# duckmayr/gpirt

Hardware: AMD Instinct MI355X
Metric: MCMC iterations/sec at N=8192 x m=1024 (higher is better)
Workload: dtype f64

## Files before the change

### gpirt_amd/_lib.py

```python
from __future__ import annotations

import ctypes as C
import os

import numpy as np

HERE = os.path.dirname(os.path.abspath(__file__))
LIB_PATH = os.environ.get("GPIRT_HIP_LIBRARY") or os.path.join(HERE, "libgpirt_hip.so")

NGRID = 1001
RNG_RSTREAM, RNG_ITEM = 0, 1
ST_INIT_F, ST_INIT_BETA, ST_F_Z, ST_F_ESS, ST_FSTAR, ST_THETA, ST_BETA = 1, 2, 3, 4, 5, 6, 7
ST_PPC = 8
ST_ELL = 9
ST_AMP = 10
ST_CARRY = 11

E_ARG, E_HIP, E_NODEVICE, E_ALLOC, E_RNG, E_INTERRUPT, E_NUMERIC = -1, -2, -3, -4, -5, -6, -7

SUM_THETA_BETA, SUM_F, SUM_PRED, SUM_WAIC = 1, 2, 4, 8
SUM_PARTS = {"theta_beta": SUM_THETA_BETA, "f": SUM_F, "pred": SUM_PRED, "waic": SUM_WAIC}
SUM_DIAG = 16
SUM_THETA_HIST, SUM_IRF_BAND = 32, 128
SUM_PARTS.update(diag=SUM_DIAG, theta_hist=SUM_THETA_HIST, irf_band=SUM_IRF_BAND)
# ... 650 lines not shown
    "gpirt_ppc_person_combine": (_i32, [_vp, _i32, C.POINTER(_vp), C.POINTER(PpcPerson)]),
    "gpirt_sampler_ppc_resid_enable": (_i32, [_vp, _i32]),
    "gpirt_sampler_ppc_resid_get": (_i32, [_vp, C.c_char_p, _vp, _i64]),
    "gpirt_sampler_ppc_resid_state": (_i32, [_vp, C.POINTER(_vp), C.POINTER(_i64)]),
    "gpirt_ppc_resid_combine": (_i32, [_vp, _i32, C.POINTER(_vp), C.POINTER(PpcResid)]),
    "gpirt_sampler_equate_enable": (_i32, [_vp, _vp, _vp, _i32]),
    "gpirt_sampler_equate_accumulate": (_i32, [_vp]),
    "gpirt_sampler_equate_get": (_i32, [_vp, C.c_char_p, _vp, _i64]),
    "gpirt_sampler_equate_state": (_i32, [_vp, C.POINTER(_vp), C.POINTER(_i64)]),
    "gpirt_equate_state_bytes": (_i32, [_i64, _i64, _i64, C.POINTER(_i64)]),
    "gpirt_equate_combine": (_i32, [_vp, _i32, C.POINTER(_vp), C.POINTER(Equate)]),
    "gpirt_sampler_loo_enable": (_i32, [_vp, _i64, _i32, _i32]),
    "gpirt_sampler_loo_accumulate": (_i32, [_vp]),
    "gpirt_sampler_loo_get": (_i32, [_vp, C.c_char_p, _vp, _i64]),
    "gpirt_sampler_loo_state": (_i32, [_vp, C.POINTER(_vp), C.POINTER(_i64)]),
    "gpirt_loo_tail_length": (_i32, [_i64, _i32, C.POINTER(_i64)]),
    "gpirt_loo_state_bytes": (_i32, [_i64, _i64, _i64, C.POINTER(_i64)]),
    "gpirt_loo_combine": (_i32, [_vp, _i32, C.POINTER(_vp), C.POINTER(Loo)]),
    "gpirt_sampler_shape_order_enable": (_i32, [_vp, _i32]),
    "gpirt_sampler_shape_order_get": (_i32, [_vp, C.c_char_p, _vp, _i64]),
    "gpirt_sampler_shape_order_state": (_i32, [_vp, C.POINTER(_vp), C.POINTER(_i64)]),
    "gpirt_shape_order_state_bytes": (_i32, [_i64, _i32, C.POINTER(_i64)]),
    "gpirt_shape_order_combine": (_i32, [_vp, _i32, C.POINTER(_vp), C.POINTER(ShapeOrder)]),
    "gpirt_sampler_summary_accumulate": (_i32, [_vp]),
    "gpirt_sampler_summary_get": (_i32, [_vp, C.c_char_p, _dp, _i64]),
    "gpirt_sampler_summary_totals": (_i32, [_vp, _dp]),
    "gpirt_sampler_create": (_i32, [C.POINTER(_vp), _vp, _dp, _i64, _i64, _dp, _dp, _dp, _dp,
                                     C.POINTER(Options), _vp]),
    "gpirt_sampler_destroy": (_i32, [_vp]),
    "gpirt_sampler_init": (_i32, [_vp]),
    "gpirt_sampler_step": (_i32, [_vp]),
    "gpirt_sampler_draw_f": (_i32, [_vp]),
    "gpirt_sampler_draw_fstar": (_i32, [_vp]),
    "gpirt_sampler_theta_partial": (_i32, [_vp]),
    "gpirt_sampler_theta_finish": (_i32, [_vp]),
    "gpirt_sampler_set_theta_block": (_i32, [_vp, _vp, _i64, _i64, _i64]),
    "gpirt_sampler_theta_block": (_i32, [_vp]),
    "gpirt_sampler_theta_commit": (_i32, [_vp]),
    "gpirt_sampler_draw_beta": (_i32, [_vp]),
    "gpirt_sampler_factor": (_i32, [_vp]),
    "gpirt_sampler_skip_factor": (_i32, [_vp]),
    "gpirt_sampler_adopt_factor": (_i32, [_vp, _i32]),
    "gpirt_sampler_build_cov": (_i32, [_vp]),
    "gpirt_sampler_panel_factor": (_i32, [_vp, _i64]),
    "gpirt_sampler_panel_update": (_i32, [_vp, _i64, _i64]),
    "gpirt_sampler_panel_copy": (_i32, [_vp, _i64, _vp, _i32]),
    "gpirt_sampler_panel_rows": (_i32, [_vp, C.POINTER(_i64)]),
    "gpirt_sampler_panel_factor_part": (_i32, [_vp, _i64, _i32]),
    "gpirt_sampler_panel_update_part": (_i32, [_vp, _i64, _i64, _i32]),
    "gpirt_sampler_panel_copy_part": (_i32, [_vp, _i64, _i32, _vp, _i64, _i32]),
    "gpirt_sampler_ldl": (_i32, [_vp, C.POINTER(_i64)]),
    "gpirt_sampler_nu_lr_draws": (_i32, [_vp, C.POINTER(_i64)]),
    "gpirt_sampler_ess_pack_draws": (_i32, [_vp, C.POINTER(_i64)]),
    "gpirt_sampler_nu_lr_rows": (_i32, [_vp, _vp, _i64]),
    "gpirt_sampler_fstar_free_draws": (_i32, [_vp, C.POINTER(_i64)]),
    "gpirt_sampler_factor_lr_count": (_i32, [_vp, C.POINTER(_i64)]),
    "gpirt_sampler_dense_factor_count": (_i32, [_vp, C.POINTER(_i64)]),
    "gpirt_sampler_dense_factor": (_i32, [_vp]),
    "gpirt_sampler_factor_lr_parts": (_i32, [_vp, _vp, _i64]),
    "gpirt_sampler_factor_lr_width": (_i32, [_vp, C.POINTER(_i32)]),
    "gpirt_sampler_factor_lr_blocks": (_i32, [_vp, _vp, _i64]),
    "gpirt_sampler_copy_state": (_i32, [_vp, _vp]),
    "gpirt_sampler_accumulate_irf": (_i32, [_vp]),
    "gpirt_sampler_iteration": (_i32, [_vp, C.POINTER(_i32)]),
    "gpirt_sampler_check": (_i32, [_vp]),
    "gpirt_sampler_devptr": (_i32, [_vp, C.c_char_p, C.POINTER(_vp), C.POINTER(_i64)]),
    "gpirt_sampler_get": (_i32, [_vp, C.c_char_p, _vp, _i64]),
    "gpirt_sampler_set": (_i32, [_vp, C.c_char_p, _dp, _i64]),
    "gpirt_sampler_finish_irfs": (_i32, [_vp, _i32, _dp]),
    "gpirt_sampler_enable_timing": (_i32, [_vp, _i32]),
    "gpirt_sampler_stage_times": (_i32, [_vp, _dp, _i32, C.POINTER(_i32), C.POINTER(C.c_char_p)]),
    "gpirt_prof_trailing": (_i32, [_vp, _i32, _dp, C.POINTER(_i64), _dp]),
    "gpirt_prof_enable": (_i32, [_vp, _i32]),
    "gpirt_prof_syrk": (_i32, [_vp, _i32, _i32, _dp, C.POINTER(_i64), _dp]),
    "gpirt_prof_syrk_bytes": (_i32, [_vp, _i32, _dp]),
    "gpirt_sampler_set_iteration": (_i32, [_vp, _i32]),
    "gpirt_ell_grid": (_i32, [_dbl, _dbl, _i32, _dp]),
    "gpirt_ell_check": (_i32, [_dbl, _dbl, _i32, _dp, _i32, _i32, C.POINTER(Kernel), C.POINTER(Options), _i64]),
    "gpirt_sampler_ell_enable": (_i32, [_vp, _dbl, _dbl, _i32, _dp, _i32, _i32, _i32]),
    "gpirt_sampler_draw_ell": (_i32, [_vp]),
    "gpirt_sampler_ell_width": (_i32, [_vp, _i32]),
    "gpirt_sampler_ell_get": (_i32, [_vp, C.c_char_p, _vp, _i64]),
    "gpirt_sampler_ell_stats": (_i32, [_vp, C.POINTER(Ell)]),
    "gpirt_sampler_draw_ell_centred": (_i32, [_vp]),
    "gpirt_sampler_ell_width_centred": (_i32, [_vp, _i32]),
    "gpirt_sampler_ell_centred_stats": (_i32, [_vp, C.POINTER(EllCentred)]),
    "gpirt_amp_check": (_i32, [_dbl, _dbl, _i32, _dp, _i32, C.POINTER(_i32), _i64, C.POINTER(Options)]),
    "gpirt_sampler_amp_set": (_i32, [_vp, _dp]),
    "gpirt_sampler_amp_enable": (_i32, [_vp, _dbl, _dbl, _i32, _dp, _i32, C.POINTER(_i32), _i64, _i32]),
    "gpirt_sampler_draw_amp": (_i32, [_vp]),
    "gpirt_sampler_amp_width": (_i32, [_vp, C.POINTER(_i32)]),
    "gpirt_sampler_amp_record": (_i32, [_vp]),
    "gpirt_sampler_amp_get": (_i32, [_vp, C.c_char_p, _vp, _i64]),
    "gpirt_sampler_amp_stats": (_i32, [_vp, C.POINTER(Amp)]),
    "gpirt_sampler_draw_amp_centred": (_i32, [_vp]),
    "gpirt_sampler_amp_centred_stats": (_i32, [_vp, C.POINTER(AmpCentred)]),
    "gpirt_sampler_draw_beta_centred": (_i32, [_vp]),
    "gpirt_sampler_beta_centred_get": (_i32, [_vp, C.c_char_p, _vp, _i64]),
    "gpirt_sampler_beta_centred_stats": (_i32, [_vp, C.POINTER(BetaCentred)]),
    "gpirt_sampler_scale_enable": (_i32, [_vp, _dbl, _dbl]),
    "gpirt_sampler_scale_width": (_i32, [_vp, _i32, _dbl]),
    "gpirt_sampler_draw_scale": (_i32, [_vp, _i32]),
    "gpirt_sampler_scale_get": (_i32, [_vp, C.c_char_p, _vp, _i64]),
    "gpirt_sampler_scale_stats": (_i32, [_vp, C.POINTER(Scale)]),
    "gpirt_sampler_step_consistent_scale": (_i32, [_vp, _i32, _i32]),
    "gpirt_pop_check": (_i32, [C.POINTER(C.c_int32), _i64, _i32, _dp, _i64, _i32, _dbl, _i32, _dbl, _dbl, _i32, _dp, _dp,
# ... 96 lines not shown
```

### gpirt_amd/csrc/api.hip

```cpp
#include "common.h"
#include "kernels.h"
#include "rstream.h"

#include <stdarg.h>
#include <stdlib.h>
#include <new>
#include <vector>
#include <algorithm>

namespace gpirt {

static thread_local char g_err[512] = "";

static int env_value(const char* name, int dflt)
{
    const char* v = getenv(name);
    if (!v || !*v) return dflt;
    return atoi(v);
}
const Config& env_config()
{
    static const Config c = [] {
        Config d;
        d.nbo = env_value("GPIRT_NBO", d.nbo);            d.nbp = env_value("GPIRT_NBP", d.nbp);
        d.lookahead = env_value("GPIRT_LOOKAHEAD", d.lookahead);
        d.panel = env_value("GPIRT_PANEL", d.panel);      d.defer = env_value("GPIRT_DEFER", d.defer);
        d.trsm_inv = env_value("GPIRT_TRSM_INV", d.trsm_inv);
        d.ll_exact = env_value("GPIRT_LL_EXACT", d.ll_exact);
        d.ess_screen = env_value("GPIRT_ESS_SCREEN", d.ess_screen);
        d.theta_fixed = env_value("GPIRT_THETA_FIXED", d.theta_fixed);
        d.bordered = env_value("GPIRT_BORDERED", d.bordered);
        d.early_inv = env_value("GPIRT_EARLY_INV", d.early_inv);
        d.prep_early = env_value("GPIRT_PREP_EARLY", d.prep_early);
        d.guard_verbose = env_value("GPIRT_GUARD_VERBOSE", d.guard_verbose);
        d.rs_predict = env_value("GPIRT_RS_PREDICT", d.rs_predict);
        d.rs_lr = env_value("GPIRT_RS_LR", d.rs_lr);
        d.nu_lr = env_value("GPIRT_NU_LR", d.nu_lr);
        d.nu_sub = env_value("GPIRT_NU_SUB", NU_LR_SUB);
        d.fstar_free = env_value("GPIRT_FSTAR_FREE", d.fstar_free);
        d.factor_lr = env_value("GPIRT_FACTOR_LR", d.factor_lr);
        d.flr_fuse = env_value("GPIRT_FLR_FUSE", d.flr_fuse);
        d.flr_narrow = env_value("GPIRT_FLR_NARROW", d.flr_narrow);
        d.beta_screen = env_value("GPIRT_BETA_SCREEN", d.beta_screen);
        d.zfill_compact = env_value("GPIRT_ZFILL_COMPACT", d.zfill_compact);
        d.ess_pack = env_value("GPIRT_ESS_PACK", d.ess_pack);
        if (d.nbo < 64) d.nbo = 1024;
        if (d.nbp != 0 && d.nbp < 64) d.nbp = 512;
        return d;
    }();
    return c;
}

void set_error(const char* fmt, ...)
{
    va_list ap;
    va_start(ap, fmt);
    vsnprintf(g_err, sizeof(g_err), fmt, ap);
    va_end(ap);
}

int ensure_work(gpirt_handle_t h, size_t bytes)
{
    if (bytes <= h->work_bytes) return 0;
    GP_HIP(hipStreamSynchronize(h->stream));
    if (h->d_work) GP_HIP(hipFree(h->d_work));
    h->d_work = nullptr;
    h->work_bytes = 0;
    hipError_t e = hipMalloc(&h->d_work, bytes);
    if (e != hipSuccess) { set_error("hipMalloc(%zu) failed: %s", bytes, hipGetErrorString(e)); return GPIRT_E_ALLOC; }
    h->work_bytes = bytes;
    GP_HIP(poison_fresh(h, h->d_work, bytes, h->stream));
    return 0;
}

static int check_device(int device)
{
    int count = 0;
    hipError_t e = hipGetDeviceCount(&count);
    if (e != hipSuccess || count <= 0) {
        set_error("no HIP device visible (%s): libgpirt_hip has no CPU fallback",
                  e == hipSuccess ? "device count 0" : hipGetErrorString(e));
        return GPIRT_E_NODEVICE;
    }
    if (device >= count) { set_error("device %d out of range (%d visible)", device, count); return GPIRT_E_ARG; }
    return 0;
}

__global__ __launch_bounds__(256) void mfma_f64_peak_kernel(double* out, int iters)
{
    d4 acc[8];
#pragma unroll
    for (int i = 0; i < 8; ++i) acc[i] = d4{0.0, 0.0, 0.0, 0.0};
    double a = 1.0 + threadIdx.x * 1e-3, b = 1.0 - threadIdx.x * 1e-3;
    for (int it = 0; it < iters; ++it) {
#pragma unroll
        for (int i = 0; i < 8; ++i) acc[i] = __builtin_amdgcn_mfma_f64_16x16x4f64(a, b, acc[i], 0, 0, 0);
    }
    double s = 0.0;
// ... 15 lines not shown

int potrf_panel_copy(hipStream_t stream, double* A, int64_t n, int64_t lda, int64_t p, double* buf, bool to_buf,
                     int64_t extra_rows, int half, int64_t capacity)
{
    const int64_t W = potrf_panel_width(), H = potrf_subpanel_width(n), P0 = p * W;
    if (p < 0 || P0 >= n || half < 0 || half > 2) { set_error("panel %lld / half %d out of range", (long long)p, half); return GPIRT_E_ARG; }
    const int64_t P1 = (P0 + W < n) ? P0 + W : n;
    const int64_t mid = (P0 + H < P1) ? P0 + H : P1;
    const int64_t K0 = (half == 1) ? mid : P0, K1 = (half == 0) ? mid : P1;
    const int64_t w = K1 - K0, rows = n + extra_rows - K0;
    if (w <= 0) return 0;
    if (capacity >= 0 && rows * w > capacity) {
        set_error("panel copy: part %d of panel %lld is %lld x %lld doubles, the buffer holds %lld", half, (long long)p,
                  (long long)rows, (long long)w, (long long)capacity);
        return GPIRT_E_ARG;
    }
    double* a = A + K0 + K0 * lda;
    if (to_buf) GP_HIP(hipMemcpy2DAsync(buf, (size_t)rows * 8, a, (size_t)lda * 8, (size_t)rows * 8, (size_t)w, hipMemcpyDeviceToDevice, stream));
    else        GP_HIP(hipMemcpy2DAsync(a, (size_t)lda * 8, buf, (size_t)rows * 8, (size_t)rows * 8, (size_t)w, hipMemcpyDeviceToDevice, stream));
    return 0;
}

}

using namespace gpirt;

static int create_own_stream(gpirt_handle_t* out, int device, bool high_priority);
namespace gpirt {
int create_side_handle(gpirt_handle_t* out, int device) { return create_own_stream(out, device, true); }
}

namespace gpirt {
int prof_pair_begin(gpirt_handle_t h, hipStream_t stream, ProfPair& pp)
{
    pp = ProfPair{nullptr, nullptr, 0.0, 0, 0.0};
    if (!h->prof.enabled) return 0;
    if (!h->prof.free_pairs.empty()) { pp = h->prof.free_pairs.back(); h->prof.free_pairs.pop_back(); }
    else { GP_HIP(hipEventCreate(&pp.e0)); GP_HIP(hipEventCreate(&pp.e1)); }
    GP_HIP(hipEventRecord(pp.e0, stream));
    return 0;
}
int prof_pair_end(gpirt_handle_t h, hipStream_t stream, ProfPair& pp, int cls, double flops, double bytes)
{
    if (!pp.e0) return 0;
    GP_HIP(hipEventRecord(pp.e1, stream));
    pp.flops = flops; pp.bytes = bytes; pp.cls = cls;
    h->prof.pending.push_back(pp);
    return 0;
}
}

extern "C" {

int gpirt_version(void) { return 144; }

const char* gpirt_last_error(void) { return g_err; }

int gpirt_device_count(int* count)
{
    GP_ARG(count != nullptr);
    int c = 0;
    hipError_t e = hipGetDeviceCount(&c);
    *count = (e == hipSuccess) ? c : 0;
    return 0;
}

int gpirt_create(gpirt_handle_t* out, int device, void* stream)
{
    GP_ARG(out != nullptr);
    *out = nullptr;
    GP_TRY(check_device(device < 0 ? 0 : device));
    if (device >= 0) GP_HIP(hipSetDevice(device));
    int cur = 0;
    GP_HIP(hipGetDevice(&cur));
    hipDeviceProp_t prop;
    GP_HIP(hipGetDeviceProperties(&prop, cur));
    if (strncmp(prop.gcnArchName, "gfx950", 6) != 0) {
        set_error("device %d is %s; libgpirt_hip is built for gfx950 (MI355X) only", cur, prop.gcnArchName);
        return GPIRT_E_NODEVICE;
    }
    gpirt_handle_s* h = new (std::nothrow) gpirt_handle_s();
    if (!h) { set_error("out of host memory"); return GPIRT_E_ALLOC; }
    h->device = cur;
    h->cfg = env_config();
    h->n_cu = prop.multiProcessorCount;
    h->stream = (hipStream_t)stream;
    h->own_stream = false;
    const size_t prog_cap = 2048;
    hipError_t e = hipMalloc(&h->d_info, 64);
    if (e == hipSuccess) e = hipMalloc(&h->d_prog, 2 * prog_cap * sizeof(unsigned long long));
    if (e == hipSuccess) e = hipHostMalloc(&h->h_info, 64, hipHostMallocDefault);
    if (e == hipSuccess) e = hipMemsetAsync(h->d_info, 0, 64, h->stream);
    if (e == hipSuccess) e = hipMemsetAsync(h->d_prog, 0, 2 * prog_cap * sizeof(unsigned long long), h->stream);
    if (e == hipSuccess) e = hipStreamSynchronize(h->stream);
    if (e != hipSuccess) {
        set_error("handle workspace setup failed: %s", hipGetErrorString(e));
        gpirt_destroy(h);
        return GPIRT_E_ALLOC;
    }
    h->prog_cap = prog_cap;
    *out = h;
    return 0;
}

int gpirt_destroy(gpirt_handle_t h)
{
    if (!h) return 0;
// ... 23 lines not shown
    if (h->own_stream) hipStreamDestroy(h->stream);
    delete h;
    return 0;
}

int gpirt_synchronize(gpirt_handle_t h)
{
    GP_ARG(h != nullptr);
    GP_HIP(hipStreamSynchronize(h->stream));
    return 0;
}

static int create_own_stream(gpirt_handle_t* out, int device, bool high_priority)
{
    GP_ARG(out != nullptr);
    *out = nullptr;
    GP_TRY(check_device(device < 0 ? 0 : device));
    if (device >= 0) GP_HIP(hipSetDevice(device));
    hipStream_t st = nullptr;
    int lo_pri = 0, hi_pri = 0;
    hipError_t e = hipSuccess;
    if (high_priority) e = hipDeviceGetStreamPriorityRange(&lo_pri, &hi_pri);
    if (e == hipSuccess)
        e = high_priority ? hipStreamCreateWithPriority(&st, hipStreamNonBlocking, hi_pri)
                          : hipStreamCreateWithFlags(&st, hipStreamNonBlocking);
    if (e != hipSuccess) { set_error("hipStreamCreate failed: %s", hipGetErrorString(e)); return GPIRT_E_HIP; }
    const int rc = gpirt_create(out, device, st);
    if (rc != 0) { hipStreamDestroy(st); return rc; }
    (*out)->own_stream = true;
    return 0;
}

int gpirt_create_own_stream(gpirt_handle_t* out, int device) { return create_own_stream(out, device, false); }

static int* config_slot(gpirt_handle_t h, const char* name, bool* read_only)
{
    struct E { const char* k; int* p; bool ro; } tab[] = {
        { "GPIRT_NBO", &h->cfg.nbo, true }, { "GPIRT_NBP", &h->cfg.nbp, true },
        { "GPIRT_LOOKAHEAD", &h->cfg.lookahead, false }, { "GPIRT_PANEL", &h->cfg.panel, false },
        { "GPIRT_DEFER", &h->cfg.defer, false }, { "GPIRT_TRSM_INV", &h->cfg.trsm_inv, false },
        { "GPIRT_LL_EXACT", &h->cfg.ll_exact, false }, { "GPIRT_ESS_SCREEN", &h->cfg.ess_screen, false }, { "GPIRT_THETA_FIXED", &h->cfg.theta_fixed, false }, { "GPIRT_BORDERED", &h->cfg.bordered, false },
        { "GPIRT_EARLY_INV", &h->cfg.early_inv, false }, { "GPIRT_PREP_EARLY", &h->cfg.prep_early, false },
        { "GPIRT_RS_PREDICT", &h->cfg.rs_predict, false },
        { "GPIRT_RS_LR", &h->cfg.rs_lr, false },
        { "GPIRT_NU_LR", &h->cfg.nu_lr, false },
        { "GPIRT_NU_SUB", &h->cfg.nu_sub, false },
        { "GPIRT_FSTAR_FREE", &h->cfg.fstar_free, false },
        { "GPIRT_FACTOR_LR", &h->cfg.factor_lr, false },
        { "GPIRT_FLR_FUSE", &h->cfg.flr_fuse, false },
        { "GPIRT_FLR_NARROW", &h->cfg.flr_narrow, false },
        { "GPIRT_BETA_SCREEN", &h->cfg.beta_screen, false },
        { "GPIRT_ZFILL_COMPACT", &h->cfg.zfill_compact, false },
        { "GPIRT_ESS_PACK", &h->cfg.ess_pack, false },
    };
    for (auto& e : tab)
        if (strcmp(e.k, name) == 0) { if (read_only) *read_only = e.ro; return e.p; }
    return nullptr;
}

int gpirt_config_get(gpirt_handle_t h, const char* name, int* value)
{
    GP_ARG(h && name && value);
    int* p = config_slot(h, name, nullptr);
    if (!p) { set_error("unknown switch '%s'", name); return GPIRT_E_ARG; }
    *value = *p;
    return 0;
}

int gpirt_config_set(gpirt_handle_t h, const char* name, int value)
{
    GP_ARG(h && name);
    bool ro = false;
    int* p = config_slot(h, name, &ro);
    if (!p) { set_error("unknown switch '%s'", name); return GPIRT_E_ARG; }
    if (ro) { set_error("%s is fixed per process (set it in the environment before the library is loaded)", name); return GPIRT_E_ARG; }
    if (p == &h->cfg.nu_sub && !nu_lr_sub_ok(value)) { set_error("GPIRT_NU_SUB must be 64, 128, 256 or 512 (got %d)", value); return GPIRT_E_ARG; }
    GP_HIP(hipStreamSynchronize(h->stream));
    *p = value;
    if (h->aux) *config_slot(h->aux, name, nullptr) = value;
    return 0;
}

void gpirt_kernel_default(gpirt_kernel* k)
{
    if (!k) return;
    memset(k, 0, sizeof(*k));
    k->family = GPIRT_KERNEL_SE;
    k->length_scale = 1.0;
}

int gpirt_kernel_check(const gpirt_kernel* k, int kstar_rank, double* cert_out, int* min_rank_out)
{
    if (cert_out) *cert_out = 0.0;
    if (min_rank_out) *min_rank_out = 0;
    KernelSpec spec;
    GP_TRY(kernel_spec_from(k, &spec));
    return kernel_rank_check(spec, kstar_rank, cert_out, min_rank_out);
}

int gpirt_kernel_set(gpirt_handle_t h, const gpirt_kernel* k)
{
    GP_ARG(h != nullptr);
    KernelSpec spec;
    GP_TRY(kernel_spec_from(k, &spec));
    if (h->live_samplers > 0) {
        set_error("gpirt_kernel_set: %d sampler(s) created on this handle are alive; a sampler keeps the kernel it was created "
// ... 625 lines not shown
```

### gpirt_amd/csrc/common.h

```cpp
#pragma once

#include <hip/hip_runtime.h>
#include <stdint.h>
#include <stdio.h>
#include <string.h>
#include <math.h>
#include <vector>

#include "../../include/gpirt_hip.h"

namespace gpirt {

void set_error(const char* fmt, ...);

#define GP_HIP(call)                                                                         \
    do {                                                                                     \
        hipError_t e_ = (call);                                                              \
        if (e_ != hipSuccess) {                                                              \
            gpirt::set_error("%s failed: %s (%s:%d)", #call, hipGetErrorString(e_), __FILE__, \
                             __LINE__);                                                      \
            return GPIRT_E_HIP;                                                              \
        }                                                                                    \
    } while (0)

#define GP_ARG(cond)                                                                         \
    do {                                                                                     \
        if (!(cond)) {                                                                       \
            gpirt::set_error("bad argument: %s (%s:%d)", #cond, __FILE__, __LINE__);         \
            return GPIRT_E_ARG;                                                              \
        }                                                                                    \
    } while (0)

#define GP_TRY(call)                                                                         \
    do {                                                                                     \
        int r_ = (call);                                                                     \
        if (r_ != 0) return r_;                                                              \
    } while (0)

constexpr int PROF_CLASSES = 6;
struct ProfPair { hipEvent_t e0, e1; double flops; int cls; double bytes; };
struct Prof {
    bool        enabled = false;
    double      ms[PROF_CLASSES] = {};
    int64_t     launches[PROF_CLASSES] = {};
    double      flops[PROF_CLASSES] = {};
    double      bytes[PROF_CLASSES] = {};
    std::vector<ProfPair> pending;
    std::vector<ProfPair> free_pairs;
};

struct Config {
    int  nbo = 1024, nbp = 0;
    int  lookahead = 1;
    int  panel = 1;
    int  defer = 0;
    int  trsm_inv = 1;
    int  ll_exact = 0;
    int  theta_fixed = 1;
    int  ess_screen = 1;
    int  bordered = 1;
    int  early_inv = 1;
    int  prep_early = 1;
    int  rs_lr = 1;
    int  nu_lr = 1;
    int  nu_sub = 0;
    int  fstar_free = 1;
    int  factor_lr = 1;
    int  flr_fuse = 1;
    int  flr_narrow = 1;
    int  beta_screen = 1;
    int  ess_pack = 1;
    int  zfill_compact = 1;
    int  rs_predict = 1;
    int  guard_verbose = 0;
};
const Config& env_config();

struct KernelSpec {
    int    family = GPIRT_KERNEL_SE;
    double length_scale = 1.0;
    double inv_ell = 1.0;
    bool is_default() const { return family == GPIRT_KERNEL_SE && length_scale == 1.0; }
};

}

struct gpirt_handle_s {
    int          device = 0;
    gpirt::Config cfg;
    gpirt::KernelSpec kern;
    hipStream_t  stream = nullptr;
    bool         own_stream = false;
    int*         d_info = nullptr;
    int*         h_info = nullptr;
    double*      d_work = nullptr;
    size_t       work_bytes = 0;
    gpirt::Prof  prof;
    hipStream_t  side = nullptr;
    hipEvent_t   ev_fork = nullptr, ev_join = nullptr, ev_mid = nullptr, ev_half = nullptr;
    gpirt_handle_t aux = nullptr;
    const double* inv_partial_L = nullptr;
    int64_t      inv_partial_pairs = 0;
    bool         slim_leaf = false;
    hipEvent_t   ev_prelast = nullptr;
    int64_t      prelast_cols = 0;
    unsigned long long* d_prog = nullptr;
    double*      d_winv = nullptr;
    int64_t      winv_blocks = 0;
    double*      d_defer_ws = nullptr;
    size_t       defer_ws_bytes = 0;
    size_t       prog_cap = 0;
    unsigned long long prog_seq = 0;
    long long*   panel_trace = nullptr;
    int64_t      panel_trace_k0 = -1;
    int64_t      panel_trace_cap = 0;
    int          n_cu = 0;
    int          live_samplers = 0;
    bool         zombie = false;
    int          guard_fallbacks = 0;
    int64_t      cur_nbp = 512;
    long long    factor_count = 0;
    int          rs_trace_pass = -1;
    int          rs_mispredict = 0;
    int          rs_cand_limit = 0;
// ... 141 lines not shown
```

### gpirt_amd/csrc/kernels.h

```cpp
#pragma once

#include "common.h"

namespace gpirt {

enum { TRI_NONE = 0, TRI_SYRK_LOWER = 1, TRI_A_LOWER = 2, TRI_A_UPPER = 3, TRI_SYRK_LOWER_TRAILING = 4,
       TRI_SYRK_LOWER_BACKGROUND = 5  };
bool gemm_trailing_uses_128(int64_t M, int64_t N, bool background = false);
int launch_gemm_update_potf2(hipStream_t stream, int64_t M, int64_t N, int64_t K, const double* P, int64_t ldp,
                             double* C, int64_t ldc, int nb_next, int k0_next, int* info);

int launch_gemm(gpirt_handle_t h, hipStream_t stream, bool ta, bool tb, int tri, int64_t M,
                int64_t N, int64_t K, double alpha, const double* A, int64_t lda, const double* B,
                int64_t ldb, double beta, double* C, int64_t ldc, int64_t Mread = 0, const int* run_if = nullptr);

int launch_gemm_batched(hipStream_t stream, bool ta, bool tb, int tri, int64_t M, int64_t N, int64_t K, double alpha,
                        const double* A, int64_t lda, int64_t strideA, const double* B, int64_t ldb, int64_t strideB,
                        double beta, double* C, int64_t ldc, int64_t strideC, int batch);
int launch_gemm_batched_dual(hipStream_t stream, int tri, int64_t M, int64_t N, int64_t K, const double* A, int64_t lda,
                             int64_t strideA, const double* B, int64_t ldb, int64_t strideB, int64_t K2, const double* A2,
                             int64_t lda2, int64_t strideA2, const double* B2, int64_t ldb2, int64_t strideB2, double* C,
                             int64_t ldc, int64_t strideC, int batch);

int launch_syrk_panels(hipStream_t stream, int64_t M, int64_t N, int64_t kpart, int nparts, double alpha, const double* A,
// ... 346 lines not shown
    int64_t n, m;
    int sub;
};
void nu_lr_nodes(std::vector<double>& nodes, std::vector<double>& wts);
int64_t nu_lr_slabs(int64_t n);
int launch_nu_lr_basis(hipStream_t stream, const double* theta, int64_t n, const double* nodes, const double* wts, double* V);
int launch_nu_lr(hipStream_t stream, const NuLrArgs& a, double* flops, double* bytes);
constexpr int FSTAR_FREE_RANK = NU_LR_RANK;
void fstar_free_factor(const KernelSpec& kern, std::vector<double>& F);
int launch_fstar_free(hipStream_t stream, const double* V, int64_t n, const double* F, double eps, double* work, double* parts,
                      int nsplit, double* Cu, int* err);
int launch_fstar_free_xhat(hipStream_t stream, const double* Gv, const double* F, double eps, double* Xh, int batch, int* err,
                           bool prefix = false, double* R = nullptr,
                           bool chain = false);
struct FactorLrArgs {
    const double* theta; int64_t n;
    const double *nodes, *wts;
    double* V;
    const double* F; double eps;
    double *G, *Xh;
    double* X;
    double* D;
    double* L; int64_t ldl;
    double* Bt;
    int* err;
    int part;
};
int64_t factor_lr_parts(int64_t n, int part = 0);
int launch_factor_lr(gpirt_handle_t h, hipStream_t stream, const FactorLrArgs& a);
int launch_rs3p_products(hipStream_t stream, const Rs3Args& a);
int launch_rs3p_decide(hipStream_t stream, const Rs3Args& a);
int launch_rs_pred_start(hipStream_t stream, const uint64_t* anchor, uint64_t* anchorP, const int* k_last, int64_t m);
int launch_rs_gather(hipStream_t stream, const double* Nrm, const uint64_t* posv, const uint64_t* anchorP, int64_t n, int64_t j0,
                     int64_t m, double* Z);
int launch_rs_verify(hipStream_t stream, const RsVerifyArgs& a);
int launch_rs_commit(hipStream_t stream, const RsVerifyArgs& a, uint64_t* anchor, uint64_t* pos, uint64_t* ctl, int* err, double* f,
                     int* k_out);
int launch_ll_term_probe(hipStream_t stream, const double* a, int64_t n, double* out, int fast);
int launch_ll_bar(hipStream_t stream, const double* f, const double* y, const double* mu, int64_t n,
                  int64_t m, double* out);

int launch_colnorm_s(hipStream_t stream, const double* tmp, int64_t n, int64_t N, int64_t ld, double* s);
int launch_lowrank_s(hipStream_t stream, const double* V, int64_t N, int r, const double* G, int64_t ldg, double* s);
struct FstarEpiArgs {
    const double* mean; const double* mu_star; const double* s; double* out;
    int64_t N, m;
    uint64_t seed; uint32_t iter; uint32_t item0;
    const double* U; uint64_t* pos; uint64_t cap; int* err;
    double* mean_out;
    int* off_scratch;
    const double* amp;
};
int launch_fstar_epilogue(hipStream_t stream, const FstarEpiArgs& a);

int launch_indicators(hipStream_t stream, const double* y, int64_t n, int64_t m, double* Ypm );
int launch_loglik_terms(hipStream_t stream, const double* fstar, int64_t N, int64_t m, double* Gpm , int64_t ldg,
                        const int* run_if = nullptr);
int launch_theta_nan_fix(hipStream_t stream, const double* Gpm, int64_t ldg, const double* Ypm , int64_t n, int64_t m,
                         double* lp, int64_t N, int64_t ldlp, const int* run_if = nullptr);
struct TfDims { int64_t mp, ksteps, iblocks, gblocks; };
TfDims tf_dims(int64_t n, int64_t m, int64_t N);
size_t tf_y8_bytes(const TfDims& d);
size_t tf_gq_bytes(const TfDims& d);
size_t tf_aux_bytes(const TfDims& d);
int* tf_overflow(void* aux, const TfDims& d);
int launch_tf_indicators(hipStream_t stream, const double* y, int64_t n, int64_t ldy, int64_t m, const TfDims& d, void* Y8);
int launch_theta_fixed(hipStream_t stream, const double* fstar, int64_t N, int64_t n, int64_t m, const TfDims& d,
                       const void* Y8, void* Gq, void* aux, double* logpost, int64_t ldlp, bool trace = false,
                       gpirt_handle_t prof = nullptr);
long long* tf_trace(void* aux, const TfDims& d);
int tf_trace_wgs();
struct ThetaArgs {
    const double* logpost;
    int64_t N, n;
    int64_t i0;
    int stabilise;
    uint64_t seed; uint32_t iter;
    const double* U; uint64_t* pos; uint64_t cap;
    double* theta_out; int* degenerate; int* err;
    const double* log_prior; const int32_t* codes;
};
int launch_theta_sample(hipStream_t stream, const ThetaArgs& a);

struct BetaArgs {
    double* beta; const double* theta; const double* y; const double* f;
    const double* pm; const double* ps; const double* step;
    int64_t n, m, N;
    double* mu; double* mu_star;
    uint64_t seed; uint32_t iter; uint32_t item0;
    const double* U; uint64_t* pos; const uint64_t* item_off; uint64_t cap; int* err;
    int screen;
    int* path;
};
int launch_draw_beta(hipStream_t stream, const BetaArgs& a);
int launch_linear_mean(hipStream_t stream, const double* x, int64_t n, const double* beta, int64_t m, double* mu);

int prof_pair_begin(gpirt_handle_t h, hipStream_t stream, ProfPair& pp);
int prof_pair_end(gpirt_handle_t h, hipStream_t stream, ProfPair& pp, int cls, double flops, double bytes);

int report_panel_guard(gpirt_handle_t h, const int* info_words, hipStream_t stream);

int create_side_handle(gpirt_handle_t* out, int device);

constexpr int SUM_LAYOUT_VERSION = 1;
constexpr int SUM_HEADER_WORDS = 8;
struct SumLayout {
    int64_t tb_mean = -1, tb_m2 = -1, lse = -1, ll_mean = -1, ll_m2 = -1, y = -1, p_sum = -1, f_mean = -1, f_m2 = -1, irf = -1;
    int64_t dtb[7] = { -1, -1, -1, -1, -1, -1, -1 };
    int64_t df[7] = { -1, -1, -1, -1, -1, -1, -1 };
    int64_t total = 0;
};
enum { DG_H1_MEAN, DG_H1_M2, DG_H2_MEAN, DG_H2_M2, DG_BSUM, DG_BM_MEAN, DG_BM_M2 };
SumLayout summary_layout(int64_t n, int64_t m, int parts);
struct QntLayout {
    int64_t th_hist[3] = { -1, -1, -1 };
    int64_t th_off = -1;
    int64_t psum = -1;
    int64_t band_nan = -1;
    int64_t band = -1;
    int64_t total = 0;
};
QntLayout quantile_layout(int64_t n, int64_t m, int parts);
// ... 526 lines not shown
```

### gpirt_amd/csrc/sampler.hip

```cpp
#include "common.h"
#include "kernels.h"
#include "rstream.h"

#include <stdlib.h>
#include <new>
#include <mutex>
#include <type_traits>
#include <string>
#include <vector>

using namespace gpirt;

namespace {

constexpr int KSPLIT = 16;

enum { ST_DRAW_F = 0, ST_FSTAR, ST_THETA_GEMM, ST_THETA_SAMPLE, ST_BETA, ST_FACTOR, ST_COUNT };
const char* const kStageNames[ST_COUNT] = { "draw_f", "draw_fstar", "theta_gemm", "theta_sample",
                                            "draw_beta", "factor" };

}

enum { ELL_WHITENED = 0, ELL_CENTRED = 1 };
struct EllUpdate {
// ... 92 lines not shown
    double last_ms = 0.0, item_ms = 0.0;
};

struct ScaleState {
    bool on = false;
    uint32_t t[2] = {};
    double width[2] = {};
    ScaleArgs a{};
    int last_kind = -1;
    int prior_ok = -1;
    hipEvent_t tev[7] = {};
    double last_ms[2] = {};
    double times[6] = {};
};

struct CarryState {
    int64_t calls = 0;
    unsigned long long* counters = nullptr;
    double* quad = nullptr;
    hipEvent_t tev[2] = {};
    double last_ms = 0.0;
};

struct gpirt_sampler_s {
    gpirt_handle_t h = nullptr;
    int64_t n = 0, m = 0, N = GPIRT_NGRID;
    gpirt_options opt{};
    KernelSpec kern;
    RStream* rs = nullptr;
    double *y = nullptr, *Ypm = nullptr, *theta = nullptr, *theta_new = nullptr, *f = nullptr,
           *Z = nullptr, *NU = nullptr, *beta = nullptr, *mu = nullptr, *mu_star = nullptr,
           *fstar = nullptr, *L = nullptr, *tstar = nullptr, *kstar = nullptr, *rhs = nullptr,
           *mean = nullptr, *s = nullptr, *Gpm = nullptr, *logpost = nullptr, *irf_sum = nullptr,
           *pm = nullptr, *ps = nullptr, *step = nullptr;
    int kr = 0;
    double *knodes = nullptr, *kV = nullptr, *kparts = nullptr, *kP = nullptr;
    int64_t ext = 0, ldl = 0, node_off = -1, rank_off = 0;
    bool ext_grid = false, rows_valid = false, fstar_rows = false;
    double *nu_nodes = nullptr, *nu_wts = nullptr, *nuV = nullptr, *nuT = nullptr;
    bool nu_kern_ok = false, theta_ok = false, theta_alone = false;
    int64_t nu_lr_draws = 0;
    gpirt_handle_t haux = nullptr;
    hipEvent_t ev_trmm = nullptr, ev_prep = nullptr;
    bool prep_valid = false, prep_pending = false;
    double *ffF = nullptr, *ffW = nullptr;
    bool ff_have = false, prep_free = false;
    double ff_ell = 0.0;
    int64_t fstar_free_draws = 0;
    double *theta_L = nullptr, *flrG = nullptr, *flrXh = nullptr, *flrX = nullptr, *flrD = nullptr;
    bool L_structured = false;
    int L_part_width = 0;
    hipEvent_t ev_flr = nullptr;
    int64_t factor_lr_count = 0, dense_factor_count = 0;
    uint32_t z_filled_iter = 0;
    hipEvent_t ev_zfill = nullptr;
    bool beta_deferred = false, beta_pending = false;
    hipEvent_t ev_beta = nullptr;
    int64_t blk_i0 = 0, blk_n = 0, blk_m = 0;
    double *Ypm_blk = nullptr, *Gpm_full = nullptr, *logpost_blk = nullptr, *fstar_full = nullptr, *theta_stage = nullptr;
    TfDims tfd{}, tfd_blk{};
    double *tf_y8 = nullptr, *tf_gq = nullptr, *tf_aux = nullptr, *tf_y8_blk = nullptr, *tf_gq_blk = nullptr, *tf_aux_blk = nullptr;
    int *ess_k = nullptr, *flags = nullptr;
    int *fstar_off = nullptr;
    int *h_flags = nullptr;
    double* U = nullptr; double* hU = nullptr; uint64_t U_cap = 0;
    uint64_t* pos = nullptr; uint64_t* h_pos = nullptr; uint64_t* beta_off = nullptr;
    uint64_t beta_total = 0;
    RStream saved{};
    bool stream_open = false;
    gpirt_rstream_s* rs_obj = nullptr;
    bool ahead_attached = false;
    uint64_t ahead_gen = 0, ahead_used = 0, a_len = 0;
    std::vector<std::pair<uint64_t, RStream>> snaps;
    uint32_t *hA = nullptr, *Sraw = nullptr;
    double *S = nullptr, *U2 = nullptr;
    hipStream_t cs = nullptr;
    hipEvent_t ev_up = nullptr, ev_asm = nullptr;
    bool spec_ok = false;
    uint64_t *posv = nullptr, *anchor = nullptr, *h_next = nullptr;
    unsigned long long* rs_flags = nullptr; double* rs_partial = nullptr; uint64_t rs_tag = 0;
    double* Lt = nullptr;
    double *Nrm = nullptr, *rs_part = nullptr;
    uint32_t* rs_units = nullptr; int rs_nunits = 0, rs_nfull = 0;
    uint32_t* rs_unitsP = nullptr; int rs_nunitsP = 0, rs_nfullP = 0;
    long long* rs_trace = nullptr;
    float *Lt32 = nullptr, *rs_part32 = nullptr;
    uint64_t *anchorP = nullptr, *rs_ctl = nullptr, *rs_posP = nullptr;
    double *rs_dec_part = nullptr, *rs_dec_rec = nullptr; unsigned* rs_dec_ticket = nullptr;
    double rs_pass_rate = 0.0; uint64_t rs_pass_seen = 0;
    int *rs_kpred = nullptr, *rs_kv = nullptr, *rs_used = nullptr, *rs_ierr = nullptr, *rs_errP = nullptr;
    double *lr_nodes = nullptr, *lr_wts = nullptr, *lr_M = nullptr, *lr_V64 = nullptr, *lr_Gb = nullptr;
    float *lr_V32t = nullptr, *lr_Ct32 = nullptr, *lr_Y = nullptr;
    int* lr_bad = nullptr; uint32_t* lr_units = nullptr; int lr_nunits = 0;
    bool lr_on = false; int lr_strikes = 0; uint64_t rs_mis_seen = 0;
    int iter = 0;
    bool initialised = false;
    bool sticky_info = false;
    bool factor_fresh = false;
    bool counted = false;
    bool in_init = false;
    bool timing = false;
    hipEvent_t ev[ST_COUNT + 1] = {};
    double stage_ms[ST_COUNT] = {};
    std::vector<void*> allocs;
    std::vector<double> host_tmp;
    SummaryState sum;
    PpcState ppc;
    RankState rank;
    ShapeState shape;
    ScoreState score;
    SumscoreState sumscore;
    EquateState equate;
    LooState loo;
    AcfState acf;
    GroupsState groups;
    EllState ell;
    AmpState amp;
    OrdState ord;
    PopState pop;
    CarryState carry;
    SmoothF sf;
    BetaCentredState bc;
    ScaleState sc;
    bool lp_current = false;
    bool mu_linear = false;
    uint32_t* ess_ypk = nullptr;
    bool ess_ypk_valid = false;
    int64_t ess_pack_draws = 0;
};

namespace {

template <typename T>
int dalloc(gpirt_sampler_s* s, T** p, size_t count, bool numbers = true)
{
    void* q = nullptr;
    const size_t bytes = (count ? count : 1) * sizeof(T);
    hipError_t e = hipMalloc(&q, bytes);
    if (e != hipSuccess) {
        set_error("hipMalloc(%zu bytes) failed: %s", bytes, hipGetErrorString(e));
        return GPIRT_E_ALLOC;
    }
    s->allocs.push_back(q);
    *p = reinterpret_cast<T*>(q);
    if (std::is_same<T, double>::value || std::is_same<T, float>::value) {
        if (numbers && poison_fresh(s->h, q, bytes, s->h->stream) != hipSuccess) {
            set_error("hipMemsetAsync(%zu bytes) failed", bytes);
            return GPIRT_E_HIP;
        }
    }
    return 0;
}

inline bool stream_mode(const gpirt_sampler_s* s) { return s->opt.rng_kind == GPIRT_RNG_RSTREAM; }

int report_degenerate_theta(gpirt_sampler_s* s, int count);

void ahead_generate(gpirt_sampler_s* s, uint32_t* dst, uint64_t count)
{
    constexpr uint64_t EVERY = 1ull << 16;
    while (count) {
        const uint64_t c = count < EVERY ? count : EVERY;
        s->snaps.emplace_back(s->ahead_gen, *s->rs);
        s->rs->fill_raw(dst, c);
        s->ahead_gen += c; dst += c; count -= c;
    }
}

void ahead_resolve(void* owner, bool gone)
{
    gpirt_sampler_s* s = static_cast<gpirt_sampler_s*>(owner);
    if (s->ahead_attached) {
        if (s->ev_up) hipEventSynchronize(s->ev_up);
        size_t best = 0;
        for (size_t q = 0; q < s->snaps.size(); ++q) if (s->snaps[q].first <= s->ahead_used) best = q;
        *s->rs = s->snaps[best].second;
        s->rs->skip(s->ahead_used - s->snaps[best].first);
    }
    s->ahead_attached = false;
    s->snaps.clear();
    s->ahead_gen = s->ahead_used = s->a_len = 0;
    if (s->rs_obj) { s->rs_obj->owner = nullptr; s->rs_obj->resolve = nullptr; }
    if (gone) { s->rs_obj = nullptr; s->rs = nullptr; }
// ... 156 lines not shown
        std::lock_guard<std::mutex> lock(mu);
        if (cached.empty() || cached_ell != s->kern.length_scale) {
            fstar_free_factor(s->kern, cached);
            cached_ell = s->kern.length_scale;
        }
        F = cached;
    }
    GP_HIP(hipMemcpyAsync(s->ffF, F.data(), sizeof(double) * F.size(), hipMemcpyHostToDevice, s->h->stream));
    GP_HIP(hipStreamSynchronize(s->h->stream));
    s->ff_have = true; s->ff_ell = s->kern.length_scale;
    return 0;
}

bool fstar_free_ok(const gpirt_sampler_s* s, bool state_only = false)
{
    const int mode = s->h->cfg.fstar_free;
    return mode != 2 && (mode == 3 || s->n >= 2048) && s->kr == NU_LR_RANK && s->fstar_rows && s->node_off >= 0 && s->nuV &&
           !stream_mode(s) && s->nu_kern_ok && !s->opt.kernel_fp32 && s->theta_ok && (state_only || !s->theta_alone) && !s->ell.on &&
           s->ffF && s->ff_have && s->kern.family == GPIRT_KERNEL_SE && s->ff_ell == s->kern.length_scale;
}

bool factor_lr_ok(const gpirt_sampler_s* s)
{
    const Config& c = s->h->cfg;
    return s->opt.factor_structured && s->theta_L && c.factor_lr != 2 && (c.factor_lr == 3 || s->n >= 2048) &&
           c.nu_lr != 2 && (c.nu_lr == 3 || s->n >= 2048) && fstar_free_ok(s, true);
}

int fstar_prep_free(gpirt_sampler_s* s, hipStream_t st, bool basis)
{
    const int64_t n = s->n;
    const int r = s->kr;
    const double* Bt = s->L + n + s->rank_off;
    if (basis) GP_TRY(launch_nu_lr_basis(st, s->theta, n, s->nu_nodes, s->nu_wts, s->nuV));
    GP_TRY(launch_fstar_free(st, s->nuV, n, s->ffF, GPIRT_JITTER, s->ffW, s->kparts, KSPLIT, s->rhs + (size_t)n * r, s->flags));
    return launch_gemm_splitk(st, false, true, r, r, n, 1.0, Bt, s->ldl, Bt, s->ldl, s->kparts, r, (int64_t)r * r, KSPLIT,
                              s->kP, r, 0.0);
}
int report_degenerate_theta(gpirt_sampler_s* s, int count);
int rebuild_rows(gpirt_sampler_s* s);
int beta_sync(gpirt_sampler_s* s);
int ensure_dense_factor(gpirt_sampler_s* s);
int ensure_factor_width(gpirt_sampler_s* s, int need);

int z_sync(gpirt_sampler_s* s)
{
    if (s->z_filled_iter != 0 && s->ev_zfill) GP_HIP(hipStreamWaitEvent(s->h->stream, s->ev_zfill, 0));
    s->z_filled_iter = 0;
    return 0;
}

int do_draw_f(gpirt_sampler_s* s)
{
    s->lp_current = false;
    gpirt_handle_t h = s->h;
    hipStream_t st = h->stream;
    const int64_t n = s->n, m = s->m;
    const uint32_t iter = (uint32_t)(s->iter + 1);
    GP_TRY(beta_sync(s));
    s->factor_fresh = false;
    if (!stream_mode(s)) {
        const bool nu_lr = s->node_off >= 0 && s->nuV && h->cfg.nu_lr != 2 && (h->cfg.nu_lr == 3 || n >= 2048) &&
                           s->nu_kern_ok && !s->opt.kernel_fp32 && s->theta_ok && !s->theta_alone;
        if (!nu_lr) GP_TRY(ensure_dense_factor(s));
        if (nu_lr) GP_TRY(rebuild_rows(s));
        if (nu_lr) GP_TRY(ensure_factor_width(s, h->cfg.nu_sub));
        const bool prep = s->haux && s->kr > 0 && s->fstar_rows && s->rows_valid && !s->prep_valid;
        const bool free = prep && fstar_free_ok(s);
        if (prep && !free) GP_TRY(ensure_dense_factor(s));
        const bool early = prep && !free && !(h->cfg.prep_early == 2 && m > 128);
        if (early || (free && !nu_lr)) GP_HIP(hipEventRecord(s->ev_trmm, st));
        if (nu_lr && s->prep_pending && s->prep_free) {
            GP_HIP(hipStreamWaitEvent(st, s->ev_prep, 0));
            s->prep_pending = false;
        }
        if (s->z_filled_iter == iter && s->ev_zfill) {
            GP_HIP(hipStreamWaitEvent(st, s->ev_zfill, 0));
            s->z_filled_iter = 0;
        } else {
            GP_TRY(z_sync(s));
            GP_TRY(launch_item_uniforms(st, s->opt.seed, iter, GPIRT_ST_F_Z, (uint32_t)s->opt.item0, m, n, s->Z, true, s->h->cfg.zfill_compact == 1));
        }
        {
            ProfPair pp;
            GP_TRY(prof_pair_begin(h, st, pp));
            if (nu_lr) {
                double flops = 0.0, bytes = 0.0;
                NuLrArgs q{};
                q.L = s->L; q.ldl = s->ldl; q.Bt = s->L + n + s->node_off; q.V = s->nuV; q.Z = s->Z; q.NU = s->NU; q.T = s->nuT;
                q.n = n; q.m = m; q.sub = h->cfg.nu_sub;
                GP_TRY(launch_nu_lr_basis(st, s->theta, n, s->nu_nodes, s->nu_wts, s->nuV));
                if (free) GP_HIP(hipEventRecord(s->ev_trmm, st));
                GP_TRY(launch_nu_lr(st, q, &flops, &bytes));
                GP_TRY(prof_pair_end(h, st, pp, 3, flops, bytes));
                s->nu_lr_draws += 1;
            } else {
                GP_TRY(launch_gemm(h, st, false, false, TRI_A_LOWER, n, m, n, 1.0, s->L, s->ldl, s->Z, n, 0.0, s->NU, n));
                GP_TRY(prof_pair_end(h, st, pp, 3, (double)n * (double)n * (double)m, 8.0 * (0.5 * (double)n * (double)n + 2.0 * (double)n * (double)m)));
            }
        }
        if (s->amp.mode) GP_TRY(launch_amp_scale(st, s->NU, s->amp.amp, n, m));
        if (prep && !early && !free) GP_HIP(hipEventRecord(s->ev_trmm, st));
        if (s->ord.on) {
            EssOrdArgs a{};
            a.f = s->f; a.nu = s->NU; a.mu = s->mu; a.cat = s->ord.cat; a.thr = s->ord.thr; a.counts = s->ord.counts;
            a.C = s->ord.C; a.n = n; a.m = m; a.k_out = s->ess_k; a.err = s->flags;
            a.seed = s->opt.seed; a.iter = iter; a.item0 = (uint32_t)s->opt.item0;
// ... 129 lines not shown
        if (predict) GP_HIP(hipMemcpyAsync(s->h_next + 2, s->rs_ctl + 3, sizeof(uint64_t), hipMemcpyDeviceToHost, st));
        if (predict) GP_HIP(hipMemcpyAsync(s->h_next + 3, s->rs_ctl + 1, sizeof(uint64_t), hipMemcpyDeviceToHost, st));
        if (lr) GP_HIP(hipMemcpyAsync(s->h_next + 4, s->lr_bad, sizeof(int), hipMemcpyDeviceToHost, st));
        if (s->stream_open && !topped) { GP_TRY(ahead_topup(s, stream_window(s))); topped = true; }
        GP_HIP(hipStreamSynchronize(st));
        if ((int)s->h_next[1] != 0) break;
        if (predict) {
            if (lr && (int)s->h_next[4] != 0) { s->lr_on = false; lr = false; }
            if (lr && s->h_next[3] != s->rs_mis_seen) { lr = false; lr_missed = true; }
            s->rs_mis_seen = s->h_next[3];
        }
        if ((int64_t)s->h_next[0] <= done) {
            if (predict) {
                predict = false;
                GP_TRY(launch_advance_pos(st, s->rs_ctl + 2, 1));
                continue;
            }
            set_error("R-stream replay: draw_f made no progress"); return GPIRT_E_NUMERIC;
        }
        if (predict && (int64_t)s->h_next[0] > done) {
            const uint64_t real = s->h_next[2] - s->rs_pass_seen;
            s->rs_pass_seen = s->h_next[2];
            s->rs_pass_rate = (double)real / (double)((int64_t)s->h_next[0] - done);
        }
        done = (int64_t)s->h_next[0];
    }
    if (s->lr_on) {
        s->lr_strikes = lr_missed ? s->lr_strikes + 1 : 0;
        if (s->lr_strikes >= 3) s->lr_on = false;
    }
    return 0;
}

int fstar_prep(gpirt_sampler_s* s, gpirt_handle_t hh)
{
    hipStream_t st = hh->stream;
    const int64_t n = s->n;
    const int r = s->kr;
    double* Cu = s->rhs + (size_t)n * r;
    const double* Bt = s->L + n + s->rank_off;
    GP_TRY(launch_transpose(st, Bt, r, n, s->ldl, Cu, n));
    if (hh == s->haux && hh->inv_partial_L == s->L && hh->inv_partial_pairs > 0 && hh->trsm_winv_L != s->L) {
        GP_TRY(trsm_inverses_build(hh, st, s->L, n, s->ldl, true, hh->inv_partial_pairs, (n / 256) / 2));
        trsm_inverses_mark(hh, s->L, n, s->ldl, true);
        hh->inv_partial_L = nullptr; hh->inv_partial_pairs = 0;
    }
    GP_TRY(launch_trsm_lower(hh, st, s->L, n, s->ldl, Cu, r, n, true, true));
    return launch_gemm_splitk(st, false, true, r, r, n, 1.0, Bt, s->ldl, Bt, s->ldl, s->kparts, r, (int64_t)r * r, KSPLIT,
                              s->kP, r, 0.0);
}

int do_draw_fstar(gpirt_sampler_s* s, uint32_t iter)
{
    s->lp_current = false;
    gpirt_handle_t h = s->h;
    hipStream_t st = h->stream;
    const int64_t n = s->n, m = s->m, N = s->N;
    double* tmp = s->rhs;
    double* W = s->rhs + (size_t)n * N;
    const bool fused = s->opt.fstar_fused != 0;
    GP_TRY(beta_sync(s));
    s->factor_fresh = false;
    GP_TRY(rebuild_rows(s));
    if (s->kr > 0) {
        const int r = s->kr;
        double* Bu = s->rhs;
        double* Cu = s->rhs + (size_t)n * r;
        const bool bordered = s->fstar_rows;
        if (bordered) {
            if (!s->prep_valid) {
                if (s->prep_pending) { GP_HIP(hipStreamWaitEvent(st, s->ev_prep, 0)); s->prep_pending = false; }
                s->prep_free = fstar_free_ok(s);
                if (s->prep_free) GP_TRY(fstar_prep_free(s, st, true));
                else { GP_TRY(ensure_dense_factor(s)); GP_TRY(fstar_prep(s, h)); }
                s->prep_valid = true;
            }
            else if (s->prep_pending) { GP_HIP(hipStreamWaitEvent(st, s->ev_prep, 0)); s->prep_pending = false; }
            if (s->prep_free) s->fstar_free_draws += 1;
        } else {
            GP_TRY(launch_se_kernel(st, s->kern, s->theta, n, s->knodes, r, Bu, n, 0.0));
            GP_TRY(launch_trsm_lower(h, st, s->L, n, s->ldl, Bu, r, n, false));
            GP_HIP(hipMemcpyAsync(Cu, Bu, sizeof(double) * (size_t)n * r, hipMemcpyDeviceToDevice, st));
            GP_TRY(launch_trsm_lower(h, st, s->L, n, s->ldl, Cu, r, n, true, true));
        }
        double* G = s->kP;
        double* Q = s->kP + (size_t)r * r;
        if (!bordered)
            GP_TRY(launch_gemm_splitk(st, true, false, r, r, n, 1.0, Bu, n, Bu, n, s->kparts, r, (int64_t)r * r, KSPLIT, G, r, 0.0));
        GP_TRY(launch_gemm_splitk(st, true, false, r, m, n, 1.0, Cu, n, s->f, n, s->kparts, r, (int64_t)r * m, KSPLIT, Q, r, 0.0));
        GP_TRY(launch_lowrank_s(st, s->kV, N, r, G, r, s->s));
        GP_TRY(launch_gemm(h, st, false, false, TRI_NONE, N, m, r, 1.0, s->kV, N, Q, r, 0.0, s->mean, N));
        FstarEpiArgs a{};
        a.mean = s->mean; a.mu_star = s->mu_star; a.s = s->s; a.out = s->fstar; a.N = N; a.m = m;
        a.seed = s->opt.seed; a.iter = iter; a.item0 = (uint32_t)s->opt.item0; a.err = s->flags;
        if (stream_mode(s)) { a.U = s->U; a.pos = s->pos; a.cap = s->U_cap; a.off_scratch = s->fstar_off; }
        if (s->shape.on) a.mean_out = s->shape.gbar;
        if (s->amp.mode) a.amp = s->amp.amp;
        return launch_fstar_epilogue(st, a);
    }
    GP_HIP(hipMemcpyAsync(W, s->f, sizeof(double) * (size_t)n * m, hipMemcpyDeviceToDevice, st));
    if (s->ext_grid) {
        if (!fused) GP_TRY(launch_se_kernel(st, s->kern, s->theta, n, s->tstar, N, s->kstar, n, 0.0));
        GP_TRY(launch_transpose(st, s->L + n, N, n, s->ldl, tmp, n));
        GP_TRY(launch_trsm_lower(h, st, s->L, n, s->ldl, W, m, n, false));
    } else {
        if (fused) {
            GP_TRY(launch_se_kernel(st, s->kern, s->theta, n, s->tstar, N, tmp, n, 0.0));
        } else {
            GP_TRY(launch_se_kernel(st, s->kern, s->theta, n, s->tstar, N, s->kstar, n, 0.0));
            GP_HIP(hipMemcpyAsync(tmp, s->kstar, sizeof(double) * (size_t)n * N, hipMemcpyDeviceToDevice, st));
        }
        GP_TRY(launch_trsm_lower(h, st, s->L, n, s->ldl, s->rhs, N + m, n, false));
    }
    GP_TRY(launch_colnorm_s(st, tmp, n, N, n, s->s));
    if (fused) {
        GP_TRY(launch_gemm(h, st, true, false, TRI_NONE, N, m, n, 1.0, tmp, n, W, n, 0.0, s->mean, N));
    } else {
        GP_TRY(launch_trsm_lower(h, st, s->L, n, s->ldl, W, m, n, true, true));
        GP_TRY(launch_gemm(h, st, true, false, TRI_NONE, N, m, n, 1.0, s->kstar, n, W, n, 0.0, s->mean, N));
    }
    FstarEpiArgs a{};
    a.mean = s->mean; a.mu_star = s->mu_star; a.s = s->s; a.out = s->fstar; a.N = N; a.m = m;
    a.seed = s->opt.seed; a.iter = iter; a.item0 = (uint32_t)s->opt.item0; a.err = s->flags;
    if (stream_mode(s)) { a.U = s->U; a.pos = s->pos; a.cap = s->U_cap; a.off_scratch = s->fstar_off; }
    if (s->shape.on) a.mean_out = s->shape.gbar;
    if (s->amp.mode) a.amp = s->amp.amp;
    return launch_fstar_epilogue(st, a);
}

int theta_product(gpirt_sampler_s* s, const double* fstar_in, double* logpost_out)
{
    hipStream_t st = s->h->stream;
    const int64_t n = s->n, m = s->m, N = s->N;
    const int64_t Np = (N + 127) / 128 * 128;
    const int* only_if = nullptr;
    if (s->h->cfg.theta_fixed == 1) {
        GP_TRY(launch_theta_fixed(st, fstar_in, N, n, m, s->tfd, s->tf_y8, s->tf_gq, s->tf_aux, logpost_out, N, false, s->h));
        only_if = tf_overflow(s->tf_aux, s->tfd);
    }
    GP_TRY(launch_loglik_terms(st, fstar_in, N, m, s->Gpm, Np, only_if));
    GP_TRY(launch_gemm(s->h, st, false, true, TRI_NONE, N, n, 2 * m, 1.0, s->Gpm, Np, s->Ypm, n, 0.0, logpost_out, N, Np, only_if));
    return launch_theta_nan_fix(st, s->Gpm, Np, s->Ypm, n, m, logpost_out, N, N, only_if);
}

int theta_product_ord(gpirt_sampler_s* s, const double* fstar_in, double* logpost_out)
{
    hipStream_t st = s->h->stream;
    const OrdState& A = s->ord;
    const int64_t n = s->n, m = s->m, N = s->N;
    const int64_t Np = (N + 127) / 128 * 128;
    GP_TRY(launch_ord_loglik_terms(st, fstar_in, N, m, A.C, A.thr, A.G, Np));
    GP_TRY(launch_gemm(s->h, st, false, true, TRI_NONE, N, n, (int64_t)A.C * m, 1.0, A.G, Np, A.Y, n, 0.0, logpost_out, N, Np));
    return launch_ord_nan_fix(st, A.G, Np, A.cat, n, m, logpost_out, N, N);
}

int do_theta_partial(gpirt_sampler_s* s)
{
    if (s->ord.on) {
        GP_TRY(theta_product_ord(s, s->fstar, s->logpost));
        s->lp_current = true;
        return 0;
    }
    GP_TRY(theta_product(s, s->fstar, s->logpost));
    s->lp_current = true;
    return 0;
}

int do_theta_finish(gpirt_sampler_s* s)
{
    hipStream_t st = s->h->stream;
    ThetaArgs a{};
    a.logpost = s->logpost; a.N = s->N; a.n = s->n; a.stabilise = s->opt.theta_stabilise;
    a.seed = s->opt.seed; a.iter = (uint32_t)(s->iter + 1);
    a.theta_out = s->theta; a.degenerate = s->flags + 1; a.err = s->flags;
    if (stream_mode(s)) { a.U = s->U; a.pos = s->pos; a.cap = s->U_cap; }
    if (s->pop.mode) { a.log_prior = s->pop.log_prior; a.codes = s->pop.codes; }
    GP_TRY(launch_theta_sample(st, a));
    if (stream_mode(s)) GP_TRY(launch_advance_pos(st, s->pos, (uint64_t)s->n));
    s->lp_current = false;
    s->mu_linear = false;
    s->theta_ok = true;
    return 0;
}

int do_theta_block(gpirt_sampler_s* s)
{
    hipStream_t st = s->h->stream;
    const int64_t N = s->N, nb = s->blk_n, mt = s->blk_m;
    const int64_t Np = (N + 127) / 128 * 128;
    GP_HIP(hipMemsetAsync(s->theta_stage, 0, sizeof(double) * (size_t)s->n, st));
    if (nb == 0) return 0;
    const int* only_if = nullptr;
    if (s->h->cfg.theta_fixed == 1) {
        GP_TRY(launch_theta_fixed(st, s->fstar_full, N, nb, mt, s->tfd_blk, s->tf_y8_blk, s->tf_gq_blk, s->tf_aux_blk, s->logpost_blk, N, false, s->h));
        only_if = tf_overflow(s->tf_aux_blk, s->tfd_blk);
    }
    GP_TRY(launch_loglik_terms(st, s->fstar_full, N, mt, s->Gpm_full, Np, only_if));
    GP_TRY(launch_gemm(s->h, st, false, true, TRI_NONE, N, nb, 2 * mt, 1.0, s->Gpm_full, Np, s->Ypm_blk, nb, 0.0,
                       s->logpost_blk, N, Np, only_if));
    GP_TRY(launch_theta_nan_fix(st, s->Gpm_full, Np, s->Ypm_blk, nb, mt, s->logpost_blk, N, N, only_if));
    ThetaArgs a{};
    a.logpost = s->logpost_blk; a.N = N; a.n = nb; a.i0 = s->blk_i0; a.stabilise = s->opt.theta_stabilise;
    a.seed = s->opt.seed; a.iter = (uint32_t)(s->iter + 1);
    a.theta_out = s->theta_stage; a.degenerate = s->flags + 1; a.err = s->flags;
    return launch_theta_sample(st, a);
}

int launch_beta_on(gpirt_sampler_s* s, hipStream_t st)
{
    s->lp_current = false;
    s->mu_linear = !s->ord.on;
    if (s->ord.on) {
        BetaOrdArgs a{};
        a.beta = s->beta; a.theta = s->theta; a.cat = s->ord.cat; a.f = s->f; a.thr = s->ord.thr; a.pm = s->pm; a.ps = s->ps;
        a.step = s->step; a.C = s->ord.C; a.n = s->n; a.m = s->m; a.N = s->N; a.mu = s->mu; a.mu_star = s->mu_star;
        a.seed = s->opt.seed; a.iter = (uint32_t)(s->iter + 1); a.item0 = (uint32_t)s->opt.item0;
        return launch_draw_beta_ord(st, a);
    }
    BetaArgs a{};
    a.beta = s->beta; a.theta = s->theta; a.y = s->y; a.f = s->f; a.pm = s->pm; a.ps = s->ps;
    a.step = s->step; a.n = s->n; a.m = s->m; a.N = s->N; a.mu = s->mu; a.mu_star = s->mu_star;
    a.seed = s->opt.seed; a.iter = (uint32_t)(s->iter + 1); a.item0 = (uint32_t)s->opt.item0;
    a.err = s->flags;
    a.screen = s->h->cfg.beta_screen == 1;
    if (stream_mode(s)) { a.U = s->U; a.pos = s->pos; a.item_off = s->beta_off; a.cap = s->U_cap; }
    GP_TRY(launch_draw_beta(st, a));
    if (stream_mode(s)) GP_TRY(launch_advance_pos(st, s->pos, s->beta_total));
    return 0;
}

int beta_sync(gpirt_sampler_s* s)
{
    if (s->beta_deferred) {
        s->beta_deferred = false;
        GP_TRY(launch_beta_on(s, s->h->stream));
    }
    if (s->beta_pending) {
        GP_HIP(hipStreamWaitEvent(s->h->stream, s->ev_beta, 0));
        s->beta_pending = false;
    }
    return 0;
}

int do_draw_beta(gpirt_sampler_s* s)
{
    const bool defer = s->h->cfg.early_inv != 2 && !stream_mode(s) && s->haux && s->ev_beta && s->initialised;
    GP_TRY(beta_sync(s));
    if (defer) { s->beta_deferred = true; return 0; }
    return launch_beta_on(s, s->h->stream);
}

int carry_refusals(gpirt_sampler_s* s, int nugget, const char* entry)
{
    if (!s->initialised) { set_error("%s needs an initialised sampler (gpirt_sampler_init)", entry); return GPIRT_E_ARG; }
    if (stream_mode(s)) {
        set_error("carry: rng = reference (GPIRT_RNG_RSTREAM) is refused, R's stream has no such draw");
        return GPIRT_E_ARG;
    }
    if (nugget != 0 && nugget != 1) { set_error("carry: nugget = %d, it must be 0 or 1", nugget); return GPIRT_E_ARG; }
    return 0;
}

int do_carry_f(gpirt_sampler_s* s, int nugget, bool timed)
{
    CarryState& c = s->carry;
    hipStream_t st = s->h->stream;
    GP_TRY(beta_sync(s));
    s->lp_current = false;
    s->mu_linear = false;
    if (!c.counters) {
        GP_TRY(dalloc(s, &c.counters, 6));
        GP_HIP(hipMemsetAsync(c.counters, 0, 6 * sizeof(unsigned long long), st));
    }
    CarryArgs a{};
    a.slot = (int)(c.calls & 1);
    a.f = s->f; a.theta = s->theta; a.fstar = s->fstar; a.mu_star = s->mu_star; a.n = s->n; a.m = s->m; a.N = s->N;
    a.amp = s->amp.mode ? s->amp.amp : nullptr;
    a.counters = c.counters;
    a.seed = s->opt.seed; a.iter = (uint32_t)(s->iter + 1); a.item0 = (uint32_t)s->opt.item0; a.nugget = nugget;
    if (timed) {
        for (hipEvent_t& t : c.tev) if (!t) GP_HIP(hipEventCreate(&t));
        GP_HIP(hipEventRecord(c.tev[0], st));
    }
    GP_TRY(launch_carry_f(st, a));
    if (timed) GP_HIP(hipEventRecord(c.tev[1], st));
    c.calls += 1;
    c.last_ms = 0.0;
    return 0;
}

void invalidate_factor_products(gpirt_sampler_s* s)
{
    s->prep_valid = false;
    if (s->haux && s->haux->inv_partial_L == s->L) { s->haux->inv_partial_L = nullptr; s->haux->inv_partial_pairs = 0; }
    if (s->h->trsm_winv_L == s->L) s->h->trsm_winv_L = nullptr;
    if (s->haux && s->haux->trsm_winv_L == s->L) s->haux->trsm_winv_L = nullptr;
}

int aux_join(gpirt_sampler_s* s, bool beta_too = true, bool z_too = true)
{
    hipStream_t st = s->h->stream;
    if (s->prep_pending) { GP_HIP(hipStreamWaitEvent(st, s->ev_prep, 0)); s->prep_pending = false; }
    if (beta_too) GP_TRY(beta_sync(s));
    if (z_too) GP_TRY(z_sync(s));
    return 0;
}

int build_cov(gpirt_sampler_s* s, const double* theta = nullptr)
{
    hipStream_t st = s->h->stream;
    if (!theta) theta = s->theta;
    s->L_structured = false;
    GP_TRY(launch_se_kernel_lower(st, s->kern, theta, s->n, s->L, s->ldl, GPIRT_JITTER, s->opt.kernel_fp32 != 0));
    if (s->fstar_rows && s->kr > 0) GP_TRY(launch_se_kernel(st, s->kern, s->knodes, s->kr, theta, s->n, s->L + s->n + s->rank_off, s->ldl, 0.0));
    if (s->ext_grid) GP_TRY(launch_se_kernel(st, s->kern, s->tstar, s->N, theta, s->n, s->L + s->n, s->ldl, 0.0));
    if (s->node_off >= 0 && !(s->fstar_rows && s->kr == NU_LR_RANK))
        GP_TRY(launch_se_kernel(st, s->kern, s->nu_nodes, NU_LR_RANK, theta, s->n, s->L + s->n + s->node_off, s->ldl, 0.0));
    return 0;
}

int rebuild_rows(gpirt_sampler_s* s)
// ... 204 lines not shown
                     (void*)p->hist_mu, (void*)p->hist_sd, (void*)p->draws })
        if (q) hipFree(q);
    for (hipEvent_t t : p->tev) if (t) hipEventDestroy(t);
    const uint32_t calls = p->t;
    *p = PopState();
    p->t = calls;
}

int ell_join(gpirt_sampler_s* s)
{
    GP_TRY(aux_join(s, true, false));
    if (s->haux) {
        GP_HIP(hipEventRecord(s->ell.ev, s->haux->stream));
        GP_HIP(hipStreamWaitEvent(s->h->stream, s->ell.ev, 0));
    }
    return 0;
}

void ell_set_kernel(gpirt_sampler_s* s, double ell)
{
    s->kern.length_scale = ell;
    s->kern.inv_ell = 1.0 / ell;
}

int ell_settle_factor(gpirt_sampler_s* s)
{
    if (!s->factor_fresh) return 0;
    gpirt_handle_t h = s->h;
    hipStream_t st = h->stream;
    GP_HIP(hipMemcpyAsync(h->h_info, h->d_info, 8 * sizeof(int), hipMemcpyDeviceToHost, st));
    GP_HIP(hipStreamSynchronize(st));
    if (h->h_info[1] != 0) {
        if (h->cfg.panel == 2) return report_panel_guard(h, h->h_info, st);
        GP_TRY(recover_factor(s));
        GP_HIP(hipMemcpyAsync(h->h_info, h->d_info, 8 * sizeof(int), hipMemcpyDeviceToHost, st));
        GP_HIP(hipStreamSynchronize(st));
        if (h->h_info[1] != 0) return report_panel_guard(h, h->h_info, st);
    }
    if (*h->h_info > 0) {
        set_error("chol(): decomposition failed (leading minor of order %d is not positive definite)", *h->h_info);
        return *h->h_info;
    }
    return 0;
}

int do_draw_ell(gpirt_sampler_s* s, int kind)
{
    EllState& e = s->ell;
    EllUpdate& c = e.up[kind];
    gpirt_handle_t h = s->h;
    hipStream_t st = h->stream;
    const int64_t n = s->n, m = s->m;
    GP_TRY(ell_settle_factor(s));
    s->lp_current = false;
    const uint32_t t = c.t + 1;
    const double u0 = item_uniform(s->opt.seed, t, GPIRT_ST_ELL, (uint32_t)kind, 0),
                 u1 = item_uniform(s->opt.seed, t, GPIRT_ST_ELL, (uint32_t)kind, 1);
    auto counted = [&]() { c.t = t; c.updates += 1; c.last_u0 = u0; c.last_u1 = u1; };
    const int w = c.w;
    int j = (int)floor(u0 * (double)(2 * w));
    if (j > 2 * w - 1) j = 2 * w - 1;
    const int kp = e.k + (j < w ? j - w : j - w + 1);
    if (kp < 0 || kp >= e.P) { counted(); c.last_proposed = kp; c.out_of_range += 1; c.last = 2; return 0; }
    GP_TRY(ell_join(s));
    GP_TRY(ensure_dense_factor(s));
    s->factor_fresh = false;
    const bool timed = s->timing;
    if (timed)
        for (hipEvent_t& t : e.tev) if (!t) GP_HIP(hipEventCreate(&t));
    auto tick = [&](int i) { if (timed) hipEventRecord(e.tev[i], st); };
    const KernelSpec kern_before = s->kern;
    const bool rows_before = s->rows_valid;
    const size_t fbytes = sizeof(double) * (size_t)(n * m), lbytes = sizeof(double) * (size_t)(s->ldl * n);
    auto restore = [&]() -> int {
        s->kern = kern_before;
        s->rows_valid = rows_before;
        invalidate_factor_products(s);
        GP_HIP(hipMemcpyAsync(s->L, e.Lsave, lbytes, hipMemcpyDeviceToDevice, st));
        return 0;
    };
    tick(0);
    GP_HIP(hipMemcpyAsync(s->NU, s->f, fbytes, hipMemcpyDeviceToDevice, st));
    if (kind == ELL_CENTRED) GP_HIP(hipMemcpyAsync(e.nuprop, s->f, fbytes, hipMemcpyDeviceToDevice, st));
    GP_HIP(hipMemcpyAsync(e.Lsave, s->L, lbytes, hipMemcpyDeviceToDevice, st));
    tick(1);
    GP_TRY(launch_trsm_lower(h, st, s->L, n, s->ldl, s->NU, m, n, false));
    tick(2);
    ell_set_kernel(s, e.grid[(size_t)kp]);
    int rc = factor_core(s);
    c.factorisations += 1;
    tick(3);
    const double lp_diff = e.log_prior[(size_t)kp] - e.log_prior[(size_t)e.k], log_u = log(u1);
    for (int attempt = 0; !rc; ++attempt) {
        if (kind == ELL_WHITENED) {
            rc = launch_gemm(h, st, false, false, TRI_A_LOWER, n, m, n, 1.0, s->L, s->ldl, s->NU, n, 0.0, e.fprop, n);
            tick(4);
            if (!rc) rc = launch_ell_delta(st, s->f, e.fprop, s->mu, s->y, n, m, e.delta, e.nonfin);
            tick(5);
            if (!rc) rc = launch_ell_decide(st, e.delta, e.nonfin, m, lp_diff, log_u, h->d_info, e.rec, e.flag);
            tick(6);
            if (!rc) rc = launch_ell_commit(st, e.flag, s->f, e.fprop, n * m);
            tick(7);
        } else {
            if (attempt > 0 && hipMemcpyAsync(e.nuprop, s->f, fbytes, hipMemcpyDeviceToDevice, st) != hipSuccess) {
                set_error("length-scale update: copying f failed: %s", hipGetErrorString(hipGetLastError()));
                rc = GPIRT_E_HIP;
            }
// ... 265 lines not shown
}

}

extern "C" {

int gpirt_sampler_create(gpirt_sampler_t* out, gpirt_handle_t h, const double* h_y, int64_t n,
                         int64_t m, const double* h_theta0, const double* h_pm, const double* h_ps,
                         const double* h_step, const gpirt_options* opts, gpirt_rstream_t rs)
{
    GP_ARG(out && h && h_y && h_theta0 && h_pm && h_ps && h_step && n > 0 && m > 0);
    *out = nullptr;
    for (int64_t i = 0; i < n * m; ++i) {
        const double v = h_y[i];
        if (!(v == 1.0 || v == -1.0 || v != v)) { set_error("y must be +1, -1 or NaN (a missing response)"); return GPIRT_E_ARG; }
    }
    gpirt_sampler_s* s = new (std::nothrow) gpirt_sampler_s();
    if (!s) { set_error("out of host memory"); return GPIRT_E_ALLOC; }
    s->h = h; s->n = n; s->m = m; s->N = GPIRT_NGRID;
    if (opts) s->opt = *opts; else gpirt_default_options(&s->opt);
    if (s->opt.m_total <= 0) s->opt.m_total = m;
    s->kern = h->kern;
    if (!s->kern.is_default()) {
        if (s->opt.kernel_fp32) {
            set_error("kernel_fp32 needs the default kernel (squared exponential, length_scale 1): the handle's kernel is family %d, "
                      "length_scale %g", s->kern.family, s->kern.length_scale);
            delete s;
            return GPIRT_E_ARG;
        }
        if (s->opt.kstar_rank != 0 && s->opt.fstar_fused && s->opt.kstar_rank >= 16 && s->opt.kstar_rank <= 128 &&
            (s->opt.kstar_rank % 16) == 0) {
            const int rc_k = kernel_rank_check(s->kern, s->opt.kstar_rank, nullptr, nullptr);
            if (rc_k) { delete s; return rc_k; }
        }
    }
    if (stream_mode(s)) {
        if (!rs) { set_error("GPIRT_RNG_RSTREAM needs an R stream state"); delete s; return GPIRT_E_ARG; }
        if (s->opt.item0 != 0 || s->opt.m_total != m) {
            set_error("R-stream replay is sequential over items and cannot be sharded"); delete s; return GPIRT_E_ARG;
        }
        rstream_sync(rs);
        s->rs = &rs->r; s->rs_obj = rs;
        rs->attached.push_back(s); rs->forget = rstream_forget;
    }
    const int64_t N = s->N;
    hipStream_t st = h->stream;
    int rc = 0;
#define GP_A(p, cnt) do { rc = dalloc(s, &(p), (size_t)(cnt)); if (rc) { gpirt_sampler_destroy(s); return rc; } } while (0)
    GP_A(s->y, n * m);       GP_A(s->Ypm, n * 2 * m);  GP_A(s->theta, n);       GP_A(s->theta_new, n);
    s->tfd = tf_dims(n, m, N);
#define GP_AI(p, cnt) do { rc = dalloc(s, &(p), (size_t)(cnt), false); if (rc) { gpirt_sampler_destroy(s); return rc; } } while (0)
    GP_AI(s->tf_y8, tf_y8_bytes(s->tfd) / 8 + 2); GP_AI(s->tf_gq, tf_gq_bytes(s->tfd) / 8 + 2); GP_AI(s->tf_aux, tf_aux_bytes(s->tfd) / 8 + 2);
#undef GP_AI
    GP_A(s->f, n * m);       GP_A(s->Z, n * m);        GP_A(s->NU, n * (m > 1 + TRMV_SPLIT ? m : 1 + TRMV_SPLIT));   GP_A(s->beta, 2 * m);
    s->kr = s->opt.kstar_rank;
    if (s->kr != 0 && (!s->opt.fstar_fused || s->kr < 16 || s->kr > 128 || (s->kr % 16) != 0)) {
        set_error("kstar_rank must be a multiple of 16 in 16..128 and needs fstar_fused");
        gpirt_sampler_destroy(s);
        return GPIRT_E_ARG;
    }
    if (s->opt.factor_structured != 0 && s->opt.factor_structured != 1) {
        set_error("factor_structured must be 0 or 1");
        gpirt_sampler_destroy(s);
        return GPIRT_E_ARG;
    }
    const bool bordered_ok = (n % 64) == 0 && h->cfg.bordered != 2;
    if (bordered_ok) {
        if (s->kr == NU_LR_RANK) { s->ext = s->kr; s->node_off = 0; s->rank_off = 0; s->fstar_rows = true; }
        else if (s->kr > 0) { s->ext = NU_LR_RANK + s->kr; s->node_off = 0; s->rank_off = NU_LR_RANK; s->fstar_rows = true; }
        else if (n >= 1024) {
            s->node_off = (N + 63) / 64 * 64;
            s->ext = s->node_off + NU_LR_RANK;
            s->ext_grid = true; s->fstar_rows = true;
        } else { s->ext = NU_LR_RANK; s->node_off = 0; }
    } else if ((n % 64) == 0) { s->ext = NU_LR_RANK; s->node_off = 0; }
    s->ldl = n + s->ext;
    s->theta_ok = true;
    for (int64_t i = 0; i < n; ++i) s->theta_ok = s->theta_ok && h_theta0[i] >= -5.0 && h_theta0[i] <= 5.0;
    s->nu_kern_ok = nu_kernel_ok(s->kern);
    GP_A(s->mu, n * m);      GP_A(s->mu_star, N * m + 1); GP_A(s->fstar, N * m + 1); GP_A(s->L, s->ldl * n);
    GP_A(s->tstar, N + 1);   GP_A(s->rhs, n * (N + m) + 2); GP_A(s->mean, N * m + 1); GP_A(s->s, N + 1);
    GP_A(s->Gpm, ((N + 127) / 128 * 128) * 2 * m + 2); GP_A(s->logpost, N * n + 2); GP_A(s->irf_sum, N * m + 1);
    if (hipMemsetAsync(s->Gpm, 0, sizeof(double) * (size_t)(((N + 127) / 128 * 128) * 2 * m + 2), st) != hipSuccess) {
        set_error("hipMemsetAsync(Gpm) failed"); gpirt_sampler_destroy(s); return GPIRT_E_HIP;
    }
    GP_A(s->pm, 2 * m);      GP_A(s->ps, 2 * m);       GP_A(s->step, 2 * m);
    GP_A(s->ess_k, m);       GP_A(s->flags, 4);
    if (!stream_mode(s) && ess_pack_eligible(n)) {
        rc = dalloc(s, &s->ess_ypk, (size_t)(512 * m), false);
        if (rc) { gpirt_sampler_destroy(s); return rc; }
    }
    if (!s->opt.fstar_fused) GP_A(s->kstar, n * N + 2);
    if (s->node_off >= 0) {
        GP_A(s->nu_nodes, NU_LR_RANK); GP_A(s->nu_wts, NU_LR_RANK);
        if (!stream_mode(s)) {
            GP_A(s->nuV, n * NU_LR_RANK); GP_A(s->nuT, nu_lr_slabs(n) * NU_LR_RANK * m);
            if (hipMemsetAsync(s->nuT, 0, sizeof(double) * (size_t)(NU_LR_RANK * m), st) != hipSuccess) {
                set_error("hipMemsetAsync(nuT) failed"); gpirt_sampler_destroy(s); return GPIRT_E_HIP;
            }
        }
        if (!stream_mode(s) && s->kr == NU_LR_RANK && s->fstar_rows) {
            GP_A(s->ffF, FSTAR_FREE_RANK * FSTAR_FREE_RANK); GP_A(s->ffW, 2 * FSTAR_FREE_RANK * FSTAR_FREE_RANK);
            if (s->opt.factor_structured) {
                const int64_t fp = factor_lr_parts(n, NU_LR_SUB_MIN) * NU_LR_RANK * NU_LR_RANK;
                GP_A(s->theta_L, n); GP_A(s->flrG, fp); GP_A(s->flrXh, fp); GP_A(s->flrX, NU_LR_RANK * n);
                GP_A(s->flrD, factor_lr_parts(n) * (NU_LR_PART / 64) * NU_LR_RANK * NU_LR_RANK);
// ... 305 lines not shown
}

int gpirt_sampler_draw_f(gpirt_sampler_t s) { GP_ARG(s && s->initialised); return do_draw_f(s); }
int gpirt_sampler_draw_fstar(gpirt_sampler_t s) { GP_ARG(s && s->initialised); return do_draw_fstar(s, (uint32_t)(s->iter + 1)); }
int gpirt_sampler_theta_partial(gpirt_sampler_t s) { GP_ARG(s && s->initialised); return do_theta_partial(s); }
int gpirt_sampler_theta_finish(gpirt_sampler_t s) { GP_ARG(s && s->initialised); return do_theta_finish(s); }

int gpirt_sampler_set_theta_block(gpirt_sampler_t s, const double* y_block, int64_t i0, int64_t n_block, int64_t m_total)
{
    GP_ARG(s && (y_block || n_block == 0) && i0 >= 0 && n_block >= 0 && i0 + n_block <= s->n && m_total >= s->m);
    if (stream_mode(s)) { set_error("the R-stream replay cannot be sharded"); return GPIRT_E_ARG; }
    if (s->fstar_full) { set_error("the theta block is already set"); return GPIRT_E_ARG; }
    GP_TRY(ord_refuse(s, "gpirt_sampler_set_theta_block", "the respondent-block theta path has no one-hot product"));
    if (s->pop.mode) {
        set_error("gpirt_sampler_set_theta_block is refused while a population prior is on: the block path would need the codes of its respondents");
        return GPIRT_E_ARG;
    }
    const int64_t N = s->N, Np = (N + 127) / 128 * 128;
    int rc = 0;
    double* yb = nullptr;
#define GP_B(p, cnt) do { rc = dalloc(s, &(p), (size_t)(cnt)); if (rc) return rc; } while (0)
    GP_B(s->Ypm_blk, n_block * 2 * m_total + 2); GP_B(s->Gpm_full, Np * 2 * m_total + 2);
    GP_B(s->logpost_blk, N * n_block + 2);       GP_B(s->fstar_full, N * m_total + 2);
    GP_B(s->theta_stage, s->n + 1);              GP_B(yb, n_block * m_total + 1);
    s->tfd_blk = tf_dims(n_block, m_total, N);
#undef GP_B
#define GP_B(p, cnt) do { rc = dalloc(s, &(p), (size_t)(cnt), false); if (rc) return rc; } while (0)
    GP_B(s->tf_y8_blk, tf_y8_bytes(s->tfd_blk) / 8 + 2); GP_B(s->tf_gq_blk, tf_gq_bytes(s->tfd_blk) / 8 + 2);
    GP_B(s->tf_aux_blk, tf_aux_bytes(s->tfd_blk) / 8 + 2);
#undef GP_B
    hipStream_t st = s->h->stream;
    GP_HIP(hipMemsetAsync(s->Gpm_full, 0, sizeof(double) * (size_t)(Np * 2 * m_total + 2), st));
    if (n_block > 0) {
        GP_HIP(hipMemcpyAsync(yb, y_block, sizeof(double) * (size_t)(n_block * m_total), hipMemcpyHostToDevice, st));
        GP_TRY(launch_indicators(st, yb, n_block, m_total, s->Ypm_blk));
        GP_TRY(launch_tf_indicators(st, yb, n_block, n_block, m_total, s->tfd_blk, s->tf_y8_blk));
    }
    GP_HIP(hipStreamSynchronize(st));
    s->blk_i0 = i0; s->blk_n = n_block; s->blk_m = m_total;
    return 0;
}

int gpirt_sampler_theta_block(gpirt_sampler_t s)
{
    GP_ARG(s && s->initialised);
    if (!s->fstar_full) { set_error("gpirt_sampler_set_theta_block has not been called"); return GPIRT_E_ARG; }
    return do_theta_block(s);
}

int gpirt_sampler_theta_commit(gpirt_sampler_t s)
{
    GP_ARG(s && s->initialised && s->theta_stage);
    GP_HIP(hipMemcpyAsync(s->theta, s->theta_stage, sizeof(double) * (size_t)s->n, hipMemcpyDeviceToDevice, s->h->stream));
    s->lp_current = false;
    s->mu_linear = false;
    s->theta_ok = true;
    return 0;
}
int gpirt_sampler_draw_beta(gpirt_sampler_t s) { GP_ARG(s && s->initialised); return do_draw_beta(s); }
int gpirt_sampler_factor(gpirt_sampler_t s)
{
    GP_ARG(s && s->initialised);
    GP_TRY(do_factor(s));
    s->iter += 1;
    return 0;
}

int gpirt_sampler_build_cov(gpirt_sampler_t s)
{
    GP_ARG(s && s->initialised);
    hipStream_t st = s->h->stream;
    if (!s->sticky_info) GP_HIP(hipMemsetAsync(s->h->d_info, 0, sizeof(int), st));
    GP_TRY(aux_join(s));
    invalidate_factor_products(s);
    return build_cov(s);
}

int gpirt_sampler_adopt_factor(gpirt_sampler_t s, int rows_with_L)
{
    GP_ARG(s && s->initialised);
    GP_TRY(beta_sync(s));
    invalidate_factor_products(s);
    s->L_structured = false;
    s->factor_fresh = false;
    s->rows_valid = rows_with_L != 0;
    s->theta_alone = false;
    s->iter += 1;
    return 0;
}

int gpirt_sampler_skip_factor(gpirt_sampler_t s) { return gpirt_sampler_adopt_factor(s, 0); }

int gpirt_sampler_step(gpirt_sampler_t s)
{
    GP_ARG(s && s->initialised);
    if (stream_mode(s)) GP_TRY(stream_begin(s, stream_window(s)));
    mark(s, 0);
    GP_TRY(do_draw_f(s));            mark(s, 1);
    GP_TRY(do_draw_fstar(s, (uint32_t)(s->iter + 1))); mark(s, 2);
    GP_TRY(do_theta_partial(s));     mark(s, 3);
    GP_TRY(do_theta_finish(s));      mark(s, 4);
    GP_TRY(do_draw_beta(s));         mark(s, 5);
    GP_TRY(do_factor(s));            mark(s, 6);
    s->iter += 1;
    if (stream_mode(s)) GP_TRY(stream_end(s, stream_window(s)));
    if (s->timing) {
        GP_HIP(hipEventSynchronize(s->ev[ST_COUNT]));
// ... 1188 lines not shown
    std::vector<double> F;
    fstar_free_factor(s->kern, F);
    uint64_t live = 0;
    int r = 0;
    for (int k = 0; k < R; ++k) {
        long double sq = 0.0L;
        for (int i = 0; i < R; ++i) sq += (long double)F[(size_t)(i + R * k)] * (long double)F[(size_t)(i + R * k)];
        if (sq <= 1e-13L) { for (int i = 0; i < R; ++i) F[(size_t)(i + R * k)] = 0.0; }
        else { live |= 1ull << k; r += 1; }
    }
    hipStream_t st = s->h->stream;
    S.have = false;
    GP_HIP(hipMemcpyAsync(S.F, F.data(), sizeof(double) * F.size(), hipMemcpyHostToDevice, st));
    GP_HIP(hipStreamSynchronize(st));
    S.live = live; S.r = r;
    S.have = true; S.ell = s->kern.length_scale;
    return 0;
}

int gpirt_sampler_draw_amp_centred(gpirt_sampler_t s)
{
    GP_ARG(s != nullptr);
    const char* me = "gpirt_sampler_draw_amp_centred";
    GP_TRY(ord_refuse(s, "gpirt_sampler_draw_amp_centred", ORD_BINARY));
    if (!s->initialised) { set_error("%s needs an initialised sampler (gpirt_sampler_init)", me); return GPIRT_E_ARG; }
    if (stream_mode(s)) { set_error("%s: rng = reference (GPIRT_RNG_RSTREAM) is refused, R's stream has no such draw", me); return GPIRT_E_ARG; }
    if (s->opt.kernel_fp32) { set_error("%s: kernel_fp32 is refused, the single-precision build is the default kernel's alone", me); return GPIRT_E_ARG; }
    if (s->opt.item0 != 0 || (s->opt.m_total > 0 && s->opt.m_total != s->m)) {
        set_error("%s: an item shard (item0 = %lld, m_total = %lld) is refused, the amplitudes are kept for all items of one sampler", me,
                  (long long)s->opt.item0, (long long)s->opt.m_total);
        return GPIRT_E_ARG;
    }
    AmpState& A = s->amp;
    if (A.mode != 2) {
        set_error("%s: the amplitudes are not in the sampled mode (gpirt_sampler_amp_enable): %s", me,
                  A.mode == 1 ? "they are fixed" : "they are off");
        return GPIRT_E_ARG;
    }
    if (!s->nu_kern_ok) {
        if (s->kern.family != GPIRT_KERNEL_SE) {
            set_error("%s: the handle's kernel is not a squared exponential, it has no rank-64 form (gpirt_kernel_check(kernel, 64))", me);
            return GPIRT_E_ARG;
        }
        const int rc = kernel_rank_check(s->kern, AMP_CENTRED_RANK, nullptr, nullptr);
        if (rc) return rc;
        set_error("%s: the length-scale grid's smallest value fails gpirt_kernel_check(kernel, 64)", me);
        return GPIRT_E_ARG;
    }
    if (!s->theta_ok) {
        set_error("%s: a theta is not finite or lies outside [-5, 5], the rank-64 basis does not hold there", me);
        return GPIRT_E_ARG;
    }
    GP_TRY(beta_sync(s));
    s->lp_current = false;
    s->mu_linear = false;
    GP_TRY(amp_centred_alloc(s));
    GP_TRY(smooth_factor(s));
    AmpCentredArgs a = A.ca;
    a.F = s->sf.F; a.live = s->sf.live; a.r = s->sf.r;
    a.f = s->f; a.mu = s->mu; a.y = s->y; a.n = s->n; a.m = s->m;
    a.theta = s->theta; a.eps = GPIRT_JITTER;
    a.H = s->NU;
    a.grid = A.d_grid; a.log_prior = A.d_log_prior; a.P = A.P;
    a.idx = A.idx; a.amp = A.amp;
    a.seed = s->opt.seed; a.t = A.ct + 1; a.item0 = (uint32_t)s->opt.item0;
    a.err = s->flags;
    hipStream_t st = s->h->stream;
    const bool timed = s->timing;
    if (timed) {
        for (hipEvent_t& t : A.ctev) if (!t) GP_HIP(hipEventCreate(&t));
        GP_HIP(hipEventRecord(A.ctev[0], st));
    }
    GP_TRY(launch_amp_centred(st, a));
    A.ct += 1;
    if (timed) {
        GP_HIP(hipEventRecord(A.ctev[1], st));
        GP_HIP(hipEventSynchronize(A.ctev[1]));
        float ms = 0.f;
        hipEventElapsedTime(&ms, A.ctev[0], A.ctev[1]);
        A.clast_ms = ms;
    }
    return 0;
}

int gpirt_sampler_amp_centred_stats(gpirt_sampler_t s, gpirt_amp_centred* out)
{
    GP_ARG(s && out);
    const AmpState& A = s->amp;
    memset(out, 0, sizeof(*out));
    out->calls = A.ct; out->accept_rate = (double)NAN; out->last_ms = A.clast_ms;
    if (A.mode != 2 || !A.cbuf) return 0;
    out->rank = s->sf.have ? s->sf.r : 0;
    const int64_t m = s->m;
    std::vector<long long> cnt(4 * (size_t)m);
    hipStream_t st = s->h->stream;
    GP_HIP(hipMemcpyAsync(cnt.data(), A.ca.counts, sizeof(long long) * 4 * (size_t)m, hipMemcpyDeviceToHost, st));
    GP_HIP(hipStreamSynchronize(st));
    for (int64_t j = 0; j < m; ++j) {
        out->updates += cnt[(size_t)j]; out->accepted += cnt[(size_t)(m + j)];
        out->same += cnt[(size_t)(2 * m + j)]; out->failed += cnt[(size_t)(3 * m + j)];
    }
    const int64_t decided = out->updates - out->same - out->failed;
    if (decided > 0) out->accept_rate = (double)out->accepted / (double)decided;
    return 0;
}

static int beta_centred_alloc(gpirt_sampler_t s)
// ... 21 lines not shown
    std::vector<double> hn, hw;
    nu_lr_nodes(hn, hw);
    hipStream_t st = s->h->stream;
    if (hipMemsetAsync(buf, 0, sizeof(double) * total, st) != hipSuccess ||
        hipMemcpyAsync(nodes, hn.data(), sizeof(double) * R, hipMemcpyHostToDevice, st) != hipSuccess ||
        hipMemcpyAsync(wts, hw.data(), sizeof(double) * R, hipMemcpyHostToDevice, st) != hipSuccess ||
        hipStreamSynchronize(st) != hipSuccess) {
        set_error("beta (centred): the upload failed");
        return GPIRT_E_HIP;
    }
    Bc.buf = buf;
    return 0;
}

int gpirt_sampler_draw_beta_centred(gpirt_sampler_t s)
{
    GP_ARG(s != nullptr);
    const char* me = "gpirt_sampler_draw_beta_centred";
    GP_TRY(ord_refuse(s, "gpirt_sampler_draw_beta_centred", "it moves the intercept, which ordinal responses pin at 0"));
    if (!s->initialised) { set_error("%s needs an initialised sampler (gpirt_sampler_init)", me); return GPIRT_E_ARG; }
    if (stream_mode(s)) { set_error("%s: rng = reference (GPIRT_RNG_RSTREAM) is refused, R's stream has no such draw", me); return GPIRT_E_ARG; }
    if (s->opt.kernel_fp32) { set_error("%s: kernel_fp32 is refused, the single-precision build is the default kernel's alone", me); return GPIRT_E_ARG; }
    if (s->opt.item0 != 0 || (s->opt.m_total > 0 && s->opt.m_total != s->m)) {
        set_error("%s: an item shard (item0 = %lld, m_total = %lld) is refused, the shared 2 x 2 matrix is built for all items of one sampler", me,
                  (long long)s->opt.item0, (long long)s->opt.m_total);
        return GPIRT_E_ARG;
    }
    if (!s->nu_kern_ok) {
        if (s->kern.family != GPIRT_KERNEL_SE) {
            set_error("%s: the handle's kernel is not a squared exponential, it has no rank-64 form (gpirt_kernel_check(kernel, 64))", me);
            return GPIRT_E_ARG;
        }
        const int rc = kernel_rank_check(s->kern, BETA_CENTRED_RANK, nullptr, nullptr);
        if (rc) return rc;
        set_error("%s: the length-scale grid's smallest value fails gpirt_kernel_check(kernel, 64)", me);
        return GPIRT_E_ARG;
    }
    if (!s->theta_ok) {
        set_error("%s: a theta is not finite or lies outside [-5, 5], the rank-64 basis does not hold there", me);
        return GPIRT_E_ARG;
    }
    BetaCentredState& Bc = s->bc;
    if (Bc.prior_ok < 0) {
        Bc.prior_ok = 1;
        const double* ps = s->host_tmp.data() + 2 * s->m;
        for (int64_t e = 0; e < 2 * s->m; ++e)
            if (!(ps[e] > 0.0) || !(ps[e] <= 1.79769313486231570815e308)) Bc.prior_ok = 0;
    }
    if (!Bc.prior_ok) {
        set_error("%s: a prior sd of beta is not finite and > 0, the conditional has no precision to add", me);
        return GPIRT_E_ARG;
    }
    GP_TRY(beta_sync(s));
    s->lp_current = false;
    s->mu_linear = false;
    GP_TRY(beta_centred_alloc(s));
    GP_TRY(smooth_factor(s));
    BetaCentredArgs a = Bc.a;
    a.f = s->f; a.beta = s->beta; a.mu = s->mu; a.mu_star = s->mu_star; a.n = s->n; a.m = s->m; a.N = s->N;
    a.theta = s->theta; a.tstar = s->tstar; a.pm = s->pm; a.ps = s->ps;
    a.amp = s->amp.mode ? s->amp.amp : nullptr;
    a.F = s->sf.F; a.eps = GPIRT_JITTER;
    a.seed = s->opt.seed; a.t = Bc.t + 1; a.item0 = (uint32_t)s->opt.item0;
    a.err = s->flags;
    hipStream_t st = s->h->stream;
    const bool timed = s->timing;
    if (timed) {
        for (hipEvent_t& t : Bc.tev) if (!t) GP_HIP(hipEventCreate(&t));
        GP_HIP(hipEventRecord(Bc.tev[0], st));
        a.kev[0] = Bc.tev[2]; a.kev[1] = Bc.tev[3];
    }
    GP_TRY(launch_beta_centred(st, a));
    Bc.t += 1;
    if (timed) {
        GP_HIP(hipEventRecord(Bc.tev[1], st));
        GP_HIP(hipEventSynchronize(Bc.tev[1]));
        float ms = 0.f;
        hipEventElapsedTime(&ms, Bc.tev[0], Bc.tev[1]);
        Bc.last_ms = ms;
        hipEventElapsedTime(&ms, Bc.tev[2], Bc.tev[3]);
        Bc.item_ms = ms;
    }
    return 0;
}

int gpirt_sampler_beta_centred_get(gpirt_sampler_t s, const char* name, void* h_out, int64_t bytes)
{
    GP_ARG(s && name && h_out);
    BetaCentredState& Bc = s->bc;
    if (strcmp(name, "time") == 0 || strcmp(name, "time_item") == 0) {
        if (bytes != 8) { set_error("beta (centred): '%s' holds 8 bytes, %lld were asked for", name, (long long)bytes); return GPIRT_E_ARG; }
        memcpy(h_out, name[4] ? &Bc.item_ms : &Bc.last_ms, 8);
        return 0;
    }
    GP_TRY(needs(Bc.buf != nullptr && Bc.t > 0, "the centred beta update's arrays are", "one gpirt_sampler_draw_beta_centred call"));
    const BetaCentredArgs& c = Bc.a;
    const int64_t n = s->n, m = s->m, R = BETA_CENTRED_RANK;
    const void* dev = nullptr;
    int64_t want = 0;
    if (strcmp(name, "W") == 0) { dev = c.W; want = 8 * 2 * n; }
    else if (strcmp(name, "B") == 0) { dev = c.B; want = 8 * 4; }
    else if (strcmp(name, "P") == 0) { dev = c.P; want = 8 * 2 * R; }
    else if (strcmp(name, "Gx") == 0) { dev = c.Gx; want = 8 * 2 * R; }
    else if (strcmp(name, "T") == 0) { dev = c.T; want = 8 * 2 * m; }
    else if (strcmp(name, "z") == 0) { dev = c.Z; want = 8 * 2 * m; }
    else if (strcmp(name, "mean") == 0) { dev = c.mean; want = 8 * 2 * m; }
    else if (strcmp(name, "beta_old") == 0) { dev = c.beta_old; want = 8 * 2 * m; }
// ... 223 lines not shown
        if (strcmp(name, "record") == 0) { dev = c.rec; want = 8 * SCALE_REC_COUNT; }
        else if (strcmp(name, "lz") == 0) { dev = c.lz; want = 8 * n; }
        else if (strcmp(name, "lz_prop") == 0) { dev = c.lz_prop; want = 8 * n; }
        else if (strcmp(name, "dlz") == 0) { dev = c.dlz; want = 8 * n; }
        else if (strcmp(name, "beta_prop") == 0) { dev = c.beta_prop; want = 8 * 2 * m; }
        else if (strcmp(name, "mu_prop") == 0) { dev = c.mu2; want = 8 * N * m; }
        else if (strcmp(name, "fstar_prop") == 0) { dev = c.fstar2; want = 8 * N * m; }
        else if (strcmp(name, "logpost_prop") == 0) { dev = c.logpost2; want = 8 * N * n; }
        else { set_error("unknown scale array '%s'", name); return GPIRT_E_ARG; }
    }
    if (bytes != want) { set_error("scale: '%s' holds %lld bytes, %lld were asked for", name, (long long)want, (long long)bytes); return GPIRT_E_ARG; }
    if (host) { memcpy(h_out, host, (size_t)want); return 0; }
    hipStream_t st = s->h->stream;
    GP_HIP(hipMemcpyAsync(h_out, dev, (size_t)want, hipMemcpyDeviceToHost, st));
    GP_HIP(hipStreamSynchronize(st));
    return 0;
}

int gpirt_sampler_scale_stats(gpirt_sampler_t s, gpirt_scale* out)
{
    GP_ARG(s && out);
    const ScaleState& Sc = s->sc;
    memset(out, 0, sizeof(*out));
    out->on = Sc.on ? 1 : 0;
    for (int k = 0; k < 2; ++k) { out->calls[k] = Sc.t[k]; out->width[k] = Sc.width[k]; out->last_ms[k] = Sc.last_ms[k]; }
    if (!Sc.on) return 0;
    long long cnt[6];
    hipStream_t st = s->h->stream;
    GP_HIP(hipMemcpyAsync(cnt, Sc.a.counts, sizeof(cnt), hipMemcpyDeviceToHost, st));
    GP_HIP(hipStreamSynchronize(st));
    for (int k = 0; k < 2; ++k) { out->accepted[k] = cnt[2 + k]; out->failed[k] = cnt[4 + k]; }
    return 0;
}

static int pop_refusals(gpirt_sampler_t s, const char* entry)
{
    if (!s->initialised) { set_error("%s needs an initialised sampler (gpirt_sampler_init)", entry); return GPIRT_E_ARG; }
    if (s->fstar_full) {
        set_error("%s is refused while gpirt_sampler_set_theta_block is in use: the block path would need the codes of its respondents", entry);
        return GPIRT_E_ARG;
    }
    if (s->opt.m_total > 0 && s->opt.m_total != s->m) {
        set_error("population prior: an item shard (item0 = %lld, m_total = %lld) is refused, the respondent-block theta path "
                  "would need the codes of its respondents", (long long)s->opt.item0, (long long)s->opt.m_total);
        return GPIRT_E_ARG;
    }
    return 0;
}

int gpirt_sampler_pop_set(gpirt_sampler_t s, const int32_t* codes, int G, const double* log_prior)
{
    GP_ARG(s != nullptr);
    PopState& A = s->pop;
    s->lp_current = false;
    s->mu_linear = false;
    if (!codes) {
        if (A.mode == 2) { set_error("gpirt_sampler_pop_set(NULL): the population prior is sampled, gpirt_sampler_pop_enable(on = 0) turns it off"); return GPIRT_E_ARG; }
        GP_HIP(hipStreamSynchronize(s->h->stream));
        pop_free(&A);
        return 0;
    }
    if (A.mode == 2) {
        set_error("gpirt_sampler_pop_set after gpirt_sampler_pop_enable: turn the sampled population prior off first (on = 0)");
        return GPIRT_E_ARG;
    }
    GP_ARG(log_prior != nullptr);
    GP_TRY(pop_refusals(s, "gpirt_sampler_pop_set"));
    const int64_t n = s->n, N = s->N;
    GP_TRY(gpirt_pop_check(codes, n, G, log_prior, G, 0, 0.0, 0, 0.0, 0.0, 0, nullptr, nullptr, nullptr, nullptr, &s->opt));
    hipStream_t st = s->h->stream;
    GP_HIP(hipStreamSynchronize(st));
    pop_free(&A);
    if (hipMalloc((void**)&A.codes, sizeof(int32_t) * (size_t)n) != hipSuccess ||
        hipMalloc((void**)&A.log_prior, sizeof(double) * (size_t)G * (size_t)N) != hipSuccess) {
        set_error("population prior: hipMalloc failed");
        pop_free(&A);
        return GPIRT_E_ALLOC;
    }
    if (hipMemcpyAsync(A.codes, codes, sizeof(int32_t) * (size_t)n, hipMemcpyHostToDevice, st) != hipSuccess ||
        hipMemcpyAsync(A.log_prior, log_prior, sizeof(double) * (size_t)G * (size_t)N, hipMemcpyHostToDevice, st) != hipSuccess ||
        hipStreamSynchronize(st) != hipSuccess) {
        set_error("population prior: the upload failed");
        pop_free(&A);
        return GPIRT_E_HIP;
    }
    A.G = G;
    A.mode = 1;
    return 0;
}

int gpirt_sampler_pop_enable(gpirt_sampler_t s, const int32_t* codes, int G, const double* anchor_row, double mu_hi, int P_mu,
                             double sd_lo, double sd_hi, int P_sd, const double* log_hyper_mu, const double* log_hyper_sd,
                             const int* a0, const int* b0, int64_t planned_draws, int on)
{
    GP_ARG(s != nullptr);
    PopState& A = s->pop;
    s->lp_current = false;
    s->mu_linear = false;
    if (!on) {
        if (A.mode == 1) { set_error("gpirt_sampler_pop_enable(on = 0): the population prior is fixed, gpirt_sampler_pop_set(NULL) turns it off"); return GPIRT_E_ARG; }
        GP_HIP(hipStreamSynchronize(s->h->stream));
        pop_free(&A);
        return 0;
    }
    if (A.mode == 1) {
        set_error("gpirt_sampler_pop_enable after gpirt_sampler_pop_set: turn the fixed population prior off first (gpirt_sampler_pop_set(NULL))");
        return GPIRT_E_ARG;
    }
    GP_ARG(codes != nullptr);
    GP_TRY(pop_refusals(s, "gpirt_sampler_pop_enable"));
    const int64_t n = s->n, N = s->N;
    GP_TRY(gpirt_pop_check(codes, n, G, anchor_row, anchor_row ? 1 : 0, 1, mu_hi, P_mu, sd_lo, sd_hi, P_sd, log_hyper_mu, log_hyper_sd,
                           a0, b0, &s->opt));
    if (planned_draws < 0 || planned_draws > (int64_t)1 << 31) {
        set_error("population prior: planned_draws = %lld, it must lie in 0 .. 2^31", (long long)planned_draws);
        return GPIRT_E_ARG;
    }
    hipStream_t st = s->h->stream;
    GP_HIP(hipStreamSynchronize(st));
    pop_free(&A);
    auto fail = [&](int rc, const char* what) { set_error("population prior: %s failed", what); pop_free(&A); return rc; };
    const size_t Gs = (size_t)G, Pm = (size_t)P_mu, Ps = (size_t)P_sd;
    const size_t draw_bytes = sizeof(int32_t) * (size_t)(planned_draws ? planned_draws : 1) * 2 * Gs;
    if (hipMalloc((void**)&A.codes, sizeof(int32_t) * (size_t)n) != hipSuccess ||
        hipMalloc((void**)&A.log_prior, sizeof(double) * Gs * (size_t)N) != hipSuccess ||
        hipMalloc((void**)&A.d_mu, sizeof(double) * Pm) != hipSuccess ||
        hipMalloc((void**)&A.d_sd, sizeof(double) * Ps) != hipSuccess ||
        hipMalloc((void**)&A.d_lse, sizeof(double) * Pm * Ps) != hipSuccess ||
        hipMalloc((void**)&A.d_hyper_mu, sizeof(double) * Pm) != hipSuccess ||
        hipMalloc((void**)&A.d_hyper_sd, sizeof(double) * Ps) != hipSuccess ||
        hipMalloc((void**)&A.lp_mu, sizeof(double) * Gs * Pm) != hipSuccess ||
        hipMalloc((void**)&A.lp_sd, sizeof(double) * Gs * Ps) != hipSuccess ||
        hipMalloc((void**)&A.idx, sizeof(int) * 2 * Gs) != hipSuccess ||
        hipMalloc((void**)&A.stats, sizeof(long long) * 4 * Gs) != hipSuccess ||
        hipMalloc((void**)&A.counts, sizeof(long long) * 4 * Gs) != hipSuccess ||
        hipMalloc((void**)&A.hist_mu, sizeof(uint32_t) * Pm * Gs) != hipSuccess ||
        hipMalloc((void**)&A.hist_sd, sizeof(uint32_t) * Ps * Gs) != hipSuccess ||
        hipMalloc((void**)&A.draws, draw_bytes) != hipSuccess) return fail(GPIRT_E_ALLOC, "hipMalloc");
    A.G = G; A.P_mu = P_mu; A.P_sd = P_sd; A.planned = planned_draws; A.recorded = 0;
    A.mu_hi = mu_hi; A.sd_lo = sd_lo; A.sd_hi = sd_hi;
    A.mu.resize(Pm); A.sd.resize(Ps); A.lse.resize(Pm * Ps);
    A.hyper_mu.assign(Pm, 0.0); A.hyper_sd.assign(Ps, 0.0);
    pop_grids_fill(mu_hi, P_mu, sd_lo, sd_hi, P_sd, A.mu.data(), A.sd.data());
    pop_lse_fill(A.mu.data(), P_mu, A.sd.data(), P_sd, A.lse.data());
    if (log_hyper_mu) A.hyper_mu.assign(log_hyper_mu, log_hyper_mu + Pm);
    if (log_hyper_sd) A.hyper_sd.assign(log_hyper_sd, log_hyper_sd + Ps);
    const int near1 = amp_nearest_one(A.sd.data(), P_sd);
    std::vector<int> idx(2 * Gs, -1);
    std::vector<double> table(Gs * (size_t)N);
    if (anchor_row) memcpy(table.data(), anchor_row, sizeof(double) * (size_t)N);
    else pop_default_row(table.data());
    for (int g = 1; g < G; ++g) {
        const int a = a0 ? a0[g] : (P_mu - 1) / 2, b = b0 ? b0[g] : near1;
        idx[2 * (size_t)g] = a; idx[2 * (size_t)g + 1] = b;
        pop_normal_row(A.mu[(size_t)a], A.sd[(size_t)b], table.data() + (size_t)g * (size_t)N);
    }
    if (hipMemcpyAsync(A.codes, codes, sizeof(int32_t) * (size_t)n, hipMemcpyHostToDevice, st) != hipSuccess ||
        hipMemcpyAsync(A.log_prior, table.data(), sizeof(double) * Gs * (size_t)N, hipMemcpyHostToDevice, st) != hipSuccess ||
        hipMemcpyAsync(A.d_mu, A.mu.data(), sizeof(double) * Pm, hipMemcpyHostToDevice, st) != hipSuccess ||
        hipMemcpyAsync(A.d_sd, A.sd.data(), sizeof(double) * Ps, hipMemcpyHostToDevice, st) != hipSuccess ||
        hipMemcpyAsync(A.d_lse, A.lse.data(), sizeof(double) * Pm * Ps, hipMemcpyHostToDevice, st) != hipSuccess ||
        hipMemcpyAsync(A.d_hyper_mu, A.hyper_mu.data(), sizeof(double) * Pm, hipMemcpyHostToDevice, st) != hipSuccess ||
        hipMemcpyAsync(A.d_hyper_sd, A.hyper_sd.data(), sizeof(double) * Ps, hipMemcpyHostToDevice, st) != hipSuccess ||
        hipMemcpyAsync(A.idx, idx.data(), sizeof(int) * 2 * Gs, hipMemcpyHostToDevice, st) != hipSuccess ||
        hipMemsetAsync(A.lp_mu, 0, sizeof(double) * Gs * Pm, st) != hipSuccess ||
        hipMemsetAsync(A.lp_sd, 0, sizeof(double) * Gs * Ps, st) != hipSuccess ||
        hipMemsetAsync(A.stats, 0, sizeof(long long) * 4 * Gs, st) != hipSuccess ||
        hipMemsetAsync(A.counts, 0, sizeof(long long) * 4 * Gs, st) != hipSuccess ||
        hipMemsetAsync(A.hist_mu, 0, sizeof(uint32_t) * Pm * Gs, st) != hipSuccess ||
        hipMemsetAsync(A.hist_sd, 0, sizeof(uint32_t) * Ps * Gs, st) != hipSuccess ||
        hipMemsetAsync(A.draws, 0, draw_bytes, st) != hipSuccess ||
        hipStreamSynchronize(st) != hipSuccess) return fail(GPIRT_E_HIP, "the upload");
    A.mode = 2;
    return 0;
}

int gpirt_sampler_draw_pop(gpirt_sampler_t s)
{
    GP_ARG(s && s->initialised);
    PopState& A = s->pop;
    GP_TRY(needs(A.mode == 2, "the population prior's update is", "gpirt_sampler_pop_enable"));
    s->lp_current = false;
    s->mu_linear = false;
    PopUpdateArgs a{};
    a.stats = A.stats; a.mu = A.d_mu; a.sd = A.d_sd; a.P_mu = A.P_mu; a.P_sd = A.P_sd;
    a.hyper_mu = A.d_hyper_mu; a.hyper_sd = A.d_hyper_sd; a.lse = A.d_lse;
    a.idx = A.idx; a.lp_mu = A.lp_mu; a.lp_sd = A.lp_sd; a.log_prior = A.log_prior; a.counts = A.counts;
    a.G = A.G; a.N = (int)s->N; a.seed = s->opt.seed; a.t = A.t + 1;
    hipStream_t st = s->h->stream;
    const bool timed = s->timing;
    if (timed) {
        for (hipEvent_t& t : A.tev) if (!t) GP_HIP(hipEventCreate(&t));
        GP_HIP(hipEventRecord(A.tev[0], st));
    }
    GP_TRY(launch_pop_stats(st, s->theta, A.codes, s->n, A.G, A.stats));
    GP_TRY(launch_pop_update(st, a));
    A.t += 1;
    if (timed) {
        GP_HIP(hipEventRecord(A.tev[1], st));
        GP_HIP(hipEventSynchronize(A.tev[1]));
        float ms = 0.f;
        hipEventElapsedTime(&ms, A.tev[0], A.tev[1]);
        A.last_ms = ms;
    }
    return 0;
}

int gpirt_sampler_pop_record(gpirt_sampler_t s)
{
    GP_ARG(s != nullptr);
    PopState& A = s->pop;
    GP_TRY(needs(A.mode == 2, "the population prior's update is", "gpirt_sampler_pop_enable"));
    if (A.recorded >= A.planned) {
        set_error("population prior: all %lld planned draws are recorded", (long long)A.planned);
        return GPIRT_E_ARG;
    }
    GP_TRY(launch_pop_record(s->h->stream, A.idx, A.G, A.P_mu, A.P_sd, A.recorded, A.hist_mu, A.hist_sd, A.draws));
    A.recorded += 1;
    return 0;
}

int gpirt_sampler_pop_get(gpirt_sampler_t s, const char* name, void* h_out, int64_t bytes)
{
    GP_ARG(s && name && h_out && bytes >= 0);
    PopState& A = s->pop;
    GP_TRY(needs(A.mode != 0, "a population prior is", "gpirt_sampler_pop_set, gpirt_sampler_pop_enable"));
    const int64_t n = s->n, N = s->N, G = A.G, Pm = A.P_mu, Ps = A.P_sd;
    const void* host = nullptr; const void* dev = nullptr; int64_t want = 0;
    const bool both = strcmp(name, "codes") == 0 || strcmp(name, "log_prior") == 0;
    if (!both) GP_TRY(needs(A.mode == 2, "the population prior's update is", "gpirt_sampler_pop_enable"));
    if (strcmp(name, "codes") == 0) { dev = A.codes; want = 4 * n; }
    else if (strcmp(name, "log_prior") == 0) { dev = A.log_prior; want = 8 * G * N; }
    else if (strcmp(name, "mu_grid") == 0) { host = A.mu.data(); want = 8 * Pm; }
    else if (strcmp(name, "sd_grid") == 0) { host = A.sd.data(); want = 8 * Ps; }
    else if (strcmp(name, "lse") == 0) { host = A.lse.data(); want = 8 * Pm * Ps; }
    else if (strcmp(name, "log_hyper_mu") == 0) { host = A.hyper_mu.data(); want = 8 * Pm; }
    else if (strcmp(name, "log_hyper_sd") == 0) { host = A.hyper_sd.data(); want = 8 * Ps; }
    else if (strcmp(name, "index") == 0) { dev = A.idx; want = 8 * G; }
    else if (strcmp(name, "stats") == 0) { dev = A.stats; want = 24 * G; }
    else if (strcmp(name, "off_grid") == 0) { dev = A.stats + 3 * G; want = 8 * G; }
    else if (strcmp(name, "lp_mu") == 0) { dev = A.lp_mu; want = 8 * G * Pm; }
    else if (strcmp(name, "lp_sd") == 0) { dev = A.lp_sd; want = 8 * G * Ps; }
    else if (strcmp(name, "counts") == 0) { dev = A.counts; want = 32 * G; }
    else if (strcmp(name, "hist_mu") == 0) { dev = A.hist_mu; want = 4 * Pm * G; }
    else if (strcmp(name, "hist_sd") == 0) { dev = A.hist_sd; want = 4 * Ps * G; }
    else if (strcmp(name, "draws") == 0) { dev = A.draws; want = 8 * A.recorded * G; }
    else if (strcmp(name, "time") == 0) { host = &A.last_ms; want = 8; }
    else { set_error("unknown population-prior array '%s'", name); return GPIRT_E_ARG; }
    if (bytes != want) { set_error("population prior: '%s' holds %lld bytes, %lld were asked for", name, (long long)want, (long long)bytes); return GPIRT_E_ARG; }
    if (want == 0) return 0;
    if (host) { memcpy(h_out, host, (size_t)want); return 0; }
    GP_HIP(hipMemcpyAsync(h_out, dev, (size_t)want, hipMemcpyDeviceToHost, s->h->stream));
    GP_HIP(hipStreamSynchronize(s->h->stream));
    return 0;
}

int gpirt_sampler_pop_stats(gpirt_sampler_t s, gpirt_pop* out)
{
    GP_ARG(s && out);
    const PopState& A = s->pop;
    memset(out, 0, sizeof(*out));
    out->on = A.mode; out->groups = A.G; out->n = s->n; out->calls = A.t;
    out->mu_hi = out->sd_lo = out->sd_hi = (double)NAN;
    if (A.mode != 2) return 0;
    const size_t G = (size_t)A.G;
    std::vector<long long> cnt(4 * G), stats(4 * G);
    hipStream_t st = s->h->stream;
    GP_HIP(hipMemcpyAsync(cnt.data(), A.counts, sizeof(long long) * 4 * G, hipMemcpyDeviceToHost, st));
    GP_HIP(hipMemcpyAsync(stats.data(), A.stats, sizeof(long long) * 4 * G, hipMemcpyDeviceToHost, st));
    GP_HIP(hipStreamSynchronize(st));
    out->points_mu = A.P_mu; out->points_sd = A.P_sd; out->planned_draws = A.planned; out->recorded = A.recorded;
    out->mu_hi = A.mu_hi; out->sd_lo = A.sd_lo; out->sd_hi = A.sd_hi; out->last_ms = A.last_ms;
    for (size_t g = 0; g < G; ++g) {
        out->updates += cnt[g]; out->updated += cnt[G + g]; out->skipped += cnt[2 * G + g]; out->failed += cnt[3 * G + g];
        out->off_grid += stats[3 * G + g];
    }
    return 0;
}

int gpirt_sampler_ordinal_enable(gpirt_sampler_t s, const int8_t* cat, int C, double hi, int P, const double* log_prior,
                                 const int32_t* K0, int W, int64_t planned_draws)
{
    GP_ARG(s != nullptr);
    OrdState& A = s->ord;
    const char* me = "gpirt_sampler_ordinal_enable";
    if (!cat) {
        GP_HIP(hipStreamSynchronize(s->h->stream));
        s->lp_current = false;
        ord_free(&A);
        return 0;
    }
    if (!s->initialised) { set_error("%s needs an initialised sampler (gpirt_sampler_init)", me); return GPIRT_E_ARG; }
    if (s->fstar_full) {
        set_error("%s is refused while gpirt_sampler_set_theta_block is in use: the respondent-block theta path has no one-hot product", me);
        return GPIRT_E_ARG;
    }
    if (s->opt.m_total > 0 && s->opt.m_total != s->m) {
        set_error("ordinal: an item shard (item0 = %lld, m_total = %lld) is refused, the respondent-block theta path has no one-hot product",
                  (long long)s->opt.item0, (long long)s->opt.m_total);
        return GPIRT_E_ARG;
    }
    if (s->h->cfg.ll_exact == 1) {
        set_error("%s is refused under GPIRT_LL_EXACT=1: the ordinal kernels have the fast term alone", me);
        return GPIRT_E_ARG;
    }
    const char* blk = nullptr;
    if (s->sum.parts & (GPIRT_SUM_PRED | GPIRT_SUM_WAIC)) blk = "the summaries' WAIC / pred parts (gpirt_sampler_summary_enable)";
    else if (s->ppc.on) blk = "the posterior predictive checks (gpirt_sampler_ppc_enable)";
    else if (s->loo.on) blk = "PSIS-LOO (gpirt_sampler_loo_enable)";
    else if (s->score.on) blk = "scoring (gpirt_sampler_score_enable)";
    else if (s->sumscore.on) blk = "the sum-score posteriors (gpirt_sampler_sumscore_enable)";
    else if (s->equate.on) blk = "the score equating (gpirt_sampler_equate_enable)";
    else if (s->groups.on) blk = "the group posteriors (gpirt_sampler_groups_enable)";
    else if (s->acf.on && (s->acf.parts & GPIRT_ACF_LL)) blk = "the ACF's log-likelihood series (gpirt_sampler_acf_enable)";
    if (blk) { set_error("%s is refused while %s are on: they evaluate the binary likelihood of y", me, blk); return GPIRT_E_ARG; }
    const int64_t n = s->n, m = s->m, N = s->N, Np = (N + 127) / 128 * 128;
    if (planned_draws < 0 || planned_draws > (int64_t)1 << 31) {
        set_error("ordinal: planned_draws = %lld, it must lie in 0 .. 2^31", (long long)planned_draws);
        return GPIRT_E_ARG;
    }
    hipStream_t st = s->h->stream;
    GP_TRY(beta_sync(s));
    std::vector<double> hy((size_t)(n * m));
    GP_HIP(hipMemcpyAsync(hy.data(), s->y, sizeof(double) * (size_t)(n * m), hipMemcpyDeviceToHost, st));
    GP_HIP(hipStreamSynchronize(st));
    GP_TRY(gpirt_ordinal_check(cat, hy.data(), n, m, C, hi, P, log_prior, K0, W, &s->opt));
    s->lp_current = false;
    ord_free(&A);
    auto fail = [&](int rc, const char* what) { set_error("ordinal: %s failed", what); ord_free(&A); return rc; };
    const size_t rows = (size_t)m * (size_t)(C - 1), Ps = (size_t)P;
    const size_t draw_bytes = sizeof(int32_t) * (size_t)(planned_draws ? planned_draws : 1) * rows;
    if (hipMalloc((void**)&A.cat, (size_t)(n * m)) != hipSuccess ||
        hipMalloc((void**)&A.d_grid, sizeof(double) * Ps) != hipSuccess ||
        hipMalloc((void**)&A.d_log_prior, sizeof(double) * Ps) != hipSuccess ||
        hipMalloc((void**)&A.thr, sizeof(double) * rows) != hipSuccess ||
        hipMalloc((void**)&A.lp, sizeof(double) * rows * GPIRT_ORD_MAX_WIDTH) != hipSuccess ||
        hipMalloc((void**)&A.cum, sizeof(double) * rows * (size_t)N) != hipSuccess ||
        hipMalloc((void**)&A.Y, sizeof(double) * (size_t)n * (size_t)C * (size_t)m) != hipSuccess ||
        hipMalloc((void**)&A.G, sizeof(double) * ((size_t)Np * (size_t)C * (size_t)m + 2)) != hipSuccess ||
        hipMalloc((void**)&A.idx, sizeof(int) * rows) != hipSuccess ||
        hipMalloc((void**)&A.window, sizeof(int) * rows) != hipSuccess ||
        hipMalloc((void**)&A.counts, sizeof(long long) * (size_t)m * (size_t)C) != hipSuccess ||
        hipMalloc((void**)&A.stat, sizeof(long long) * 4) != hipSuccess ||
        hipMalloc((void**)&A.hist, sizeof(uint32_t) * rows * Ps) != hipSuccess ||
        hipMalloc((void**)&A.draws, draw_bytes) != hipSuccess) return fail(GPIRT_E_ALLOC, "hipMalloc");
    A.C = C; A.P = P; A.W = W; A.lp_W = W; A.hi = hi; A.planned = planned_draws; A.recorded = 0; A.irf_draws = 0;
    A.grid.resize(Ps); A.log_prior.resize(Ps);
    ord_grid_fill(hi, P, A.grid.data());
    for (int k = 0; k < P; ++k) A.log_prior[(size_t)k] = log_prior ? log_prior[k] : -(A.grid[(size_t)k] * A.grid[(size_t)k]) / 18.0;
    std::vector<int> idx(rows);
    std::vector<double> thr(rows);
    for (int64_t j = 0; j < m; ++j)
        for (int c = 1; c < C; ++c) {
            const size_t r = (size_t)j * (size_t)(C - 1) + (size_t)(c - 1);
            idx[r] = K0 ? K0[r] : (2 * (P - 1) * c + C) / (2 * C);
            thr[r] = A.grid[(size_t)idx[r]];
        }
    if (hipMemcpyAsync(A.cat, cat, (size_t)(n * m), hipMemcpyHostToDevice, st) != hipSuccess ||
        hipMemcpyAsync(A.d_grid, A.grid.data(), sizeof(double) * Ps, hipMemcpyHostToDevice, st) != hipSuccess ||
        hipMemcpyAsync(A.d_log_prior, A.log_prior.data(), sizeof(double) * Ps, hipMemcpyHostToDevice, st) != hipSuccess ||
        hipMemcpyAsync(A.idx, idx.data(), sizeof(int) * rows, hipMemcpyHostToDevice, st) != hipSuccess ||
        hipMemcpyAsync(A.thr, thr.data(), sizeof(double) * rows, hipMemcpyHostToDevice, st) != hipSuccess ||
        hipMemsetAsync(A.lp, 0, sizeof(double) * rows * GPIRT_ORD_MAX_WIDTH, st) != hipSuccess ||
        hipMemsetAsync(A.cum, 0, sizeof(double) * rows * (size_t)N, st) != hipSuccess ||
        hipMemsetAsync(A.G, 0, sizeof(double) * ((size_t)Np * (size_t)C * (size_t)m + 2), st) != hipSuccess ||
        hipMemsetAsync(A.window, 0, sizeof(int) * rows, st) != hipSuccess ||
        hipMemsetAsync(A.stat, 0, sizeof(long long) * 4, st) != hipSuccess ||
        hipMemsetAsync(A.hist, 0, sizeof(uint32_t) * rows * Ps, st) != hipSuccess ||
        hipMemsetAsync(A.draws, 0, draw_bytes, st) != hipSuccess) return fail(GPIRT_E_HIP, "the upload");
    if (launch_ord_indicators(st, A.cat, n, m, C, A.Y) != 0 || launch_ord_counts(st, A.cat, n, m, C, A.counts) != 0)
        return fail(GPIRT_E_HIP, "the indicator launch");
    std::vector<double> hb((size_t)(2 * m));
    if (hipMemcpyAsync(hb.data(), s->beta, sizeof(double) * (size_t)(2 * m), hipMemcpyDeviceToHost, st) != hipSuccess ||
        hipStreamSynchronize(st) != hipSuccess) return fail(GPIRT_E_HIP, "reading beta");
    for (int64_t j = 0; j < m; ++j) hb[(size_t)(2 * j)] = 0.0;
    if (hipMemcpyAsync(s->beta, hb.data(), sizeof(double) * (size_t)(2 * m), hipMemcpyHostToDevice, st) != hipSuccess ||
        launch_linear_mean(st, s->theta, n, s->beta, m, s->mu) != 0 ||
        launch_linear_mean(st, s->tstar, N, s->beta, m, s->mu_star) != 0 ||
        hipStreamSynchronize(st) != hipSuccess) return fail(GPIRT_E_HIP, "pinning the intercept");
    A.on = true;
    return 0;
}

int gpirt_sampler_draw_thresholds(gpirt_sampler_t s)
{
    GP_ARG(s && s->initialised);
    OrdState& A = s->ord;
    GP_TRY(needs(A.on, "ordinal responses are", "gpirt_sampler_ordinal_enable"));
    GP_TRY(beta_sync(s));
    s->lp_current = false;
    OrdThrArgs a{};
    a.f = s->f; a.mu = s->mu; a.cat = A.cat; a.counts = A.counts; a.n = s->n; a.m = s->m;
    a.grid = A.d_grid; a.log_prior = A.d_log_prior; a.C = A.C; a.P = A.P; a.W = A.W;
    a.idx = A.idx; a.thr = A.thr; a.lp = A.lp; a.window = A.window; a.stat = A.stat;
    a.seed = s->opt.seed; a.t = A.t + 1; a.item0 = (uint32_t)s->opt.item0;
    hipStream_t st = s->h->stream;
    const bool timed = s->timing;
    if (timed) {
        for (hipEvent_t& t : A.tev) if (!t) GP_HIP(hipEventCreate(&t));
        GP_HIP(hipEventRecord(A.tev[0], st));
    }
    GP_TRY(launch_ord_thresholds(st, a));
    A.t += 1;
    A.lp_W = A.W;
    if (timed) {
        GP_HIP(hipEventRecord(A.tev[1], st));
        GP_HIP(hipEventSynchronize(A.tev[1]));
        float ms = 0.f;
        hipEventElapsedTime(&ms, A.tev[0], A.tev[1]);
        A.last_ms = ms;
    }
    return 0;
}

int gpirt_sampler_ordinal_width(gpirt_sampler_t s, int W)
{
    GP_ARG(s != nullptr);
    GP_TRY(needs(s->ord.on, "ordinal responses are", "gpirt_sampler_ordinal_enable"));
    if (W < 1 || W > GPIRT_ORD_MAX_WIDTH) { set_error("ordinal: window width W = %d, it must lie in 1 .. %d", W, GPIRT_ORD_MAX_WIDTH); return GPIRT_E_ARG; }
    s->ord.W = W;
    return 0;
}

int gpirt_sampler_ordinal_record(gpirt_sampler_t s)
{
    GP_ARG(s != nullptr);
    OrdState& A = s->ord;
    GP_TRY(needs(A.on, "ordinal responses are", "gpirt_sampler_ordinal_enable"));
    if (A.recorded >= A.planned) { set_error("ordinal: all %lld planned draws are recorded", (long long)A.planned); return GPIRT_E_ARG; }
    GP_TRY(launch_ord_record(s->h->stream, A.idx, s->m, A.C, A.P, A.recorded, A.hist, A.draws));
    A.recorded += 1;
    return 0;
}

int gpirt_sampler_ordinal_accumulate_irf(gpirt_sampler_t s)
{
    GP_ARG(s && s->initialised);
    OrdState& A = s->ord;
    GP_TRY(needs(A.on, "ordinal responses are", "gpirt_sampler_ordinal_enable"));
    GP_TRY(launch_ord_irf(s->h->stream, s->fstar, s->N, s->m, A.C, A.thr, A.cum));
    A.irf_draws += 1;
    return 0;
}
// ... 211 lines not shown

int gpirt_sampler_check(gpirt_sampler_t s)
{
    GP_ARG(s != nullptr);
    gpirt_handle_t h = s->h;
    hipStream_t st = h->stream;
    GP_TRY(aux_join(s));
    GP_HIP(hipMemcpyAsync(h->h_info, h->d_info, 8 * sizeof(int), hipMemcpyDeviceToHost, st));
    GP_HIP(hipMemcpyAsync(s->h_flags, s->flags, 2 * sizeof(int), hipMemcpyDeviceToHost, st));
    GP_HIP(hipStreamSynchronize(st));
    if (h->h_info[1] != 0) {
        if (!s->factor_fresh || h->cfg.panel == 2) return report_panel_guard(h, h->h_info, st);
        GP_TRY(recover_factor(s));
        GP_HIP(hipMemcpyAsync(h->h_info, h->d_info, 8 * sizeof(int), hipMemcpyDeviceToHost, st));
        GP_HIP(hipStreamSynchronize(st));
        if (h->h_info[1] != 0) return report_panel_guard(h, h->h_info, st);
    }
    if (*h->h_info > 0) {
        set_error("chol(): decomposition failed (leading minor of order %d is not positive definite)", *h->h_info);
        return *h->h_info;
    }
    if (s->h_flags[0] != 0) {
        set_error("sampler state is not finite (flag %d): elliptical slice sampler did not terminate or the R stream window overflowed", s->h_flags[0]);
        return s->h_flags[0];
    }
    if (s->h_flags[1] != 0) return report_degenerate_theta(s, s->h_flags[1]);
    return 0;
}

static int lookup(gpirt_sampler_t s, const char* name, void** p, int64_t* count)
{
    const int64_t n = s->n, m = s->m, N = s->N;
    struct E { const char* k; void* p; int64_t c; } tab[] = {
        { "theta", s->theta, n }, { "f", s->f, n * m }, { "beta", s->beta, 2 * m }, { "mu", s->mu, n * m },
        { "mu_star", s->mu_star, N * m }, { "fstar", s->fstar, N * m }, { "L", s->L, n * n },
        { "logpost", s->logpost, N * n }, { "irf_sum", s->irf_sum, N * m }, { "ess_k", s->ess_k, m },
        { "s", s->s, N }, { "mean", s->mean, N * m }, { "nu", s->NU, n * m }, { "z", s->Z, n * m },
        { "y", s->y, n * m }, { "rs_trace", s->rs_trace, s->rs_trace ? 128 : 0 },
        { "rs_stats", s->rs_ctl, s->rs_ctl ? 8 : 0 },
        { "fstar_full", s->fstar_full, s->fstar_full ? N * s->blk_m : 0 }, { "theta_stage", s->theta_stage, s->theta_stage ? n : 0 },
        { "gbar", s->shape.gbar, s->shape.on ? N * m : 0 },
    };
    for (auto& e : tab)
        if (strcmp(e.k, name) == 0) { *p = e.p; *count = e.c; return 0; }
    set_error("unknown sampler array '%s'", name);
    return GPIRT_E_ARG;
}

int gpirt_sampler_devptr(gpirt_sampler_t s, const char* name, void** d_ptr, int64_t* count)
{
    GP_ARG(s && name && d_ptr && count);
    GP_TRY(lookup(s, name, d_ptr, count));
    if (strcmp(name, "theta") == 0 || strcmp(name, "beta") == 0 || strcmp(name, "mu") == 0) s->mu_linear = false;
    if (strcmp(name, "y") == 0) s->ess_ypk_valid = false;
    if (strcmp(name, "L") == 0) {
        *count = s->ldl * s->n;
        GP_TRY(ensure_dense_factor(s));
    }
    return 0;
}

int gpirt_sampler_ldl(gpirt_sampler_t s, int64_t* ldl)
{
    GP_ARG(s && ldl);
    *ldl = s->ldl;
    return 0;
}

int gpirt_sampler_panel_factor(gpirt_sampler_t s, int64_t p)
{
    GP_ARG(s && s->initialised);
    GP_TRY(ensure_dense_factor(s));
    return potrf_panel_factor(s->h, s->h->stream, s->L, s->n, s->ldl, p, s->ext);
}

int gpirt_sampler_panel_update(gpirt_sampler_t s, int64_t p, int64_t c)
{
    GP_ARG(s && s->initialised);
    GP_TRY(ensure_dense_factor(s));
    return potrf_panel_update(s->h, s->h->stream, s->L, s->n, s->ldl, p, c, s->ext);
}

int gpirt_sampler_panel_copy(gpirt_sampler_t s, int64_t p, double* d_buf, int to_buf)
{
    GP_ARG(s && s->initialised && d_buf);
    GP_TRY(ensure_dense_factor(s));
    return potrf_panel_copy(s->h->stream, s->L, s->n, s->ldl, p, d_buf, to_buf != 0, s->ext);
}

int gpirt_sampler_panel_rows(gpirt_sampler_t s, int64_t* rows)
{
    GP_ARG(s && rows);
    *rows = s->n + s->ext;
    return 0;
}

int gpirt_sampler_ess_pack_draws(gpirt_sampler_t s, int64_t* draws)
{
    GP_ARG(s && draws);
    *draws = s->ess_pack_draws;
    return 0;
}

int gpirt_sampler_nu_lr_draws(gpirt_sampler_t s, int64_t* draws)
{
    GP_ARG(s && draws);
    *draws = s->nu_lr_draws;
    return 0;
}

int gpirt_sampler_fstar_free_draws(gpirt_sampler_t s, int64_t* draws)
{
    GP_ARG(s && draws);
    *draws = s->fstar_free_draws;
    return 0;
}

int gpirt_sampler_factor_lr_count(gpirt_sampler_t s, int64_t* count)
{
    GP_ARG(s && count);
    *count = s->factor_lr_count;
    return 0;
}

int gpirt_sampler_dense_factor_count(gpirt_sampler_t s, int64_t* count)
{
    GP_ARG(s && count);
    *count = s->dense_factor_count;
    return 0;
}

int gpirt_sampler_dense_factor(gpirt_sampler_t s)
{
    GP_ARG(s && s->initialised);
    return ensure_dense_factor(s);
}

int gpirt_sampler_factor_lr_parts(gpirt_sampler_t s, double* h_out, int64_t count)
{
    GP_ARG(s && h_out && count == (int64_t)NU_LR_PART * s->n);
    GP_TRY(aux_join(s));
    GP_TRY(ensure_factor_width(s, NU_LR_PART));
    memset(h_out, 0, sizeof(double) * (size_t)count);
    for (int64_t p = 0; p < s->n; p += NU_LR_PART) {
        const int64_t w = s->n - p < NU_LR_PART ? s->n - p : NU_LR_PART;
        GP_HIP(hipMemcpy2DAsync(h_out + p * NU_LR_PART, (size_t)NU_LR_PART * 8, s->L + p * (s->ldl + 1), (size_t)s->ldl * 8, (size_t)w * 8, (size_t)w,
                                hipMemcpyDeviceToHost, s->h->stream));
    }
    GP_HIP(hipStreamSynchronize(s->h->stream));
    return 0;
}

int gpirt_sampler_factor_lr_width(gpirt_sampler_t s, int* width)
// ... 29 lines not shown
    GP_HIP(hipStreamSynchronize(s->h->stream));
    return 0;
}

int gpirt_sampler_panel_factor_part(gpirt_sampler_t s, int64_t p, int half)
{
    GP_ARG(s && s->initialised);
    GP_TRY(ensure_dense_factor(s));
    return potrf_panel_factor(s->h, s->h->stream, s->L, s->n, s->ldl, p, s->ext, half);
}

int gpirt_sampler_panel_update_part(gpirt_sampler_t s, int64_t p, int64_t c, int part)
{
    GP_ARG(s && s->initialised);
    GP_TRY(ensure_dense_factor(s));
    return potrf_panel_update(s->h, s->h->stream, s->L, s->n, s->ldl, p, c, s->ext, part);
}

int gpirt_sampler_panel_copy_part(gpirt_sampler_t s, int64_t p, int half, double* d_buf, int64_t buf_doubles, int to_buf)
{
    GP_ARG(s && s->initialised && d_buf && buf_doubles >= 0);
    GP_TRY(ensure_dense_factor(s));
    return potrf_panel_copy(s->h->stream, s->L, s->n, s->ldl, p, d_buf, to_buf != 0, s->ext, half, buf_doubles);
}

int gpirt_sampler_copy_state(gpirt_sampler_t dst, gpirt_sampler_t src)
{
    GP_ARG(dst && src && dst->initialised && src->initialised && dst->n == src->n && dst->m == src->m && dst->h == src->h);
    if (dst->ord.on || src->ord.on) {
        set_error("gpirt_sampler_copy_state is refused while ordinal responses are on: the categories, thresholds and records are not copied");
        return GPIRT_E_ARG;
    }
    if (dst->ell.on || src->ell.on) {
        set_error("gpirt_sampler_copy_state is not defined while the length-scale update is on (the index and its tables are not copied)");
        return GPIRT_E_ARG;
    }
    if (dst->amp.mode || src->amp.mode) {
        set_error("gpirt_sampler_copy_state is not defined while per-item amplitudes are on (they are not copied)");
        return GPIRT_E_ARG;
    }
    if (dst->pop.mode || src->pop.mode) {
        set_error("gpirt_sampler_copy_state is not defined while a population prior is on (it is not copied)");
        return GPIRT_E_ARG;
    }
    if (dst->kern.family != src->kern.family || dst->kern.length_scale != src->kern.length_scale) {
        set_error("gpirt_sampler_copy_state: the samplers' kernels differ (length_scale %g and %g)", dst->kern.length_scale, src->kern.length_scale);
        return GPIRT_E_ARG;
    }
    hipStream_t st = dst->h->stream;
    const int64_t n = dst->n, m = dst->m, N = dst->N;
    GP_TRY(aux_join(dst)); GP_TRY(aux_join(src));
    GP_TRY(ensure_dense_factor(src));
    dst->L_structured = false;
    dst->lp_current = false;
    dst->mu_linear = false;
    src->factor_fresh = false;
    invalidate_factor_products(dst);
    GP_HIP(hipMemcpyAsync(dst->theta, src->theta, sizeof(double) * (size_t)n, hipMemcpyDeviceToDevice, st));
    GP_HIP(hipMemcpyAsync(dst->f, src->f, sizeof(double) * (size_t)(n * m), hipMemcpyDeviceToDevice, st));
    GP_HIP(hipMemcpyAsync(dst->beta, src->beta, sizeof(double) * (size_t)(2 * m), hipMemcpyDeviceToDevice, st));
    GP_HIP(hipMemcpyAsync(dst->mu, src->mu, sizeof(double) * (size_t)(n * m), hipMemcpyDeviceToDevice, st));
    GP_HIP(hipMemcpyAsync(dst->mu_star, src->mu_star, sizeof(double) * (size_t)(N * m), hipMemcpyDeviceToDevice, st));
    GP_HIP(hipMemcpyAsync(dst->fstar, src->fstar, sizeof(double) * (size_t)(N * m), hipMemcpyDeviceToDevice, st));
    GP_HIP(hipMemcpy2DAsync(dst->L, (size_t)dst->ldl * 8, src->L, (size_t)src->ldl * 8, (size_t)n * 8, (size_t)n,
                            hipMemcpyDeviceToDevice, st));
    dst->rows_valid = false;
    dst->theta_ok = src->theta_ok; dst->theta_alone = src->theta_alone;
    GP_TRY(rebuild_rows(dst));
    dst->iter = src->iter;
    return 0;
}

int gpirt_sampler_get(gpirt_sampler_t s, const char* name, double* h_out, int64_t count)
{
    GP_ARG(s && name && h_out);
    void* p; int64_t c;
    GP_TRY(lookup(s, name, &p, &c));
    GP_ARG(count <= c);
    const size_t esz = strcmp(name, "ess_k") == 0 ? sizeof(int) : sizeof(double);
    GP_TRY(aux_join(s));
    if (strcmp(name, "L") == 0) GP_TRY(ensure_dense_factor(s));
    if (strcmp(name, "L") == 0 && s->ldl != s->n) {
        GP_ARG(count == s->n * s->n);
        GP_HIP(hipMemcpy2DAsync(h_out, (size_t)s->n * 8, p, (size_t)s->ldl * 8, (size_t)s->n * 8, (size_t)s->n,
                                hipMemcpyDeviceToHost, s->h->stream));
    } else {
        GP_HIP(hipMemcpyAsync(h_out, p, esz * (size_t)count, hipMemcpyDeviceToHost, s->h->stream));
    }
    GP_HIP(hipStreamSynchronize(s->h->stream));
    return 0;
}

int gpirt_sampler_set(gpirt_sampler_t s, const char* name, const double* h_in, int64_t count)
{
    GP_ARG(s && name && h_in);
    void* p; int64_t c;
    GP_TRY(lookup(s, name, &p, &c));
    GP_ARG(count <= c && strcmp(name, "ess_k") != 0);
    if (s->ord.on && strcmp(name, "y") == 0)
        GP_TRY(ord_refuse(s, "gpirt_sampler_set(\"y\")", "the categories were checked against y's missing cells at enable"));
    if (s->ord.on && strcmp(name, "beta") == 0)
        for (int64_t q = 0; q < count; q += 2)
            if (h_in[q] != 0.0) GP_TRY(ord_refuse(s, "gpirt_sampler_set(\"beta\") with a non-zero intercept", "the intercept is pinned at 0"));
    GP_TRY(aux_join(s));
    invalidate_factor_products(s);
    s->lp_current = false;
    if (strcmp(name, "theta") == 0 || strcmp(name, "beta") == 0 || strcmp(name, "mu") == 0) s->mu_linear = false;
    if (strcmp(name, "y") == 0) s->ess_ypk_valid = false;
    if (strcmp(name, "L") == 0 || strcmp(name, "theta") == 0) s->rows_valid = false;
    if (strcmp(name, "L") == 0) s->theta_alone = false;
    if (strcmp(name, "L") == 0) {
        if (count < c) GP_TRY(ensure_dense_factor(s));
        s->L_structured = false;
    }
    if (strcmp(name, "theta") == 0) {
        s->theta_alone = true;
        s->theta_ok = count == s->n;
        for (int64_t i = 0; i < count; ++i) s->theta_ok = s->theta_ok && h_in[i] >= -5.0 && h_in[i] <= 5.0;
    }
    if (strcmp(name, "L") == 0 && s->ldl != s->n) {
        GP_ARG(count == s->n * s->n);
        GP_HIP(hipMemcpy2DAsync(p, (size_t)s->ldl * 8, h_in, (size_t)s->n * 8, (size_t)s->n * 8, (size_t)s->n,
                                hipMemcpyHostToDevice, s->h->stream));
    } else {
        GP_HIP(hipMemcpyAsync(p, h_in, sizeof(double) * (size_t)count, hipMemcpyHostToDevice, s->h->stream));
    }
    GP_HIP(hipStreamSynchronize(s->h->stream));
    return 0;
}

int gpirt_sampler_finish_irfs(gpirt_sampler_t s, int sample_iterations, double* h_irfs)
{
    GP_ARG(s && h_irfs);
    const int64_t cnt = s->N * s->m;
    GP_HIP(hipMemcpyAsync(h_irfs, s->irf_sum, sizeof(double) * (size_t)cnt, hipMemcpyDeviceToHost, s->h->stream));
    GP_HIP(hipStreamSynchronize(s->h->stream));
    const double inv = 1.0 / (double)sample_iterations;
    for (int64_t i = 0; i < cnt; ++i) h_irfs[i] = 1.0 / (1.0 + exp(-(h_irfs[i] * inv)));
    return 0;
}

int gpirt_sampler_enable_timing(gpirt_sampler_t s, int on)
{
    GP_ARG(s != nullptr);
    s->timing = on != 0;
    return 0;
}

int gpirt_sampler_stage_times(gpirt_sampler_t s, double* ms_out, int max_stages, int* n_stages,
                              const char** names_out)
{
    GP_ARG(s && ms_out && n_stages);
    static const char names[] = "draw_f\0draw_fstar\0theta_gemm\0theta_sample\0draw_beta\0factor\0";
    const int k = max_stages < ST_COUNT ? max_stages : ST_COUNT;
    for (int i = 0; i < k; ++i) ms_out[i] = s->stage_ms[i];
    *n_stages = k;
    if (names_out) *names_out = names;
    (void)kStageNames;
    return 0;
// ... 174 lines not shown
        return v;
    };
    auto save_ckpt = [&](int k) -> int {
        const int q = k % NS;
        hipStream_t st = h->stream;
        if (beta_sync(s) != 0) return fail_hip("draw_beta join");
        if (copy_pending[q] && hipStreamWaitEvent(st, ev_copied[q], 0) != hipSuccess) return fail_hip("hipStreamWaitEvent");
        double* d = ck[q];
        for (const Part& pt : parts()) {
            if (hipMemcpyAsync(d, pt.p, pt.cnt * sizeof(double), hipMemcpyDeviceToDevice, st) != hipSuccess) return fail_hip("checkpoint");
            d += even(pt.cnt);
        }
        if (hipMemcpyAsync(h_poll + 16 * q, h->d_info, 8 * sizeof(int), hipMemcpyDeviceToHost, st) != hipSuccess ||
            hipMemcpyAsync(h_poll + 16 * q + 8, s->flags, 2 * sizeof(int), hipMemcpyDeviceToHost, st) != hipSuccess ||
            hipEventRecord(ev_flags[q], st) != hipSuccess)
            return fail_hip("flag read-back");
        return 0;
    };
    auto finish_store = [&](int q) -> int {
        if (!copy_pending[q]) return 0;
        if (hipEventSynchronize(ev_copied[q]) != hipSuccess) return fail_hip("draw copy");
        const int slot = copy_slot[q];
        if (h_theta_draws)
            for (int64_t i = 0; i < n; ++i) h_theta_draws[slot + i * (int64_t)(S_it + 1)] = th_stage[q][(size_t)i];
        copy_pending[q] = false;
        return 0;
    };
    auto start_store = [&](int k) -> int {
        const int q = k % NS, slot = k - B_it;
        GP_TRY(finish_store(q));
        const double* d = ck[q];
        GP_TRY(accumulate_run(s, DrawView{ d, d + off_beta, d + off_f, d + off_mu, d + off_fstar, d + off_gbar, (uint32_t)k }));
        if (!h_theta_draws && !h_beta_draws && !h_f_draws) return 0;
        if ((h_theta_draws && hipMemcpyAsync(th_stage[q].data(), d, sizeof(double) * (size_t)n, hipMemcpyDeviceToHost, copy_stream) != hipSuccess) ||
            (h_beta_draws && hipMemcpyAsync(h_beta_draws + (int64_t)slot * 2 * m, d + off_beta, sizeof(double) * (size_t)(2 * m), hipMemcpyDeviceToHost, copy_stream) != hipSuccess) ||
            (h_f_draws && hipMemcpyAsync(h_f_draws + (int64_t)slot * n * m, d + off_f, sizeof(double) * (size_t)(n * m), hipMemcpyDeviceToHost, copy_stream) != hipSuccess) ||
            hipEventRecord(ev_copied[q], copy_stream) != hipSuccess)
            return fail_hip("draw copy");
        copy_pending[q] = true; copy_slot[q] = slot;
        return 0;
    };
    auto rollback = [&](int k) -> int {
        hipStream_t st = h->stream;
        if (hipStreamSynchronize(st) != hipSuccess) return fail_hip("hipStreamSynchronize");
        if (h->side) hipStreamSynchronize(h->side);
        if (s->haux) hipStreamSynchronize(s->haux->stream);
        s->beta_deferred = false; s->beta_pending = false; s->prep_pending = false; s->z_filled_iter = 0;
        const double* d = ck[k % NS];
        for (const Part& pt : parts()) {
            if (hipMemcpyAsync(pt.p, d, pt.cnt * sizeof(double), hipMemcpyDeviceToDevice, st) != hipSuccess) return fail_hip("rollback");
            d += even(pt.cnt);
        }
        if (hipMemsetAsync(s->flags, 0, 4 * sizeof(int), st) != hipSuccess) return fail_hip("rollback");
        s->mu_linear = false;
        s->iter = k;
        return recover_factor(s);
    };
    s->sticky_info = true;
    const int panel_mode = h->cfg.panel;
    int it = 0, verified = 0, fallback_until = 0, last_fallback = -1;
    if (!rc) rc = save_ckpt(0);
    if (!rc && hipEventSynchronize(ev_flags[0]) != hipSuccess) rc = fail_hip("hipEventSynchronize");
    while (!rc && verified < total) {
        if (it < total && verified >= it - 1) {
            if (ticked(it, total)) { set_error("interrupted"); rc = GPIRT_E_INTERRUPT; break; }
            h->cfg.panel = (it < fallback_until) ? 2 : panel_mode;
            if (h->aux) h->aux->cfg.panel = h->cfg.panel;
            rc = gpirt_sampler_step(s);
            h->cfg.panel = panel_mode;
            if (h->aux) h->aux->cfg.panel = panel_mode;
            if (!rc && it >= B_it) rc = gpirt_sampler_accumulate_irf(s);
            if (!rc) rc = save_ckpt(it + 1);
            ++it;
            continue;
        }
        const int k = verified + 1, q = k % NS;
        if (hipEventSynchronize(ev_flags[q]) != hipSuccess) { rc = fail_hip("hipEventSynchronize"); break; }
        const int* w = h_poll + 16 * q;
        if (w[1] != 0) {
            if (panel_mode == 2 || last_fallback == verified) { rc = report_panel_guard(h, w, h->stream); break; }
            rc = rollback(verified);
            last_fallback = verified; fallback_until = it; it = verified;
            continue;
        }
        if (w[0] > 0) {
            set_error("chol(): decomposition failed (leading minor of order %d is not positive definite)", w[0]);
            rc = w[0];
        } else if (w[8] != 0) {
            set_error("sampler state is not finite (flag %d)", w[8]); rc = w[8];
        } else if (w[9] != 0) {
            rc = report_degenerate_theta(s, w[9]);
        } else {
            verified = k;
            if (k > B_it) rc = start_store(k);
        }
    }
    for (int q = 0; q < NS; ++q) { const int r2 = finish_store(q); if (!rc) rc = r2; }
    if (rc != GPIRT_E_INTERRUPT) {
        const int rc2 = gpirt_sampler_check(s);
        if (!rc) rc = rc2;
    }
    if (copy_stream) { hipStreamSynchronize(copy_stream); hipStreamDestroy(copy_stream); }
    for (int q = 0; q < NS; ++q) {
        if (ck[q]) hipFree(ck[q]);
        if (ev_flags[q]) hipEventDestroy(ev_flags[q]);
        if (ev_copied[q]) hipEventDestroy(ev_copied[q]);
    }
// ... 291 lines not shown
```

### gpirt_amd/csrc/stages.hip

```cpp
#include "common.h"
#include "kernels.h"
#include "ll_fast.h"

namespace gpirt {

namespace {

#define GP_LN_SQRT_2PI 0.918938533204672741780329736406

__device__ __forceinline__ double r_rnorm(double mu, double sd, double z, bool& consumes)
{
    consumes = false;
    if (mu != mu || !isfinite(sd) || sd < 0.0) return __builtin_nan("");
    if (sd == 0.0 || !isfinite(mu)) return mu;
    consumes = true;
    return mu + sd * z;
}

__device__ __forceinline__ double r_dnorm_log(double x, double mu, double sd)
{
    const double z = fabs((x - mu) / sd);
    return -(GP_LN_SQRT_2PI + 0.5 * z * z + log(sd));
}

// ... 22 lines not shown
        t *= sv[k];
    }
    red[k] = t;
    __syncthreads();
    for (int w = 64; w > 0; w >>= 1) {
        if (k < w) red[k] += red[k + w];
        __syncthreads();
    }
    if (k == 0) s[j] = 1.0 - sqrt(fmax(red[0], 0.0));
}

__global__ __launch_bounds__(256) void fstar_offsets_kernel(const double* __restrict__ s, int N, int* __restrict__ off)
{
    __shared__ int cnt[256];
    const int tid = threadIdx.x;
    const int per = (N + 255) / 256;
    const int i0 = tid * per, i1 = (i0 + per < N) ? i0 + per : N;
    int c = 0;
    for (int i = i0; i < i1; ++i) { const double v = s[i]; c += (isfinite(v) && v > 0.0) ? 1 : 0; }
    cnt[tid] = c;
    __syncthreads();
    if (tid == 0) {
        int run = 0;
        for (int q = 0; q < 256; ++q) { const int t = cnt[q]; cnt[q] = run; run += t; }
        off[N] = run;
    }
    __syncthreads();
    c = cnt[tid];
    for (int i = i0; i < i1; ++i) {
        off[i] = c;
        const double v = s[i];
        if (isfinite(v) && v > 0.0) ++c;
    }
}

__global__ __launch_bounds__(256) void fstar_epilogue_kernel(FstarEpiArgs a, const int* __restrict__ off)
{
    const int64_t j = blockIdx.y;
    const int64_t i = (int64_t)blockIdx.x * 256 + threadIdx.x;
    if (i >= a.N) return;
    const double mean = a.mean[i + j * a.N] + a.mu_star[i + j * a.N];
    const double sd = a.amp ? a.amp[j] * a.s[i] : a.s[i];
    double z;
    if (a.U) {
        const uint64_t q = *a.pos + 2ull * ((uint64_t)j * (uint64_t)off[a.N] + (uint64_t)off[i]);
        if (q + 1 >= a.cap) { if (a.err) atomicCAS(a.err, 0, (int)GPIRT_E_RNG); z = 0.0; }
        else z = rnorm_from_two(a.U[q], a.U[q + 1]);
    } else {
        z = qnorm_as241(item_uniform(a.seed, a.iter, GPIRT_ST_FSTAR, a.item0 + (uint32_t)j, (uint32_t)i));
    }
    bool consumes;
    a.out[i + j * a.N] = r_rnorm(mean, sd, z, consumes);
    if (a.mean_out) a.mean_out[i + j * a.N] = mean;
}

__global__ void fstar_advance_kernel(uint64_t* pos, const int* off, int N, int64_t m)
{
    *pos += 2ull * (uint64_t)off[N] * (uint64_t)m;
}

__global__ void indicators_kernel(const double* __restrict__ y, int64_t total, double* __restrict__ Ypm)
{
    for (int64_t g = (int64_t)blockIdx.x * blockDim.x + threadIdx.x; g < total;
         g += (int64_t)gridDim.x * blockDim.x) {
        const double v = y[g];
        Ypm[g] = (v == 1.0) ? 1.0 : 0.0;
        Ypm[g + total] = (v == -1.0) ? 1.0 : 0.0;
    }
}

__global__ void loglik_terms_kernel(const double* __restrict__ fstar, int64_t N, int64_t m, double* __restrict__ Gpm,
                                    int64_t ldg, const int* __restrict__ run_if)
{
    if (run_if != nullptr && *run_if == 0) return;
    const int64_t total = N * m;
    for (int64_t g = (int64_t)blockIdx.x * blockDim.x + threadIdx.x; g < total;
         g += (int64_t)gridDim.x * blockDim.x) {
        const double v = fstar[g];
        const int64_t o = (g % N) + (g / N) * ldg;
        double gp = -ll_term(1.0 * v), gm = -ll_term(-1.0 * v);
        if (gp == -INFINITY) gp = -1e300;
        if (gm == -INFINITY) gm = -1e300;
        Gpm[o] = gp;
        Gpm[o + ldg * m] = gm;
    }
}

__global__ void theta_nan_fix_kernel(const double* __restrict__ Gpm, int64_t ldg, const double* __restrict__ Ypm, int64_t n,
                                     int64_t m, double* __restrict__ lp, int64_t N, int64_t ldlp, const int* __restrict__ run_if)
{
    if (run_if != nullptr && *run_if == 0) return;
    const int64_t total = N * n;
    for (int64_t g = (int64_t)blockIdx.x * blockDim.x + threadIdx.x; g < total;
         g += (int64_t)gridDim.x * blockDim.x) {
        const int64_t k = g % N, i = g / N;
        double* out = lp + k + i * ldlp;
        if (*out == *out) continue;
        double acc = 0.0;
        for (int64_t j = 0; j < m; ++j) {
            if (Ypm[i + j * n] != 0.0) acc += Gpm[k + j * ldg];
            if (Ypm[i + (m + j) * n] != 0.0) acc += Gpm[k + (m + j) * ldg];
        }
        *out = acc;
    }
}

// ... 294 lines not shown
        mu[g] = beta[0 + 2 * j] + x[i] * beta[1 + 2 * j];
    }
}

__global__ void axpy_kernel(double* __restrict__ acc, const double* __restrict__ x, int64_t count)
{
    for (int64_t g = (int64_t)blockIdx.x * blockDim.x + threadIdx.x; g < count;
         g += (int64_t)gridDim.x * blockDim.x)
        acc[g] += x[g];
}

inline unsigned grid_for(int64_t total)
{
    int64_t b = (total + 255) / 256;
    if (b > 8192) b = 8192;
    if (b < 1) b = 1;
    return (unsigned)b;
}

}

int launch_colnorm_s(hipStream_t stream, const double* tmp, int64_t n, int64_t N, int64_t ld, double* s)
{
    if (N <= 0) return 0;
    hipLaunchKernelGGL(colnorm_s_kernel, dim3((unsigned)N), dim3(256), 0, stream, tmp, n, ld, s);
    GP_HIP(hipGetLastError());
    return 0;
}

int launch_lowrank_s(hipStream_t stream, const double* V, int64_t N, int r, const double* G, int64_t ldg, double* s)
{
    if (N <= 0) return 0;
    hipLaunchKernelGGL(lowrank_s_kernel, dim3((unsigned)N), dim3(128), 0, stream, V, N, r, G, ldg, s);
    GP_HIP(hipGetLastError());
    return 0;
}

int launch_fstar_epilogue(hipStream_t stream, const FstarEpiArgs& a)
{
    if (a.N <= 0 || a.m <= 0) return 0;
    const int* off = nullptr;
    if (a.U) {
        if (!a.off_scratch) { set_error("R-stream fstar replay needs the offset scratch (N + 1 ints)"); return GPIRT_E_ARG; }
        hipLaunchKernelGGL(fstar_offsets_kernel, dim3(1), dim3(256), 0, stream, a.s, (int)a.N, a.off_scratch);
        off = a.off_scratch;
    }
    dim3 grid((unsigned)((a.N + 255) / 256), (unsigned)a.m);
    hipLaunchKernelGGL(fstar_epilogue_kernel, grid, dim3(256), 0, stream, a, off);
    if (a.U) hipLaunchKernelGGL(fstar_advance_kernel, dim3(1), dim3(1), 0, stream, a.pos, off, (int)a.N, a.m);
    GP_HIP(hipGetLastError());
    return 0;
}

int launch_indicators(hipStream_t stream, const double* y, int64_t n, int64_t m, double* Ypm)
{
    hipLaunchKernelGGL(indicators_kernel, dim3(grid_for(n * m)), dim3(256), 0, stream, y, n * m, Ypm);
    GP_HIP(hipGetLastError());
    return 0;
}

int launch_loglik_terms(hipStream_t stream, const double* fstar, int64_t N, int64_t m, double* Gpm, int64_t ldg, const int* run_if)
{
    const unsigned blocks = run_if ? (grid_for(N * m) < 256u ? grid_for(N * m) : 256u) : grid_for(N * m);
    hipLaunchKernelGGL(loglik_terms_kernel, dim3(blocks), dim3(256), 0, stream, fstar, N, m, Gpm, ldg, run_if);
    GP_HIP(hipGetLastError());
    return 0;
}

int launch_theta_nan_fix(hipStream_t stream, const double* Gpm, int64_t ldg, const double* Ypm, int64_t n, int64_t m,
                         double* lp, int64_t N, int64_t ldlp, const int* run_if)
{
    if (N * n <= 0) return 0;
    const unsigned blocks = run_if ? (grid_for(N * n) < 256u ? grid_for(N * n) : 256u) : grid_for(N * n);
    hipLaunchKernelGGL(theta_nan_fix_kernel, dim3(blocks), dim3(256), 0, stream, Gpm, ldg, Ypm, n, m, lp, N, ldlp, run_if);
    GP_HIP(hipGetLastError());
    return 0;
}

int launch_theta_sample(hipStream_t stream, const ThetaArgs& a)
{
    if (a.n <= 0) return 0;
    if (a.N > 1024) { set_error("theta grid larger than 1024 points is not supported"); return GPIRT_E_ARG; }
    if (a.log_prior && a.codes) hipLaunchKernelGGL(theta_sample_kernel<true>, dim3((unsigned)a.n), dim3(256), 0, stream, a);
    else hipLaunchKernelGGL(theta_sample_kernel<false>, dim3((unsigned)a.n), dim3(256), 0, stream, a);
    GP_HIP(hipGetLastError());
    return 0;
}

int launch_draw_beta(hipStream_t stream, const BetaArgs& a)
{
    if (a.m <= 0) return 0;
    const bool reg = a.screen == 1 && a.U == nullptr && a.n >= 1 && a.n <= 256 * 32;
    if (reg && a.n <= 256 * 8) hipLaunchKernelGGL(draw_beta_reg_kernel<8>, dim3((unsigned)a.m), dim3(256), 0, stream, a);
    else if (reg && a.n <= 256 * 16) hipLaunchKernelGGL(draw_beta_reg_kernel<16>, dim3((unsigned)a.m), dim3(256), 0, stream, a);
    else if (reg) hipLaunchKernelGGL(draw_beta_reg_kernel<32>, dim3((unsigned)a.m), dim3(256), 0, stream, a);
    else hipLaunchKernelGGL(draw_beta_kernel, dim3((unsigned)a.m), dim3(256), 0, stream, a);
    GP_HIP(hipGetLastError());
    return 0;
}

int launch_linear_mean(hipStream_t stream, const double* x, int64_t n, const double* beta, int64_t m, double* mu)
{
    if (n * m <= 0) return 0;
    hipLaunchKernelGGL(linear_mean_kernel, dim3(grid_for(n * m)), dim3(256), 0, stream, x, n, beta, m, mu);
    GP_HIP(hipGetLastError());
    return 0;
// ... 40 lines not shown
```

### gpirt_amd/csrc/theta_fixed.hip

```cpp
#include "kernels.h"

namespace gpirt {
namespace {

typedef int v4i __attribute__((ext_vector_type(4)));
typedef int v16i __attribute__((ext_vector_type(16)));

constexpr int TF_BITS = 54;
constexpr int TF_DIGITS = 7;
constexpr int TF_KS = 4;
constexpr int TF_STAGE = TF_DIGITS * TF_KS * 1024;
constexpr int TF_TRACE_WGS = 1024;
static_assert((TF_DIGITS * TF_KS) % 4 == 0 && TF_KS % 2 == 0, "the pieces of a stage are dealt to four waves in whole rounds");
static_assert(2 * TF_STAGE <= 64 * 1024, "two stages in the static LDS allowance");

__device__ __forceinline__ uint32_t pack4(int b0, int b1, int b2, int b3)
{
    return (uint32_t)(b0 & 255) | ((uint32_t)(b1 & 255) << 8) | ((uint32_t)(b2 & 255) << 16) | ((uint32_t)(b3 & 255) << 24);
}

__device__ __forceinline__ bool tf_column(int64_t k, int64_t m, int64_t mp, int64_t* j, double* sign)
{
    if (k < mp) { *j = k; *sign = 1.0; return k < m; }
    if (k < 2 * mp) { *j = k - mp; *sign = -1.0; return k - mp < m; }
    return false;
}

__global__ __launch_bounds__(256) void tf_y8_kernel(const double* __restrict__ y, int64_t n, int64_t ldy, int64_t m, TfDims d,
                                                    uint4* __restrict__ Y8)
{
    const int64_t total = d.iblocks * d.ksteps * 64;
    for (int64_t t = (int64_t)blockIdx.x * 256 + threadIdx.x; t < total; t += (int64_t)gridDim.x * 256) {
        const int lane = (int)(t & 63);
        const int64_t ks = (t >> 6) % d.ksteps, ib = (t >> 6) / d.ksteps;
        const int64_t i = ib * 32 + (lane & 31);
        int b[16];
#pragma unroll
        for (int q = 0; q < 16; ++q) {
            int64_t j; double sign;
            const bool real = tf_column(ks * 32 + 16 * (lane >> 5) + q, m, d.mp, &j, &sign);
            b[q] = (real && i < n && y[i + j * ldy] == sign) ? 1 : 0;
        }
        Y8[t] = make_uint4(pack4(b[0], b[1], b[2], b[3]), pack4(b[4], b[5], b[6], b[7]), pack4(b[8], b[9], b[10], b[11]),
                           pack4(b[12], b[13], b[14], b[15]));
    }
}

__global__ __launch_bounds__(256) void tf_rowmax_kernel(const double* __restrict__ fstar, int64_t N, int64_t m,
                                                        unsigned long long* __restrict__ amax)
{
    const int64_t g = (int64_t)blockIdx.x * 256 + threadIdx.x;
    if (g >= N) return;
    const int64_t j0 = (int64_t)blockIdx.y * 16, j1 = (j0 + 16 < m) ? j0 + 16 : m;
    unsigned long long best = 0;
    for (int64_t j = j0; j < j1; ++j) {
        const unsigned long long bits = (unsigned long long)__double_as_longlong(fabs(fstar[g + j * N]));
        best = bits > best ? bits : best;
    }
    atomicMax(amax + g, best);
}

__global__ __launch_bounds__(256) void tf_quant_kernel(const double* __restrict__ fstar, int64_t N, int64_t m, TfDims d,
                                                       const unsigned long long* __restrict__ amax, uint4* __restrict__ Gq,
                                                       double* __restrict__ scale, int* __restrict__ ovf)
{
    const int64_t g = (int64_t)blockIdx.x * 256 + threadIdx.x;
    const int64_t kg = blockIdx.y;
    if (g >= d.gblocks * 32) return;
    const int64_t ks = kg >> 1;
    const int lane = (int)(g & 31) + 32 * (int)(kg & 1);
    const int64_t piece = ((g >> 5) * d.ksteps + ks) * 64 + lane;
    const int64_t plane = d.gblocks * d.ksteps * 64;
    int64_t q[16];
#pragma unroll
    for (int t = 0; t < 16; ++t) q[t] = 0;
    if (g < N) {
        const double fmax = __longlong_as_double((long long)amax[g]);
        const bool ok = fmax <= 709.0;
        if (!ok) { if (kg == 0) atomicOr(ovf, 1); }
        const int e = ok ? ilogb(fmax + 0.6931471805599453) + 1 : 0;
        if (kg == 0) scale[g] = ok ? ldexp(1.0, e - TF_BITS) : 0.0;
        if (ok) {
#pragma unroll
            for (int t = 0; t < 16; ++t) {
                int64_t j; double sign;
                if (tf_column(kg * 16 + t, m, d.mp, &j, &sign)) {
                    const double term = ll_term(sign * fstar[g + j * N]);
                    q[t] = (int64_t)rint(ldexp(term, TF_BITS - e));
                }
            }
        }
    }
#pragma unroll
    for (int s = 0; s < TF_DIGITS; ++s) {
        int b[16];
#pragma unroll
        for (int t = 0; t < 16; ++t) {
            const int dg = (s + 1 < TF_DIGITS) ? (int)(int8_t)(q[t] & 255) : (int)q[t];
            b[t] = dg;
            q[t] = (q[t] - dg) >> 8;
        }
        Gq[(int64_t)s * plane + piece] = make_uint4(pack4(b[0], b[1], b[2], b[3]), pack4(b[4], b[5], b[6], b[7]),
                                                    pack4(b[8], b[9], b[10], b[11]), pack4(b[12], b[13], b[14], b[15]));
    }
}

struct TfMfmaArgs {
    const unsigned char* Y8; const unsigned char* Gq; const double* scale; const int* ovf;
    double* logpost; int64_t ldlp; int64_t n, N; int64_t ksteps, gblocks; int itiles;
    long long* trace;
};

template <int P>
__device__ __forceinline__ void tf_chunk(const TfMfmaArgs& a, unsigned char* lds, int c, int nchunks, int lane, int wave,
                                         const unsigned char* srcA0, const unsigned char* srcA1, const unsigned char* srcB,
                                         v4i (&ya)[2][TF_KS][2], v4i (&fb)[2][TF_DIGITS], v16i (&acc)[2][TF_DIGITS])
{
    constexpr int KS = TF_KS;
    static_assert(KS == 4, "the schedule below is written out for four k-steps");
    constexpr int NP = (TF_DIGITS * KS) / 4;
    const int64_t ksteps = a.ksteps;
// ... 112 lines not shown
        tf_chunk<1>(a, tf_lds, c + 1, nchunks, lane, wave, srcA0, srcA1, srcB, ya, fb, acc);
    }
    if (tr) { tr[2] = (long long)__builtin_amdgcn_s_memtime(); tr[3] = (long long)__builtin_amdgcn_s_memrealtime(); }

    const int64_t g = (int64_t)gb * 32 + (lane & 31);
    const double sc = g < a.N ? a.scale[g] : 0.0;
#pragma unroll
    for (int r = 0; r < 2; ++r) {
        if (g >= a.N) break;
        const int64_t i0 = (int64_t)it * 256 + (2 * wave + r) * 32 + 4 * (lane >> 5);
#pragma unroll
        for (int v = 0; v < 16; ++v) {
            const int64_t i = i0 + (v & 3) + 8 * (v >> 2);
            if (i >= a.n) continue;
            const int64_t hi = (((int64_t)acc[r][6][v] * 256 + acc[r][5][v]) * 256 + acc[r][4][v]) * 256 + acc[r][3][v];
            const int64_t lo = ((int64_t)acc[r][2][v] * 256 + acc[r][1][v]) * 256 + acc[r][0][v];
            a.logpost[g + i * a.ldlp] = -(((double)hi * 16777216.0 + (double)lo) * sc);
        }
    }
    if (tr) { tr[4] = (long long)__builtin_amdgcn_s_memtime(); tr[5] = (long long)__builtin_amdgcn_s_memrealtime(); }
}

}

TfDims tf_dims(int64_t n, int64_t m, int64_t N)
{
    TfDims d;
    d.mp = (m + 15) / 16 * 16;
    const int64_t steps = (2 * d.mp + 31) / 32;
    d.ksteps = (steps + 2 * TF_KS - 1) / (2 * TF_KS) * (2 * TF_KS);
    if (d.ksteps == 0) d.ksteps = 2 * TF_KS;
    d.iblocks = (n + 255) / 256 * 8;
    d.gblocks = (N + 31) / 32;
    return d;
}
size_t tf_y8_bytes(const TfDims& d) { return (size_t)d.iblocks * d.ksteps * 1024; }
size_t tf_gq_bytes(const TfDims& d) { return (size_t)TF_DIGITS * d.gblocks * d.ksteps * 1024; }
size_t tf_aux_bytes(const TfDims& d) { return (size_t)d.gblocks * 32 * 16 + 16 + (size_t)TF_TRACE_WGS * 6 * 8; }
long long* tf_trace(void* aux, const TfDims& d) { return reinterpret_cast<long long*>(reinterpret_cast<unsigned char*>(aux) + (size_t)d.gblocks * 32 * 16 + 16); }
int tf_trace_wgs() { return TF_TRACE_WGS; }

int launch_tf_indicators(hipStream_t stream, const double* y, int64_t n, int64_t ldy, int64_t m, const TfDims& d, void* Y8)
{
    const int64_t total = d.iblocks * d.ksteps * 64;
    if (total <= 0) return 0;
    int64_t blocks = (total + 255) / 256;
    if (blocks > 16384) blocks = 16384;
    hipLaunchKernelGGL(tf_y8_kernel, dim3((unsigned)blocks), dim3(256), 0, stream, y, n, ldy, m, d, reinterpret_cast<uint4*>(Y8));
    GP_HIP(hipGetLastError());
    return 0;
}

int launch_theta_fixed(hipStream_t stream, const double* fstar, int64_t N, int64_t n, int64_t m, const TfDims& d,
                       const void* Y8, void* Gq, void* aux, double* logpost, int64_t ldlp, bool trace, gpirt_handle_t prof)
{
    if (n <= 0 || N <= 0) return 0;
    if (m > (1 << 20) || 2 * d.ksteps > 65535) { set_error("theta_fixed: m = %lld is beyond the fixed-point product's range (GPIRT_THETA_FIXED=2 selects the fp64 product)", (long long)m); return GPIRT_E_ARG; }
    if (d.gblocks != 32) { set_error("theta_fixed: the work-group map is laid out for the reference's 1001-point grid"); return GPIRT_E_ARG; }
    unsigned long long* amax = reinterpret_cast<unsigned long long*>(aux);
    double* scale = reinterpret_cast<double*>(amax + d.gblocks * 32);
    int* ovf = tf_overflow(aux, d);
    GP_HIP(hipMemsetAsync(aux, 0, trace ? tf_aux_bytes(d) : (size_t)d.gblocks * 32 * 16 + 16, stream));
    if (m > 0) {
        hipLaunchKernelGGL(tf_rowmax_kernel, dim3((unsigned)((N + 255) / 256), (unsigned)((m + 15) / 16)), dim3(256), 0, stream, fstar, N, m, amax);
        GP_HIP(hipGetLastError());
    }
    hipLaunchKernelGGL(tf_quant_kernel, dim3((unsigned)((d.gblocks * 32 + 255) / 256), (unsigned)(d.ksteps * 2)), dim3(256), 0, stream,
                       fstar, N, m, d, amax, reinterpret_cast<uint4*>(Gq), scale, ovf);
    GP_HIP(hipGetLastError());
    TfMfmaArgs a;
    a.Y8 = reinterpret_cast<const unsigned char*>(Y8); a.Gq = reinterpret_cast<const unsigned char*>(Gq); a.scale = scale; a.ovf = ovf;
    a.logpost = logpost; a.ldlp = ldlp; a.n = n; a.N = N; a.ksteps = d.ksteps; a.gblocks = d.gblocks; a.itiles = (int)(d.iblocks / 8);
    a.trace = trace ? tf_trace(aux, d) : nullptr;
    ProfPair pp;
    if (prof) GP_TRY(prof_pair_begin(prof, stream, pp));
    hipLaunchKernelGGL(tf_mfma_kernel, dim3((unsigned)(32 * a.itiles)), dim3(256), 2 * TF_STAGE, stream, a);
    GP_HIP(hipGetLastError());
    if (prof) GP_TRY(prof_pair_end(prof, stream, pp, 5, (double)TF_DIGITS * 2.0 * (double)N * (double)n * 2.0 * (double)m,
                                   (double)tf_y8_bytes(d) + (double)tf_gq_bytes(d) + 8.0 * (double)N * (double)n));
    return 0;
}

int* tf_overflow(void* aux, const TfDims& d) { return reinterpret_cast<int*>(reinterpret_cast<unsigned char*>(aux) + (size_t)d.gblocks * 32 * 16); }

}
```

### gpirt_amd/sampler.py

```python
from __future__ import annotations

import ctypes as C

import numpy as np

from . import _lib
from ._lib import NGRID, RNG_ITEM, RNG_RSTREAM, Options, check
from .response_matrix import as_response_matrix

_dp = C.POINTER(C.c_double)


def _f64(a):
    return np.asfortranarray(np.array(a, dtype=np.float64))


def _ptr(a):
    return a.ctypes.data_as(_dp)


def _options(rng, seed, theta_stabilise, fstar_fused, device, item0=0, m_total=0, kernel_fp32=False,
             kstar_rank=0, factor_structured=False) -> Options:
    o = _lib.default_options()
    o.rng_kind = RNG_RSTREAM if rng == "reference" else RNG_ITEM
# ... 507 lines not shown

    @property
    def torch_device(self):
        import torch
        return torch.device("cuda", self.handle.device)

    @property
    def panel_rows(self) -> int:
        r = C.c_int64()
        check(self.lib.gpirt_sampler_panel_rows(self._s, C.byref(r)))
        return r.value

    def panel_factor(self, p: int):
        check(self.lib.gpirt_sampler_panel_factor(self._s, int(p)))

    def panel_update(self, p: int, c: int):
        check(self.lib.gpirt_sampler_panel_update(self._s, int(p), int(c)))

    def panel_copy(self, p: int, buf, to_buf: bool):
        check(self.lib.gpirt_sampler_panel_copy(self._s, int(p), C.c_void_p(buf.data_ptr()), int(bool(to_buf))))

    @property
    def subpanel_width(self) -> int:
        return int(self.lib.gpirt_potrf_subpanel_width(int(self.n)))

    def panel_factor_part(self, p: int, half: int):
        check(self.lib.gpirt_sampler_panel_factor_part(self._s, int(p), int(half)))

    def panel_update_part(self, p: int, c: int, part: int):
        check(self.lib.gpirt_sampler_panel_update_part(self._s, int(p), int(c), int(part)))

    def panel_copy_part(self, p: int, half: int, buf, to_buf: bool):
        check(self.lib.gpirt_sampler_panel_copy_part(self._s, int(p), int(half), C.c_void_p(buf.data_ptr()), buf.numel(),
                                                     int(bool(to_buf))))

    def streams_busy(self) -> int:
        b = C.c_int()
        check(self.lib.gpirt_debug_streams_busy(self.handle.ptr, C.byref(b)))
        return b.value

    @property
    def nu_lr_draws(self) -> int:
        r = C.c_int64()
        check(self.lib.gpirt_sampler_nu_lr_draws(self._s, C.byref(r)))
        return r.value

    @property
    def ess_pack_draws(self) -> int:
        r = C.c_int64()
        check(self.lib.gpirt_sampler_ess_pack_draws(self._s, C.byref(r)))
        return r.value

    @property
    def fstar_free_draws(self) -> int:
        r = C.c_int64()
        check(self.lib.gpirt_sampler_fstar_free_draws(self._s, C.byref(r)))
        return r.value

    @property
    def factor_lr_count(self) -> int:
        r = C.c_int64()
        check(self.lib.gpirt_sampler_factor_lr_count(self._s, C.byref(r)))
        return int(r.value)

    @property
    def dense_factor_count(self) -> int:
        r = C.c_int64()
        check(self.lib.gpirt_sampler_dense_factor_count(self._s, C.byref(r)))
        return int(r.value)

    def dense_factor(self):
        self._call("gpirt_sampler_dense_factor")

    def factor_lr_parts(self) -> list:
        out = np.empty((self.n, 512), dtype=np.float64)
        check(self.lib.gpirt_sampler_factor_lr_parts(self._s, C.c_void_p(out.ctypes.data), out.size))
        return [out[p:p + 512, :min(512, self.n - p)].T.copy() for p in range(0, self.n, 512)]

    @property
    def factor_lr_width(self) -> int:
        r = C.c_int()
        check(self.lib.gpirt_sampler_factor_lr_width(self._s, C.byref(r)))
        return int(r.value)

    def factor_lr_blocks(self) -> list:
        W = self.factor_lr_width
        out = np.empty((self.n, max(W, 1)), dtype=np.float64)
        check(self.lib.gpirt_sampler_factor_lr_blocks(self._s, C.c_void_p(out.ctypes.data), self.n * W))
        return [out[p:p + W, :min(W, self.n - p)].T.copy() for p in range(0, self.n, W)]

    def nu_lr_rows(self) -> np.ndarray:
        out = np.empty((64, self.n), order="F")
        check(self.lib.gpirt_sampler_nu_lr_rows(self._s, C.c_void_p(out.ctypes.data), out.size))
        return out

    def copy_state_from(self, other: "Sampler"):
        check(self.lib.gpirt_sampler_copy_state(self._s, other._s))

    def accumulate_irf(self): self._call("gpirt_sampler_accumulate_irf")
    def check(self): self._call("gpirt_sampler_check")

    @property
    def iteration(self) -> int:
        it = C.c_int()
        check(self.lib.gpirt_sampler_iteration(self._s, C.byref(it)))
        return it.value
# ... 1117 lines not shown
```

### include/gpirt_hip.h

```cpp
#ifndef GPIRT_HIP_H
#define GPIRT_HIP_H

#include <stddef.h>
#include <stdint.h>

#ifdef __cplusplus
extern "C" {
#endif

#define GPIRT_NGRID 1001
#define GPIRT_JITTER 0.001

enum {
    GPIRT_OK          = 0,
    GPIRT_E_ARG       = -1,
    GPIRT_E_HIP       = -2,
    GPIRT_E_NODEVICE  = -3,
    GPIRT_E_ALLOC     = -4,
    GPIRT_E_RNG       = -5,
    GPIRT_E_INTERRUPT = -6,
    GPIRT_E_NUMERIC   = -7
};

enum { GPIRT_RNG_RSTREAM = 0, GPIRT_RNG_ITEM = 1 };
// ... 48 lines not shown
} gpirt_kernel;
void gpirt_kernel_default(gpirt_kernel* k);
int  gpirt_kernel_check(const gpirt_kernel* k, int kstar_rank, double* cert_out, int* min_rank_out);
int  gpirt_kernel_set(gpirt_handle_t h, const gpirt_kernel* k);
int  gpirt_kernel_get(gpirt_handle_t h, gpirt_kernel* k);

int gpirt_se_kernel(gpirt_handle_t h, const double* d_x1, int64_t n1, const double* d_x2,
                    int64_t n2, double* d_out, int64_t ld, double jitter);

int gpirt_potrf_lower(gpirt_handle_t h, double* d_A, int64_t n, int64_t lda);

int gpirt_factor(gpirt_handle_t h, const double* d_theta, int64_t n, double* d_L, int64_t ldl);

int64_t gpirt_potrf_panel_width(void);
int gpirt_potrf_begin(gpirt_handle_t h);
int gpirt_potrf_panel_factor(gpirt_handle_t h, double* d_A, int64_t n, int64_t lda, int64_t p);
int gpirt_potrf_panel_update(gpirt_handle_t h, double* d_A, int64_t n, int64_t lda, int64_t p, int64_t c);
int gpirt_potrf_panel_copy(gpirt_handle_t h, double* d_A, int64_t n, int64_t lda, int64_t p, double* d_buf, int to_buf);
int gpirt_potrf_finish(gpirt_handle_t h);
int64_t gpirt_potrf_subpanel_width(int64_t n);
int gpirt_potrf_panel_factor_part(gpirt_handle_t h, double* d_A, int64_t n, int64_t lda, int64_t p, int half);
int gpirt_potrf_panel_update_part(gpirt_handle_t h, double* d_A, int64_t n, int64_t lda, int64_t p, int64_t c, int part);
int gpirt_potrf_panel_copy_part(gpirt_handle_t h, double* d_A, int64_t n, int64_t lda, int64_t p, int half, double* d_buf,
                                int64_t buf_doubles, int to_buf);
int gpirt_debug_streams_busy(gpirt_handle_t h, int* busy);
int gpirt_debug_panel_trace(gpirt_handle_t h, int64_t k0, long long* host_out, int64_t count);
int gpirt_debug_ll_term(gpirt_handle_t h, const double* d_a, int64_t n, double* d_out, int fast);
int gpirt_debug_theta_logpost(gpirt_handle_t h, const double* d_y, const double* d_fstar, int64_t n, int64_t m,
                              double* d_logpost_out, int* fell_back);
int gpirt_debug_theta_clock(gpirt_handle_t h, const double* d_y, const double* d_fstar, int64_t n, int64_t m,
                            long long* host_stamps, int64_t count);

int gpirt_trmm_lz(gpirt_handle_t h, const double* d_L, int64_t n, int64_t ldl, const double* d_Z,
                  int64_t m, int64_t ldz, double* d_out, int64_t ldo);

int gpirt_trsm_lower(gpirt_handle_t h, const double* d_L, int64_t n, int64_t ldl, double* d_B,
                     int64_t nrhs, int64_t ldb, int trans);

int gpirt_gemm(gpirt_handle_t h, int ta, int tb, int64_t M, int64_t N, int64_t K, double alpha,
               const double* d_A, int64_t lda, const double* d_B, int64_t ldb, double beta,
               double* d_C, int64_t ldc);

int gpirt_ll_bar(gpirt_handle_t h, const double* d_f, const double* d_y, const double* d_mu,
                 int64_t n, int64_t m, double* d_out);

int gpirt_draw_f(gpirt_handle_t h, double* d_f, const double* d_y, const double* d_L, int64_t ldl,
                 const double* d_mu, int64_t n, int64_t m, uint64_t seed, uint32_t iter,
                 int* d_k_out);

int gpirt_draw_f_linear(gpirt_handle_t h, double* d_f, const double* d_y, const double* d_L, int64_t ldl,
                        const double* d_theta, const double* d_beta, int64_t n, int64_t m, uint64_t seed,
                        uint32_t iter, int* d_k_out);
int gpirt_sampler_ess_pack_draws(gpirt_sampler_t s, int64_t* draws);

int gpirt_draw_fstar(gpirt_handle_t h, const double* d_f, const double* d_theta, const double* d_L,
                     int64_t ldl, const double* d_mu_star, int64_t n, int64_t m, uint64_t seed,
                     uint32_t iter, int fused, double* d_out, double* d_s_out, double* d_mean_out);

int gpirt_draw_theta(gpirt_handle_t h, const double* d_y, const double* d_fstar, int64_t n,
                     int64_t m, uint64_t seed, uint32_t iter, int stabilise, double* d_theta_out,
                     int* d_degenerate);

int gpirt_draw_beta(gpirt_handle_t h, double* d_beta, const double* d_theta, const double* d_y,
                    const double* d_f, const double* d_prior_means, const double* d_prior_sds,
                    const double* d_step_sizes, int64_t n, int64_t m, uint64_t seed, uint32_t iter);
int gpirt_draw_beta_paths(gpirt_handle_t h, double* d_beta, const double* d_theta, const double* d_y,
                          const double* d_f, const double* d_prior_means, const double* d_prior_sds,
                          const double* d_step_sizes, int64_t n, int64_t m, uint64_t seed, uint32_t iter, int* d_path);

int gpirt_item_uniforms(gpirt_handle_t h, uint64_t seed, uint32_t iter, uint32_t stage,
                        uint32_t item0, int64_t n_items, int64_t n_index, double* d_out);
int gpirt_item_normals(gpirt_handle_t h, uint64_t seed, uint32_t iter, uint32_t stage,
                       uint32_t item0, int64_t n_items, int64_t n_index, double* d_out);

typedef struct gpirt_rstream_s* gpirt_rstream_t;
int gpirt_rstream_create(gpirt_rstream_t* r, uint32_t seed);
int gpirt_rstream_from_state(gpirt_rstream_t* r, const uint32_t mt[624], int mti);
int gpirt_rstream_get_state(gpirt_rstream_t r, uint32_t mt[624], int* mti);
int gpirt_rstream_destroy(gpirt_rstream_t r);
int gpirt_rstream_unif(gpirt_rstream_t r, double* h_out, int64_t n);
int gpirt_rstream_norm(gpirt_rstream_t r, double* h_out, int64_t n);

typedef int (*gpirt_tick_fn)(void* ctx, int iter, int total);

typedef struct gpirt_options {
    int      rng_kind;
    uint64_t seed;
    int      theta_stabilise;
    int      fstar_fused;
    int      device;
    int      reserved0;
    int64_t  item0;
    int64_t  m_total;
    int      reserved1;
    int      kernel_fp32;
    int      kstar_rank;
    int      reserved[4];
    int      factor_structured;
} gpirt_options;

void gpirt_default_options(gpirt_options* o);
void gpirt_fast_options(gpirt_options* o);

int gpirt_mcmc(const double* h_y, int64_t n, int64_t m, const double* h_theta0,
               int sample_iterations, int burn_iterations, const double* h_prior_means,
               const double* h_prior_sds, const double* h_step_sizes, const gpirt_options* opts,
// ... 1033 lines not shown
```

Baseline: 1237.

## Fuse rank-64 fstar mean GEMM with epilogue and per-row absmax for theta

For rank-64 non-stream f* draws, a single MFMA kernel now computes the V·Q mean product, applies the sampling epilogue and atomically records each row's absolute maximum. The next theta_fixed call can then skip its memset and row-max pass over f*, and the quantisation kernel clears the alternate double-buffered maxima for the following iteration. This removes one GEMM launch, one full read of f*, and a memset per iteration. In exchange it adds state tracking for which maxima buffer matches the current f*, which must be invalidated whenever f* changes.

```diff
diff --git a/gpirt_amd/_lib.py b/gpirt_amd/_lib.py
--- a/gpirt_amd/_lib.py
+++ b/gpirt_amd/_lib.py
@@ -726,6 +726,7 @@
     "gpirt_sampler_ldl": (_i32, [_vp, C.POINTER(_i64)]),
     "gpirt_sampler_nu_lr_draws": (_i32, [_vp, C.POINTER(_i64)]),
     "gpirt_sampler_ess_pack_draws": (_i32, [_vp, C.POINTER(_i64)]),
+    "gpirt_sampler_tail_fuse_draws": (_i32, [_vp, C.POINTER(_i64)]),
     "gpirt_sampler_nu_lr_rows": (_i32, [_vp, _vp, _i64]),
     "gpirt_sampler_fstar_free_draws": (_i32, [_vp, C.POINTER(_i64)]),
     "gpirt_sampler_factor_lr_count": (_i32, [_vp, C.POINTER(_i64)]),
diff --git a/gpirt_amd/csrc/api.hip b/gpirt_amd/csrc/api.hip
--- a/gpirt_amd/csrc/api.hip
+++ b/gpirt_amd/csrc/api.hip
@@ -44,6 +44,7 @@
         d.beta_screen = env_value("GPIRT_BETA_SCREEN", d.beta_screen);
         d.zfill_compact = env_value("GPIRT_ZFILL_COMPACT", d.zfill_compact);
         d.ess_pack = env_value("GPIRT_ESS_PACK", d.ess_pack);
+        d.tail_fuse = env_value("GPIRT_TAIL_FUSE", d.tail_fuse);
         if (d.nbo < 64) d.nbo = 1024;
         if (d.nbp != 0 && d.nbp < 64) d.nbp = 512;
         return d;
@@ -165,7 +166,7 @@
 
 extern "C" {
 
-int gpirt_version(void) { return 144; }
+int gpirt_version(void) { return 145; }
 
 const char* gpirt_last_error(void) { return g_err; }
 
@@ -295,6 +296,7 @@
         { "GPIRT_BETA_SCREEN", &h->cfg.beta_screen, false },
         { "GPIRT_ZFILL_COMPACT", &h->cfg.zfill_compact, false },
         { "GPIRT_ESS_PACK", &h->cfg.ess_pack, false },
+        { "GPIRT_TAIL_FUSE", &h->cfg.tail_fuse, false },
     };
     for (auto& e : tab)
         if (strcmp(e.k, name) == 0) { if (read_only) *read_only = e.ro; return e.p; }
diff --git a/gpirt_amd/csrc/common.h b/gpirt_amd/csrc/common.h
--- a/gpirt_amd/csrc/common.h
+++ b/gpirt_amd/csrc/common.h
@@ -48,6 +48,9 @@
     std::vector<ProfPair> pending;
     std::vector<ProfPair> free_pairs;
 };
+
+constexpr int TAIL_FUSE_TAIL = 1;
+constexpr int TAIL_FUSE_DEFAULT = TAIL_FUSE_TAIL;
 
 struct Config {
     int  nbo = 1024, nbp = 0;
@@ -70,6 +73,7 @@
     int  flr_narrow = 1;
     int  beta_screen = 1;
     int  ess_pack = 1;
+    int  tail_fuse = TAIL_FUSE_DEFAULT;
     int  zfill_compact = 1;
     int  rs_predict = 1;
     int  guard_verbose = 0;
diff --git a/gpirt_amd/csrc/kernels.h b/gpirt_amd/csrc/kernels.h
--- a/gpirt_amd/csrc/kernels.h
+++ b/gpirt_amd/csrc/kernels.h
@@ -422,6 +422,13 @@
     const double* amp;
 };
 int launch_fstar_epilogue(hipStream_t stream, const FstarEpiArgs& a);
+struct FstarTailArgs {
+    FstarEpiArgs e;
+    const double* V; const double* Q; double* mean;
+    double alpha;
+    unsigned long long* amax; int* ovf_clear;
+};
+int launch_fstar_tail(hipStream_t stream, const FstarTailArgs& a);
 
 int launch_indicators(hipStream_t stream, const double* y, int64_t n, int64_t m, double* Ypm );
 int launch_loglik_terms(hipStream_t stream, const double* fstar, int64_t N, int64_t m, double* Gpm , int64_t ldg,
@@ -437,7 +444,8 @@
 int launch_tf_indicators(hipStream_t stream, const double* y, int64_t n, int64_t ldy, int64_t m, const TfDims& d, void* Y8);
 int launch_theta_fixed(hipStream_t stream, const double* fstar, int64_t N, int64_t n, int64_t m, const TfDims& d,
                        const void* Y8, void* Gq, void* aux, double* logpost, int64_t ldlp, bool trace = false,
-                       gpirt_handle_t prof = nullptr);
+                       gpirt_handle_t prof = nullptr,
+                       const unsigned long long* amax_ready = nullptr, unsigned long long* amax_clear = nullptr);
 long long* tf_trace(void* aux, const TfDims& d);
 int tf_trace_wgs();
 struct ThetaArgs {
diff --git a/gpirt_amd/csrc/sampler.hip b/gpirt_amd/csrc/sampler.hip
--- a/gpirt_amd/csrc/sampler.hip
+++ b/gpirt_amd/csrc/sampler.hip
@@ -168,6 +168,9 @@
     int L_part_width = 0;
     hipEvent_t ev_flr = nullptr;
     int64_t factor_lr_count = 0, dense_factor_count = 0;
+    unsigned long long* amax_alt = nullptr;
+    int amax_clean = -1, amax_of_fstar = -1;
+    int64_t tail_draws = 0;
     uint32_t z_filled_iter = 0;
     hipEvent_t ev_zfill = nullptr;
     bool beta_deferred = false, beta_pending = false;
@@ -245,6 +248,8 @@
     int64_t ess_pack_draws = 0;
 };
 
+inline void logpost_inputs_written(gpirt_sampler_s* s) { s->lp_current = false; s->amax_of_fstar = -1; }
+
 namespace {
 
 template <typename T>
@@ -507,7 +512,7 @@
 
 int do_draw_f(gpirt_sampler_s* s)
 {
-    s->lp_current = false;
+    logpost_inputs_written(s);
     gpirt_handle_t h = s->h;
     hipStream_t st = h->stream;
     const int64_t n = s->n, m = s->m;
@@ -743,7 +748,7 @@
 
 int do_draw_fstar(gpirt_sampler_s* s, uint32_t iter)
 {
-    s->lp_current = false;
+    logpost_inputs_written(s);
     gpirt_handle_t h = s->h;
     hipStream_t st = h->stream;
     const int64_t n = s->n, m = s->m, N = s->N;
@@ -780,13 +785,27 @@
             GP_TRY(launch_gemm_splitk(st, true, false, r, r, n, 1.0, Bu, n, Bu, n, s->kparts, r, (int64_t)r * r, KSPLIT, G, r, 0.0));
         GP_TRY(launch_gemm_splitk(st, true, false, r, m, n, 1.0, Cu, n, s->f, n, s->kparts, r, (int64_t)r * m, KSPLIT, Q, r, 0.0));
         GP_TRY(launch_lowrank_s(st, s->kV, N, r, G, r, s->s));
-        GP_TRY(launch_gemm(h, st, false, false, TRI_NONE, N, m, r, 1.0, s->kV, N, Q, r, 0.0, s->mean, N));
         FstarEpiArgs a{};
         a.mean = s->mean; a.mu_star = s->mu_star; a.s = s->s; a.out = s->fstar; a.N = N; a.m = m;
         a.seed = s->opt.seed; a.iter = iter; a.item0 = (uint32_t)s->opt.item0; a.err = s->flags;
         if (stream_mode(s)) { a.U = s->U; a.pos = s->pos; a.cap = s->U_cap; a.off_scratch = s->fstar_off; }
         if (s->shape.on) a.mean_out = s->shape.gbar;
         if (s->amp.mode) a.amp = s->amp.amp;
+        if (r == 64 && !stream_mode(s) && (h->cfg.tail_fuse & TAIL_FUSE_TAIL)) {
+            FstarTailArgs t{};
+            t.e = a; t.V = s->kV; t.Q = Q; t.mean = s->mean; t.alpha = 1.0;
+            const int buf = (h->cfg.theta_fixed == 1 && !s->ord.on && s->tf_aux && s->amax_alt) ? s->amax_clean : -1;
+            if (buf >= 0) {
+                t.amax = buf == 0 ? reinterpret_cast<unsigned long long*>(s->tf_aux) : s->amax_alt;
+                t.ovf_clear = tf_overflow(s->tf_aux, s->tfd);
+            }
+            GP_TRY(launch_fstar_tail(st, t));
+            s->amax_of_fstar = buf;
+            if (buf >= 0) s->amax_clean = -1;
+            s->tail_draws += 1;
+            return 0;
+        }
+        GP_TRY(launch_gemm(h, st, false, false, TRI_NONE, N, m, r, 1.0, s->kV, N, Q, r, 0.0, s->mean, N));
         return launch_fstar_epilogue(st, a);
     }
     GP_HIP(hipMemcpyAsync(W, s->f, sizeof(double) * (size_t)n * m, hipMemcpyDeviceToDevice, st));
@@ -826,7 +845,13 @@
     const int64_t Np = (N + 127) / 128 * 128;
     const int* only_if = nullptr;
     if (s->h->cfg.theta_fixed == 1) {
-        GP_TRY(launch_theta_fixed(st, fstar_in, N, n, m, s->tfd, s->tf_y8, s->tf_gq, s->tf_aux, logpost_out, N, false, s->h));
+        unsigned long long* bufs[2] = { reinterpret_cast<unsigned long long*>(s->tf_aux), s->amax_alt };
+        const int have = (fstar_in == s->fstar && (s->h->cfg.tail_fuse & TAIL_FUSE_TAIL) && m > 0) ? s->amax_of_fstar : -1;
+        const int clear = have >= 0 ? 1 - have : 1;
+        GP_TRY(launch_theta_fixed(st, fstar_in, N, n, m, s->tfd, s->tf_y8, s->tf_gq, s->tf_aux, logpost_out, N, false, s->h,
+                                  have >= 0 ? bufs[have] : nullptr, bufs[clear]));
+        if (have < 0) s->amax_of_fstar = -1;
+        s->amax_clean = clear;
         only_if = tf_overflow(s->tf_aux, s->tfd);
     }
     GP_TRY(launch_loglik_terms(st, fstar_in, N, m, s->Gpm, Np, only_if));
@@ -868,7 +893,7 @@
     if (s->pop.mode) { a.log_prior = s->pop.log_prior; a.codes = s->pop.codes; }
     GP_TRY(launch_theta_sample(st, a));
     if (stream_mode(s)) GP_TRY(launch_advance_pos(st, s->pos, (uint64_t)s->n));
-    s->lp_current = false;
+    logpost_inputs_written(s);
     s->mu_linear = false;
     s->theta_ok = true;
     return 0;
@@ -899,7 +924,7 @@
 
 int launch_beta_on(gpirt_sampler_s* s, hipStream_t st)
 {
-    s->lp_current = false;
+    logpost_inputs_written(s);
     s->mu_linear = !s->ord.on;
     if (s->ord.on) {
         BetaOrdArgs a{};
@@ -957,7 +982,7 @@
     CarryState& c = s->carry;
     hipStream_t st = s->h->stream;
     GP_TRY(beta_sync(s));
-    s->lp_current = false;
+    logpost_inputs_written(s);
     s->mu_linear = false;
     if (!c.counters) {
         GP_TRY(dalloc(s, &c.counters, 6));
@@ -1268,7 +1293,7 @@
     hipStream_t st = h->stream;
     const int64_t n = s->n, m = s->m;
     GP_TRY(ell_settle_factor(s));
-    s->lp_current = false;
+    logpost_inputs_written(s);
     const uint32_t t = c.t + 1;
     const double u0 = item_uniform(s->opt.seed, t, GPIRT_ST_ELL, (uint32_t)kind, 0),
                  u1 = item_uniform(s->opt.seed, t, GPIRT_ST_ELL, (uint32_t)kind, 1);
@@ -1640,6 +1665,13 @@
 #define GP_AI(p, cnt) do { rc = dalloc(s, &(p), (size_t)(cnt), false); if (rc) { gpirt_sampler_destroy(s); return rc; } } while (0)
     GP_AI(s->tf_y8, tf_y8_bytes(s->tfd) / 8 + 2); GP_AI(s->tf_gq, tf_gq_bytes(s->tfd) / 8 + 2); GP_AI(s->tf_aux, tf_aux_bytes(s->tfd) / 8 + 2);
 #undef GP_AI
+    {
+        double* alt = nullptr;
+        rc = dalloc(s, &alt, (size_t)s->tfd.gblocks * 32, false);
+        if (rc || hipMemsetAsync(alt, 0, sizeof(double) * (size_t)s->tfd.gblocks * 32, st) != hipSuccess) { gpirt_sampler_destroy(s); return rc ? rc : GPIRT_E_HIP; }
+        s->amax_alt = reinterpret_cast<unsigned long long*>(alt);
+        s->amax_clean = 1;
+    }
     GP_A(s->f, n * m);       GP_A(s->Z, n * m);        GP_A(s->NU, n * (m > 1 + TRMV_SPLIT ? m : 1 + TRMV_SPLIT));   GP_A(s->beta, 2 * m);
     s->kr = s->opt.kstar_rank;
     if (s->kr != 0 && (!s->opt.fstar_fused || s->kr < 16 || s->kr > 128 || (s->kr % 16) != 0)) {
@@ -2051,7 +2083,7 @@
 {
     GP_ARG(s && s->initialised && s->theta_stage);
     GP_HIP(hipMemcpyAsync(s->theta, s->theta_stage, sizeof(double) * (size_t)s->n, hipMemcpyDeviceToDevice, s->h->stream));
-    s->lp_current = false;
+    logpost_inputs_written(s);
     s->mu_linear = false;
     s->theta_ok = true;
     return 0;
@@ -3346,7 +3378,7 @@
         return GPIRT_E_ARG;
     }
     GP_TRY(beta_sync(s));
-    s->lp_current = false;
+    logpost_inputs_written(s);
     s->mu_linear = false;
     GP_TRY(amp_centred_alloc(s));
     GP_TRY(smooth_factor(s));
@@ -3474,7 +3506,7 @@
         return GPIRT_E_ARG;
     }
     GP_TRY(beta_sync(s));
-    s->lp_current = false;
+    logpost_inputs_written(s);
     s->mu_linear = false;
     GP_TRY(beta_centred_alloc(s));
     GP_TRY(smooth_factor(s));
@@ -3804,7 +3836,7 @@
 {
     GP_ARG(s != nullptr);
     PopState& A = s->pop;
-    s->lp_current = false;
+    logpost_inputs_written(s);
     s->mu_linear = false;
     if (!codes) {
         if (A.mode == 2) { set_error("gpirt_sampler_pop_set(NULL): the population prior is sampled, gpirt_sampler_pop_enable(on = 0) turns it off"); return GPIRT_E_ARG; }
@@ -3847,7 +3879,7 @@
 {
     GP_ARG(s != nullptr);
     PopState& A = s->pop;
-    s->lp_current = false;
+    logpost_inputs_written(s);
     s->mu_linear = false;
     if (!on) {
         if (A.mode == 1) { set_error("gpirt_sampler_pop_enable(on = 0): the population prior is fixed, gpirt_sampler_pop_set(NULL) turns it off"); return GPIRT_E_ARG; }
@@ -3932,7 +3964,7 @@
     GP_ARG(s && s->initialised);
     PopState& A = s->pop;
     GP_TRY(needs(A.mode == 2, "the population prior's update is", "gpirt_sampler_pop_enable"));
-    s->lp_current = false;
+    logpost_inputs_written(s);
     s->mu_linear = false;
     PopUpdateArgs a{};
     a.stats = A.stats; a.mu = A.d_mu; a.sd = A.d_sd; a.P_mu = A.P_mu; a.P_sd = A.P_sd;
@@ -4038,7 +4070,7 @@
     const char* me = "gpirt_sampler_ordinal_enable";
     if (!cat) {
         GP_HIP(hipStreamSynchronize(s->h->stream));
-        s->lp_current = false;
+        logpost_inputs_written(s);
         ord_free(&A);
         return 0;
     }
@@ -4077,7 +4109,7 @@
     GP_HIP(hipMemcpyAsync(hy.data(), s->y, sizeof(double) * (size_t)(n * m), hipMemcpyDeviceToHost, st));
     GP_HIP(hipStreamSynchronize(st));
     GP_TRY(gpirt_ordinal_check(cat, hy.data(), n, m, C, hi, P, log_prior, K0, W, &s->opt));
-    s->lp_current = false;
+    logpost_inputs_written(s);
     ord_free(&A);
     auto fail = [&](int rc, const char* what) { set_error("ordinal: %s failed", what); ord_free(&A); return rc; };
     const size_t rows = (size_t)m * (size_t)(C - 1), Ps = (size_t)P;
@@ -4140,7 +4172,7 @@
     OrdState& A = s->ord;
     GP_TRY(needs(A.on, "ordinal responses are", "gpirt_sampler_ordinal_enable"));
     GP_TRY(beta_sync(s));
-    s->lp_current = false;
+    logpost_inputs_written(s);
     OrdThrArgs a{};
     a.f = s->f; a.mu = s->mu; a.cat = A.cat; a.counts = A.counts; a.n = s->n; a.m = s->m;
     a.grid = A.d_grid; a.log_prior = A.d_log_prior; a.C = A.C; a.P = A.P; a.W = A.W;
@@ -4458,6 +4490,7 @@
     GP_ARG(s && name && d_ptr && count);
     GP_TRY(lookup(s, name, d_ptr, count));
     if (strcmp(name, "theta") == 0 || strcmp(name, "beta") == 0 || strcmp(name, "mu") == 0) s->mu_linear = false;
+    if (strcmp(name, "fstar") == 0) s->amax_of_fstar = -1;
     if (strcmp(name, "y") == 0) s->ess_ypk_valid = false;
     if (strcmp(name, "L") == 0) {
         *count = s->ldl * s->n;
@@ -4505,6 +4538,13 @@
 {
     GP_ARG(s && draws);
     *draws = s->ess_pack_draws;
+    return 0;
+}
+
+int gpirt_sampler_tail_fuse_draws(gpirt_sampler_t s, int64_t* draws)
+{
+    GP_ARG(s && draws);
+    *draws = s->tail_draws;
     return 0;
 }
 
@@ -4640,7 +4680,7 @@
     GP_TRY(aux_join(dst)); GP_TRY(aux_join(src));
     GP_TRY(ensure_dense_factor(src));
     dst->L_structured = false;
-    dst->lp_current = false;
+    logpost_inputs_written(dst);
     dst->mu_linear = false;
     src->factor_fresh = false;
     invalidate_factor_products(dst);
@@ -4692,7 +4732,7 @@
             if (h_in[q] != 0.0) GP_TRY(ord_refuse(s, "gpirt_sampler_set(\"beta\") with a non-zero intercept", "the intercept is pinned at 0"));
     GP_TRY(aux_join(s));
     invalidate_factor_products(s);
-    s->lp_current = false;
+    logpost_inputs_written(s);
     if (strcmp(name, "theta") == 0 || strcmp(name, "beta") == 0 || strcmp(name, "mu") == 0) s->mu_linear = false;
     if (strcmp(name, "y") == 0) s->ess_ypk_valid = false;
     if (strcmp(name, "L") == 0 || strcmp(name, "theta") == 0) s->rows_valid = false;
@@ -4973,7 +5013,7 @@
             d += even(pt.cnt);
         }
         if (hipMemsetAsync(s->flags, 0, 4 * sizeof(int), st) != hipSuccess) return fail_hip("rollback");
-        s->mu_linear = false;
+        s->mu_linear = false; logpost_inputs_written(s);
         s->iter = k;
         return recover_factor(s);
     };
diff --git a/gpirt_amd/csrc/stages.hip b/gpirt_amd/csrc/stages.hip
--- a/gpirt_amd/csrc/stages.hip
+++ b/gpirt_amd/csrc/stages.hip
@@ -98,6 +98,59 @@
     bool consumes;
     a.out[i + j * a.N] = r_rnorm(mean, sd, z, consumes);
     if (a.mean_out) a.mean_out[i + j * a.N] = mean;
+}
+
+__global__ __launch_bounds__(256) void fstar_tail_kernel(FstarTailArgs t)
+{
+    __shared__ unsigned long long rmax[2][32];
+    const FstarEpiArgs& a = t.e;
+    const int lane = threadIdx.x & 63, wave = threadIdx.x >> 6;
+    const int wm = wave & 1, wn = wave >> 1, l15 = lane & 15, l4 = lane >> 4;
+    const int64_t i = (int64_t)blockIdx.x * 32 + wm * 16 + l15;
+    const int64_t jb = (int64_t)blockIdx.y * 32 + wn * 16;
+    const int64_t jq = jb + l15;
+    if (t.ovf_clear && blockIdx.x == 0 && blockIdx.y == 0 && threadIdx.x == 0) *t.ovf_clear = 0;
+    const bool rin = i < a.N, cin = jq < a.m;
+    const double* pa = t.V + (rin ? i : 0) + (int64_t)l4 * a.N;
+    const double* pb = t.Q + l4 + (cin ? jq : 0) * 64;
+    d4 acc = d4{0.0, 0.0, 0.0, 0.0};
+#pragma unroll
+    for (int kk = 0; kk < 16; ++kk) {
+        const double av = rin ? pa[(int64_t)(4 * kk) * a.N] : 0.0;
+        const double bv = cin ? pb[4 * kk] : 0.0;
+        acc = __builtin_amdgcn_mfma_f64_16x16x4f64(bv, av, acc, 0, 0, 0);
+    }
+    unsigned long long best = 0;
+    const double si = rin ? a.s[i] : 0.0;
+#pragma unroll
+    for (int r = 0; r < 4; ++r) {
+        const int64_t j = jb + l4 + 4 * r;
+        if (rin && j < a.m) {
+            const double prod = t.alpha * acc[r];
+            t.mean[i + j * a.N] = prod;
+            const double mean = prod + a.mu_star[i + j * a.N];
+            const double sd = a.amp ? a.amp[j] * si : si;
+            const double z = qnorm_as241(item_uniform(a.seed, a.iter, GPIRT_ST_FSTAR, a.item0 + (uint32_t)j, (uint32_t)i));
+            bool consumes;
+            const double f = r_rnorm(mean, sd, z, consumes);
+            a.out[i + j * a.N] = f;
+            if (a.mean_out) a.mean_out[i + j * a.N] = mean;
+            const unsigned long long bits = (unsigned long long)__double_as_longlong(fabs(f));
+            best = bits > best ? bits : best;
+        }
+    }
+    if (!t.amax) return;
+    unsigned long long o = __shfl_xor(best, 16);
+    best = o > best ? o : best;
+    o = __shfl_xor(best, 32);
+    best = o > best ? o : best;
+    if (l4 == 0) rmax[wn][wm * 16 + l15] = best;
+    __syncthreads();
+    if (threadIdx.x < 32) {
+        const int64_t g = (int64_t)blockIdx.x * 32 + threadIdx.x;
+        const unsigned long long b0 = rmax[0][threadIdx.x], b1 = rmax[1][threadIdx.x];
+        if (g < a.N) atomicMax(t.amax + g, b0 > b1 ? b0 : b1);
+    }
 }
 
 __global__ void fstar_advance_kernel(uint64_t* pos, const int* off, int N, int64_t m)
@@ -498,6 +551,16 @@
     return 0;
 }
 
+int launch_fstar_tail(hipStream_t stream, const FstarTailArgs& a)
+{
+    if (a.e.N <= 0 || a.e.m <= 0) return 0;
+    if (a.e.U || !a.V || !a.Q || !a.mean) { set_error("launch_fstar_tail takes the item RNG and the rank-64 operands"); return GPIRT_E_ARG; }
+    dim3 grid((unsigned)((a.e.N + 31) / 32), (unsigned)((a.e.m + 31) / 32));
+    hipLaunchKernelGGL(fstar_tail_kernel, grid, dim3(256), 0, stream, a);
+    GP_HIP(hipGetLastError());
+    return 0;
+}
+
 int launch_indicators(hipStream_t stream, const double* y, int64_t n, int64_t m, double* Ypm)
 {
     hipLaunchKernelGGL(indicators_kernel, dim3(grid_for(n * m)), dim3(256), 0, stream, y, n * m, Ypm);
diff --git a/gpirt_amd/csrc/theta_fixed.hip b/gpirt_amd/csrc/theta_fixed.hip
--- a/gpirt_amd/csrc/theta_fixed.hip
+++ b/gpirt_amd/csrc/theta_fixed.hip
@@ -62,11 +62,13 @@
 
 __global__ __launch_bounds__(256) void tf_quant_kernel(const double* __restrict__ fstar, int64_t N, int64_t m, TfDims d,
                                                        const unsigned long long* __restrict__ amax, uint4* __restrict__ Gq,
-                                                       double* __restrict__ scale, int* __restrict__ ovf)
+                                                       double* __restrict__ scale, int* __restrict__ ovf,
+                                                       unsigned long long* __restrict__ clear)
 {
     const int64_t g = (int64_t)blockIdx.x * 256 + threadIdx.x;
     const int64_t kg = blockIdx.y;
     if (g >= d.gblocks * 32) return;
+    if (clear != nullptr && kg == 0) clear[g] = 0;
     const int64_t ks = kg >> 1;
     const int lane = (int)(g & 31) + 32 * (int)(kg & 1);
     const int64_t piece = ((g >> 5) * d.ksteps + ks) * 64 + lane;
@@ -285,7 +287,8 @@
 }
 
 int launch_theta_fixed(hipStream_t stream, const double* fstar, int64_t N, int64_t n, int64_t m, const TfDims& d,
-                       const void* Y8, void* Gq, void* aux, double* logpost, int64_t ldlp, bool trace, gpirt_handle_t prof)
+                       const void* Y8, void* Gq, void* aux, double* logpost, int64_t ldlp, bool trace, gpirt_handle_t prof,
+                       const unsigned long long* amax_ready, unsigned long long* amax_clear)
 {
     if (n <= 0 || N <= 0) return 0;
     if (m > (1 << 20) || 2 * d.ksteps > 65535) { set_error("theta_fixed: m = %lld is beyond the fixed-point product's range (GPIRT_THETA_FIXED=2 selects the fp64 product)", (long long)m); return GPIRT_E_ARG; }
@@ -293,13 +296,15 @@
     unsigned long long* amax = reinterpret_cast<unsigned long long*>(aux);
     double* scale = reinterpret_cast<double*>(amax + d.gblocks * 32);
     int* ovf = tf_overflow(aux, d);
-    GP_HIP(hipMemsetAsync(aux, 0, trace ? tf_aux_bytes(d) : (size_t)d.gblocks * 32 * 16 + 16, stream));
-    if (m > 0) {
+    if (amax_ready == amax_clear && amax_ready) { set_error("theta_fixed: the maxima in place cannot be the buffer to clear"); return GPIRT_E_ARG; }
+    const bool ready = amax_ready != nullptr && !trace && m > 0;
+    if (!ready) GP_HIP(hipMemsetAsync(aux, 0, trace ? tf_aux_bytes(d) : (size_t)d.gblocks * 32 * 16 + 16, stream));
+    if (m > 0 && !ready) {
         hipLaunchKernelGGL(tf_rowmax_kernel, dim3((unsigned)((N + 255) / 256), (unsigned)((m + 15) / 16)), dim3(256), 0, stream, fstar, N, m, amax);
         GP_HIP(hipGetLastError());
     }
     hipLaunchKernelGGL(tf_quant_kernel, dim3((unsigned)((d.gblocks * 32 + 255) / 256), (unsigned)(d.ksteps * 2)), dim3(256), 0, stream,
-                       fstar, N, m, d, amax, reinterpret_cast<uint4*>(Gq), scale, ovf);
+                       fstar, N, m, d, ready ? amax_ready : amax, reinterpret_cast<uint4*>(Gq), scale, ovf, amax_clear);
     GP_HIP(hipGetLastError());
     TfMfmaArgs a;
     a.Y8 = reinterpret_cast<const unsigned char*>(Y8); a.Gq = reinterpret_cast<const unsigned char*>(Gq); a.scale = scale; a.ovf = ovf;
diff --git a/gpirt_amd/sampler.py b/gpirt_amd/sampler.py
--- a/gpirt_amd/sampler.py
+++ b/gpirt_amd/sampler.py
@@ -583,6 +583,12 @@
         return r.value
 
     @property
+    def tail_fuse_draws(self) -> int:
+        r = C.c_int64()
+        check(self.lib.gpirt_sampler_tail_fuse_draws(self._s, C.byref(r)))
+        return r.value
+
+    @property
     def fstar_free_draws(self) -> int:
         r = C.c_int64()
         check(self.lib.gpirt_sampler_fstar_free_draws(self._s, C.byref(r)))
diff --git a/include/gpirt_hip.h b/include/gpirt_hip.h
--- a/include/gpirt_hip.h
+++ b/include/gpirt_hip.h
@@ -124,6 +124,8 @@
                         const double* d_theta, const double* d_beta, int64_t n, int64_t m, uint64_t seed,
                         uint32_t iter, int* d_k_out);
 int gpirt_sampler_ess_pack_draws(gpirt_sampler_t s, int64_t* draws);
+
+int gpirt_sampler_tail_fuse_draws(gpirt_sampler_t s, int64_t* draws);
 
 int gpirt_draw_fstar(gpirt_handle_t h, const double* d_f, const double* d_theta, const double* d_L,
                      int64_t ldl, const double* d_mu_star, int64_t n, int64_t m, uint64_t seed,
```

Result: slower. 1224 (-1.1%).
